# noamzilo/sed-crnn

Measured on AMD Instinct MI355X. Metric: mel-frames/sec training throughput (seq=256, mel=40), higher is better.
Workload: dtype f32; 1 GPU; BASELINE config 2: mono (B=128,256,40,1) per GPU, 3xConv3x3(128)+BN+ReLU+pool(1,2)+dropout0.5, BiGRU 2x128, Linear(256,1), BCEWithLogits, Adam lr 1e-3; full fit step (fwd+loss+bwd+allreduce+Adam); global_batch=128, seq_len=256, n_mels=40, parallelism=single

## Files before the change

### include/sedcrnn.h

```cpp
#ifndef SEDCRNN_H
#define SEDCRNN_H

#include <stddef.h>
#include <stdint.h>

#ifdef __cplusplus
extern "C" {
#endif

#define SED_MAX_CONV 4
#define SED_MAX_GRU 4
#define SED_MAX_DENSE 4

int sed_version(void);
const char* sed_last_error_string(void);

int sed_conv3x3_pack_weights(const float* w_oihw, float* wp_fwd, float* wp_dgrad,
                             int Cout, int Cin, void* stream);

int sed_conv3x3_stat_rows(int B, int Cin, int F, int T, int Cout, int x_is_nchw);

int sed_conv3x3_fwd(const float* x, int x_is_nchw, const float* wp, const float* bias,
                    float* y, float* stat_partials,
                    int B, int Cin, int F, int T, int Cout, void* stream);
// ... 72 lines not shown
                              float drop_p, uint64_t seed, const uint64_t* seed_dev, void* stream);

int sed_bn_relu_pool_route(const float* y, const float* scale, const float* shift, unsigned char* route,
                           int B, int T, int F, int C, int pool_f, int pool_t, void* stream);
int sed_bn_bwd_rows(int B, int T, int pool_t);
int sed_bn_relu_pool_drop_bwd_reduce(const float* y, const float* dout, const float* scale,
                                     const float* shift, const float* mean, const float* rstd,
                                     float* partials, int B, int T, int F, int C, int pool_f,
                                     int pool_t, int out_tcf, float drop_p, uint64_t seed, const uint64_t* seed_dev, void* stream);
int sed_bn_bwd_finalize(const float* partials, int rows, int C, float* sum_g, float* sum_gx,
                        float* dgamma, float* dbeta, void* stream);
int sed_bn_bwd_finalize_small_gamma(const float* partials, int rows, int C, float* sum_g, float* sum_gx,
                                    float* dgamma, float* dbeta, const float* dpooled, const float* pooled,
                                    const float* y, const float* gamma, const float* beta, const float* mean,
                                    const float* rstd, const float* scale, const float* shift,
                                    int B, int T, int F, int pool_f, int pool_t, float drop_p, void* stream);
int sed_bn_bwd_reduce_pooled_supported(int F, int C, int pool_f, int pool_t, int out_tcf);
int sed_bn_bwd_reduce_pooled(const float* pooled, const float* dout, const float* gamma, const float* beta,
                             const float* y, const float* mean, const float* rstd, const float* scale, const float* shift,
                             float* partials, int B, int T, int F, int C, int pool_f, int pool_t, int out_tcf, float drop_p, void* stream);
int sed_bn_relu_pool_drop_bwd_apply(const float* y, const float* dout, const float* scale,
                                    const float* shift, const float* mean, const float* rstd,
                                    const float* sum_g, const float* sum_gx, float* dy,
                                    float* dbias_partials, int B, int T, int F, int C, int pool_f,
                                    int pool_t, int out_tcf, float drop_p, uint64_t seed, const uint64_t* seed_dev, void* stream);
int sed_reduce_rows(const float* partials, int rows, int C, int row_stride, float* out, void* stream);

int sed_conv1_fused_supported(int Cin, int F, int T, int C, int pool_f, int pool_t);
int sed_conv1_fused_rows(int B, int T);
size_t sed_conv1_stats_workspace_bytes(int B, int Cin, int T);
size_t sed_conv1_moments_doubles(int Cin);
int sed_conv1_stats(const float* x, const float* wp, const float* bias, float* stat_partials, void* workspace,
                    int B, int Cin, int F, int T, int C, double* moments, void* stream);
int sed_conv1_bn_relu_pool_drop_fwd(const float* x, const float* wp, const float* bias, const float* scale,
                                    const float* shift, float* out, int B, int Cin, int F, int T, int C,
                                    int pool_f, int pool_t, float drop_p, uint64_t seed, const uint64_t* seed_dev,
                                    unsigned char* argmax_bits, void* stream);
int sed_conv1_route(const float* x, const float* wp, const float* bias, const float* scale, const float* shift,
                    unsigned char* route, int B, int Cin, int F, int T, int C, int pool_f, int pool_t, void* stream);
int sed_conv1_bwd_reduce(const float* x, const float* wp, const float* bias, const float* dout,
                         const float* scale, const float* shift, const float* mean, const float* rstd,
                         float* partials, int B, int Cin, int F, int T, int C, int pool_f, int pool_t,
                         float drop_p, uint64_t seed, const uint64_t* seed_dev, void* stream);
size_t sed_conv1_bwd_apply_workspace_bytes(int B, int Cin, int T, int C);
int sed_conv1_bwd_apply_wgrad(const float* x, const float* wp, const float* bias, const float* dout,
                              const float* scale, const float* shift, const float* mean, const float* rstd,
                              const float* sum_g, const float* sum_gx, float* dw_oihw, float* dbias,
                              void* workspace, int B, int Cin, int F, int T, int C, int pool_f, int pool_t,
                              float drop_p, uint64_t seed, const uint64_t* seed_dev,
                              const float* gamma, const float* beta, float* dgamma, void* stream);

int sed_conv1_rgrad_supported(int Cin, int F, int T, int C, int pool_f, int pool_t);
size_t sed_conv1_bwd_wgrad_workspace_bytes(int B, int Cin, int T, int C);
int sed_conv1_bwd_wgrad(const float* x, const float* dout, const float* pooled, const unsigned char* argmax_bits,
                        const double* moments, const float* wp, const float* bias, const float* mean, const float* rstd,
                        const float* scale, const float* sum_g, const float* sum_gx, float* dw_oihw, float* dbias,
                        void* workspace, int B, int Cin, int F, int T, int C, float drop_p,
                        const float* gamma, const float* beta, float* dgamma, void* stream);
int sed_conv1_bwd_wgrad_assemble(const float* partials, int rows, const double* moments, const float* wp, const float* bias,
                                 const float* mean, const float* rstd, const float* scale, const float* sum_g,
                                 const float* sum_gx, float* dw_oihw, float* dbias, int B, int Cin, int F, int T, int C,
                                 const float* gamma, const float* beta, float* dgamma, void* stream);

int sed_gemm_f32(const float* A, long a_si, long a_sk, const float* B, long b_sk, long b_sj,
                 float* C, long ldc, const float* bias, float beta, int M, int N, int K, void* stream);
size_t sed_gemm_f32_workspace_bytes(int M, int N, int K);
int sed_gemm_f32_ws(const float* A, long a_si, long a_sk, const float* B, long b_sk, long b_sj,
                    float* C, long ldc, const float* bias, int M, int N, int K, void* workspace, void* stream);

int sed_gemm_bf16_nt(const void* A, const void* B, const float* bias, float* C, long ldc, int M, int N, int K, void* stream);

int sed_gemm_f32_wgrad(const float* A, long a_si, long a_sk, const float* B, long b_sk, long b_sj,
                       float* C, long ldc, int M, int N, int K, void* workspace, void* stream);

int sed_linear_fwd(const float* x, const float* W, const float* b, float* y,
                   int M, int K, int N, int relu, void* stream);
size_t sed_linear_bwd_workspace_bytes(int M, int K, int N);
int sed_linear_bwd(const float* x, const float* W, const float* y, float* dy, float* dx,
                   float* dW, float* db, void* workspace, int M, int K, int N, int relu, void* stream);

size_t sed_gru_seq_workspace_bytes(int H);
int sed_gru_seq_fwd(const float* gi, const float* const* whh, const float* const* bhh,
                    float* out, float* saved, void* workspace, int B, int T, int H, void* stream);
size_t sed_gru_seq_bwd_workspace_bytes(int B, int H);
int sed_gru_seq_bwd(const float* dout, const float* saved, const float* const* whh,
                    float* dgi, float* dgh, float* const* dbih, float* const* dbhh, void* workspace,
                    int B, int T, int H, void* stream);
int sed_gru_seq_variant(int B, int H, int* bt, int* hreg, int* hlds);

int sed_loss_fwd_bwd(const float* logits, const float* targets, int n, int kind, float alpha,
                     float gamma, int reduction_mean, float* loss, float* dlogits, float* probs,
                     void* stream);
int sed_sigmoid(const float* x, float* y, int n, void* stream);
int sed_scale(float* x, long n, float alpha, void* stream);

size_t sed_sqnorm_workspace_bytes(long n);
int sed_grad_norm_clip_coef(const float* g, long n, float max_norm, float* norm_out,
                            void* workspace, void* stream);
int sed_adam_step(float* p, const float* g, float* m, float* v, long n, float lr, float beta1,
                  float beta2, float eps, float weight_decay, int step, const float* grad_scale,
                  const uint64_t* step_state, void* stream);
int sed_step_advance(uint64_t* step_state, void* stream);

size_t sed_logmel_tables_bytes(const float* melfb_host, int n_fft, int n_mels);
int sed_logmel_build_tables(const float* window_host, const float* melfb_host, int n_fft, int n_mels,
                            void* tables_host, size_t tables_bytes);
int sed_logmel(const float* pcm, long n_samples, const void* tables, size_t tables_bytes,
               const float* mu, const float* inv_sigma, float* out,
               int n_fft, int hop, int n_mels, int pad_mode, void* stream);
size_t sed_logmel_batch_workspace_bytes(int R);
int sed_logmel_batch(const float* pcm, long pcm_len, const long* clips_host, int R, const void* tables, size_t tables_bytes,
                     const float* mu, const float* inv_sigma, float* out, long out_rows, int n_fft, int hop, int n_mels,
                     int pad_mode, void* workspace, size_t workspace_bytes, void* stream);
size_t sed_logmel_multi_workspace_bytes(int R, int channels);
int sed_logmel_multi(const float* pcm, long pcm_len, const long* clips_host, int R, int channels, const void* tables,
                     size_t tables_bytes, const float* mu, const float* inv_sigma, float* out, long out_rows, int n_fft, int hop,
                     int n_mels, int pad_mode, void* workspace, size_t workspace_bytes, void* stream);
size_t sed_logmel_gcc_workspace_bytes(int R, int channels);
int sed_logmel_gcc(const float* pcm, long pcm_len, const long* clips_host, int R, int channels, const void* tables,
                   size_t tables_bytes, const float* mu, const float* inv_sigma, float* out, long out_rows, int n_fft, int hop,
// ... 58 lines not shown
                      const long* table_host, int S, void* workspace, size_t workspace_bytes, void* stream);

typedef sed_tune_setting sed_decoder_setting;
int sed_detect_events_classwise(const float* probs, long n_out, int K, const sed_decoder_setting* classes_host, int max_events,
                                void* workspace, size_t workspace_bytes, int* cls, int* onset, int* offset, float* peak,
                                int* peak_frame, int* count, void* stream);
int sed_detect_events_batch_classwise(const float* probs, const long* n_out_host, int R, int K,
                                      const sed_decoder_setting* classes_host, int max_events, void* workspace, size_t workspace_bytes,
                                      int* rec, int* cls, int* onset, int* offset, float* peak, int* peak_frame, int* event_off,
                                      void* stream);
int sed_stream_step_classwise(void* state, size_t state_bytes, int S, int K, int win_out, int hop_out, int median, int max_new_windows,
                              int combine, int trim, const sed_decoder_setting* classes_host, const float* logits, long logits_len,
                              const long* table_host, int max_new_decided, float* probs, long probs_rows, int max_events,
                              int* ev_stream, int* cls, int* onset, int* offset, float* peak, int* peak_frame, int* event_off,
                              void* workspace, size_t workspace_bytes, void* stream);

typedef struct sed_net_cfg {
    int B, Cin, F, T;
    int n_conv;
    int C[SED_MAX_CONV];
    int pool_f[SED_MAX_CONV], pool_t[SED_MAX_CONV];
    float drop_p[SED_MAX_CONV];
    int n_gru;
    int H[SED_MAX_GRU];
    int n_dense;
    int D[SED_MAX_DENSE];
    float bn_eps, bn_momentum;
    int conv_mode;
    int flags;
} sed_net_cfg;
#define SED_NET_AUX_FIRST 0x1
#define SED_NET_NO_GATE 0x2
#define SED_NET_DIRECT_CONV 0x4

typedef struct sed_net_params {
    float* conv_w[SED_MAX_CONV];
    float* conv_b[SED_MAX_CONV];
    float* bn_g[SED_MAX_CONV];
    float* bn_b[SED_MAX_CONV];
    float* bn_rm[SED_MAX_CONV];
    float* bn_rv[SED_MAX_CONV];
    float* gru_wih[SED_MAX_GRU][2];
    float* gru_whh[SED_MAX_GRU][2];
    float* gru_bih[SED_MAX_GRU][2];
    float* gru_bhh[SED_MAX_GRU][2];
    float* dense_w[SED_MAX_DENSE];
    float* dense_b[SED_MAX_DENSE];
} sed_net_params;

int sed_net_out_shape(const sed_net_cfg* cfg, int* Tp, int* Fp);
size_t sed_net_workspace_bytes(const sed_net_cfg* cfg, int training);
int sed_net_forward(const sed_net_cfg* cfg, const sed_net_params* p, const float* x, float* logits,
                    void* workspace, int training, uint64_t seed, const uint64_t* seed_dev, void* stream);
int sed_net_backward(const sed_net_cfg* cfg, const sed_net_params* p, const sed_net_params* g,
                     const float* x, const float* dlogits, void* workspace, uint64_t seed, const uint64_t* seed_dev,
                     int stage_begin, int stage_end, void* stream, void* aux_stream);
int sed_net_backward_ready_stage(const sed_net_cfg* cfg, int block);

int sed_net_sync_region(const sed_net_cfg* cfg, int backward, int block, size_t* offset_bytes, size_t* n_floats);
int sed_net_forward_phases(const sed_net_cfg* cfg, const sed_net_params* p, const float* x, float* logits,
                           void* workspace, int training, uint64_t seed, int phase_begin, int phase_end,
                           float count_scale, void* stream);
int sed_net_backward_phases(const sed_net_cfg* cfg, const sed_net_params* p, const sed_net_params* g,
                            const float* x, const float* dlogits, void* workspace, uint64_t seed,
                            int phase_begin, int phase_end, float count_scale, void* stream);

int sed_net_workspace_region(const sed_net_cfg* cfg, int training, const char* name, int index,
                             size_t* offset_bytes, size_t* n_floats);

int sed_net_inference_plan(const sed_net_cfg* cfg, int* conv_bf16, int* proj_bf16);

int sed_net_routing(const sed_net_cfg* cfg, const sed_net_params* p, const float* x, const void* workspace, int block,
                    unsigned char* route, void* stream);

enum sed_kernel_tag {
    SED_K_CONV_MFMA_FWD = 0,
    SED_K_CONV_SMALL_FWD,
    SED_K_CONV_MFMA_WGRAD,
    SED_K_CONV_SMALL_WGRAD,
    SED_K_BN_FWD,
    SED_K_BN_BWD_REDUCE,
    SED_K_BN_BWD_APPLY,
    SED_K_GEMM,
    SED_K_GRU_FWD,
    SED_K_GRU_BWD,
    SED_K_ADAM,
    SED_K_LOGMEL,
    SED_K_CONV_MFMA_DGRAD,
    SED_K_COUNT
// ... 11 lines not shown
```

### sed_crnn_amd/_lib.py

```python
import ctypes as C
import os

HERE = os.path.dirname(os.path.abspath(__file__))
LIB_PATH = os.environ.get("SED_CRNN_LIB") or os.path.join(HERE, "libsedcrnn.so")

SED_MAX_CONV = 4
SED_MAX_GRU = 4
SED_MAX_DENSE = 4

_fp = C.c_void_p
_stream = C.c_void_p


class NetCfg(C.Structure):
    _fields_ = [
        ("B", C.c_int), ("Cin", C.c_int), ("F", C.c_int), ("T", C.c_int),
        ("n_conv", C.c_int),
        ("C", C.c_int * SED_MAX_CONV),
        ("pool_f", C.c_int * SED_MAX_CONV), ("pool_t", C.c_int * SED_MAX_CONV),
        ("drop_p", C.c_float * SED_MAX_CONV),
        ("n_gru", C.c_int), ("H", C.c_int * SED_MAX_GRU),
        ("n_dense", C.c_int), ("D", C.c_int * SED_MAX_DENSE),
        ("bn_eps", C.c_float), ("bn_momentum", C.c_float),
        ("conv_mode", C.c_int),
# ... 26 lines not shown
    "sed_conv3x3_stat_rows": (_i, [_i, _i, _i, _i, _i, _i]),
    "sed_conv3x3_fwd": (_i, [_fp, _i, _fp, _fp, _fp, _fp, _i, _i, _i, _i, _i, _stream]),
    "sed_conv3x3_pack_weights_ex": (_i, [_fp, _fp, _fp, _i, _i, _i, _stream]),
    "sed_conv3x3_fwd_ex": (_i, [_fp, _i, _fp, _fp, _fp, _fp, _i, _i, _i, _i, _i, _i, _stream]),
    "sed_conv3x3_wgrad_workspace_bytes": (_sz, [_i, _i, _i, _i, _i]),
    "sed_conv3x3_wgrad_zero_row_bytes": (_sz, [_i, _i, _i, _i, _i]),
    "sed_conv3x3_wgrad": (_i, [_fp, _i, _fp, _fp, _fp, _i, _i, _i, _i, _i, _stream]),
    "sed_conv3x3_wgrad_ex": (_i, [_fp, _i, _fp, _fp, _fp, _i, _i, _i, _i, _i, _i, _stream]),
    "sed_conv3x3_bn_relu_pool_eval_supported": (_i, [_i, _i, _i, _i, _i]),
    "sed_conv3x3_pack_weights_bn_folded": (_i, [_fp, _fp, _fp, _fp, _fp, _fp, _f, _fp, _fp, _i, _i, _stream]),
    "sed_conv3x3_bn_relu_pool_eval": (_i, [_fp, _fp, _fp, _fp, _i, _i, _i, _i, _i, _stream]),
    "sed_conv3x3_bf16_eval_supported": (_i, [_i, _i, _i, _i, _i]),
    "sed_conv3x3_bf16_pack_weights_bn_folded": (_i, [_fp, _fp, _fp, _fp, _fp, _fp, _f, _fp, _fp, _i, _i, _stream]),
    "sed_conv3x3_bf16_bn_relu_pool_eval": (_i, [_fp, _i, _fp, _fp, _fp, _i, _i, _i, _i, _i, _stream]),
    "sed_conv3x3_dgrad_bnred_rows": (_i, [_i, _i, _i, _i, _i]),
    "sed_conv3x3_dgrad_bnred": (_i, [_fp, _fp, _fp, _fp, _fp, _fp, _fp, _fp, _fp, _fp, _f, _i, _i, _i, _i, _i, _i, _i, _i, _i, _stream]),
    "sed_conv3x3_wino_rows": (_i, [_i, _i, _i, _i, _i]),
    "sed_conv3x3_wino_phase_ticks": (_i, [_fp]),
    "sed_conv3x3_wino_packed_floats": (_sz, [_i, _i]),
    "sed_conv3x3_wino_pack_weights": (_i, [_fp, _fp, _fp, _i, _i, _stream]),
    "sed_conv3x3_wino_fwd": (_i, [_fp, _fp, _fp, _fp, _fp, _i, _i, _i, _i, _i, _stream]),
    "sed_conv3x3_wino_dgrad_bnred": (_i, [_fp, _fp, _fp, _fp, _fp, _fp, _fp, _fp, _fp, _fp, _f, _i, _i, _i, _i, _i, _i, _i, _i, _i, _stream]),
    "sed_conv3x3_wino_pack_weights_bn_folded": (_i, [_fp, _fp, _fp, _fp, _fp, _fp, _f, _fp, _fp, _i, _i, _stream]),
    "sed_conv3x3_wino_bn_relu_pool_eval": (_i, [_fp, _fp, _fp, _fp, _i, _i, _i, _i, _i, _stream]),
    "sed_conv3x3_wino_rg_rows": (_i, [_i, _i, _i, _i, _i, _i]),
    "sed_conv3x3_wino_dgrad_bnred_rg": (_i, [_fp, _fp, _fp, _fp, _fp, _fp, _fp, _fp, _fp, _f, _fp, _i, _fp, _fp, _i, _i, _i, _i, _i, _stream]),
    "sed_conv3x3_dgrad_bnred_rg_rows": (_i, [_i, _i, _i, _i, _i, _i]),
    "sed_conv3x3_dgrad_bnred_rg": (_i, [_fp, _fp, _fp, _fp, _fp, _fp, _fp, _fp, _fp, _f, _fp, _i, _fp, _fp, _i, _i, _i, _i, _i, _stream]),
    "sed_conv1_fused_supported": (_i, [_i, _i, _i, _i, _i, _i]),
    "sed_conv1_fused_rows": (_i, [_i, _i]),
    "sed_conv1_stats_workspace_bytes": (_sz, [_i, _i, _i]),
    "sed_conv1_moments_doubles": (_sz, [_i]),
    "sed_conv1_stats": (_i, [_fp, _fp, _fp, _fp, _fp, _i, _i, _i, _i, _i, _fp, _stream]),
    "sed_conv1_bn_relu_pool_drop_fwd": (_i, [_fp, _fp, _fp, _fp, _fp, _fp, _i, _i, _i, _i, _i, _i, _i, _f, _u64, _fp, _fp, _stream]),
    "sed_conv1_rgrad_supported": (_i, [_i, _i, _i, _i, _i, _i]),
    "sed_conv1_bwd_wgrad_workspace_bytes": (_sz, [_i, _i, _i, _i]),
    "sed_conv1_bwd_wgrad": (_i, [_fp, _fp, _fp, _fp, _fp, _fp, _fp, _fp, _fp, _fp, _fp, _fp, _fp, _fp, _fp, _i, _i, _i, _i, _i, _f, _fp, _fp, _fp, _stream]),
    "sed_conv1_bwd_wgrad_assemble": (_i, [_fp, _i, _fp, _fp, _fp, _fp, _fp, _fp, _fp, _fp, _fp, _fp, _i, _i, _i, _i, _i, _fp, _fp, _fp, _stream]),
    "sed_conv1_route": (_i, [_fp, _fp, _fp, _fp, _fp, _fp, _i, _i, _i, _i, _i, _i, _i, _stream]),
    "sed_conv1_bwd_reduce": (_i, [_fp, _fp, _fp, _fp, _fp, _fp, _fp, _fp, _fp, _i, _i, _i, _i, _i, _i, _i, _f, _u64, _fp, _stream]),
    "sed_conv1_bwd_apply_workspace_bytes": (_sz, [_i, _i, _i, _i]),
    "sed_conv1_bwd_apply_wgrad": (_i, [_fp, _fp, _fp, _fp, _fp, _fp, _fp, _fp, _fp, _fp, _fp, _fp, _fp, _i, _i, _i, _i, _i, _i, _i, _f, _u64, _fp, _fp, _fp, _fp, _stream]),
    "sed_bn_finalize_train": (_i, [_fp, _i, _i, _d, _fp, _fp, _fp, _fp, _f, _f, _fp, _fp, _fp, _fp, _stream]),
    "sed_bn_stat_sums": (_i, [_fp, _i, _i, _fp, _stream]),
    "sed_bn_finalize_from_sums": (_i, [_fp, _i, _d, _fp, _fp, _fp, _fp, _f, _f, _fp, _fp, _fp, _fp, _stream]),
    "sed_bn_finalize_eval": (_i, [_fp, _fp, _fp, _fp, _f, _i, _fp, _fp, _stream]),
    "sed_bn_relu_pool_drop_fwd": (_i, [_fp, _fp, _fp, _fp, _i, _i, _i, _i, _i, _i, _i, _f, _u64, _fp, _stream]),
    "sed_bn_relu_pool_route": (_i, [_fp, _fp, _fp, _fp, _i, _i, _i, _i, _i, _i, _stream]),
    "sed_bn_bwd_rows": (_i, [_i, _i, _i]),
    "sed_bn_relu_pool_drop_bwd_reduce": (_i, [_fp, _fp, _fp, _fp, _fp, _fp, _fp, _i, _i, _i, _i, _i, _i, _i, _f, _u64, _fp, _stream]),
    "sed_bn_bwd_finalize": (_i, [_fp, _i, _i, _fp, _fp, _fp, _fp, _stream]),
    "sed_bn_bwd_finalize_small_gamma": (_i, [_fp, _i, _i, _fp, _fp, _fp, _fp, _fp, _fp, _fp, _fp, _fp, _fp, _fp, _fp, _fp, _i, _i, _i, _i, _i, _f, _stream]),
    "sed_bn_bwd_reduce_pooled_supported": (_i, [_i, _i, _i, _i, _i]),
    "sed_bn_bwd_reduce_pooled": (_i, [_fp, _fp, _fp, _fp, _fp, _fp, _fp, _fp, _fp, _fp, _i, _i, _i, _i, _i, _i, _i, _f, _stream]),
    "sed_bn_relu_pool_drop_bwd_apply": (_i, [_fp, _fp, _fp, _fp, _fp, _fp, _fp, _fp, _fp, _fp, _i, _i, _i, _i, _i, _i, _i, _f, _u64, _fp, _stream]),
    "sed_reduce_rows": (_i, [_fp, _i, _i, _i, _fp, _stream]),
    "sed_gemm_f32": (_i, [_fp, _l, _l, _fp, _l, _l, _fp, _l, _fp, _f, _i, _i, _i, _stream]),
    "sed_gemm_f32_workspace_bytes": (_sz, [_i, _i, _i]),
    "sed_gemm_f32_ws": (_i, [_fp, _l, _l, _fp, _l, _l, _fp, _l, _fp, _i, _i, _i, _fp, _stream]),
    "sed_gemm_bf16_nt": (_i, [_fp, _fp, _fp, _fp, _l, _i, _i, _i, _stream]),
    "sed_gemm_f32_wgrad": (_i, [_fp, _l, _l, _fp, _l, _l, _fp, _l, _i, _i, _i, _fp, _stream]),
    "sed_linear_fwd": (_i, [_fp, _fp, _fp, _fp, _i, _i, _i, _i, _stream]),
    "sed_linear_bwd_workspace_bytes": (_sz, [_i, _i, _i]),
    "sed_linear_bwd": (_i, [_fp, _fp, _fp, _fp, _fp, _fp, _fp, _fp, _i, _i, _i, _i, _stream]),
    "sed_gru_seq_workspace_bytes": (_sz, [_i]),
    "sed_gru_seq_fwd": (_i, [_fp, _pp, _pp, _fp, _fp, _fp, _i, _i, _i, _stream]),
    "sed_gru_seq_bwd_workspace_bytes": (_sz, [_i, _i]),
    "sed_gru_seq_bwd": (_i, [_fp, _fp, _pp, _fp, _fp, _pp, _pp, _fp, _i, _i, _i, _stream]),
    "sed_gru_seq_variant": (_i, [_i, _i, C.POINTER(_i), C.POINTER(_i), C.POINTER(_i)]),
    "sed_loss_fwd_bwd": (_i, [_fp, _fp, _i, _i, _f, _f, _i, _fp, _fp, _fp, _stream]),
    "sed_sigmoid": (_i, [_fp, _fp, _i, _stream]),
    "sed_scale": (_i, [_fp, _l, _f, _stream]),
    "sed_sqnorm_workspace_bytes": (_sz, [_l]),
    "sed_grad_norm_clip_coef": (_i, [_fp, _l, _f, _fp, _fp, _stream]),
    "sed_adam_step": (_i, [_fp, _fp, _fp, _fp, _l, _f, _f, _f, _f, _f, _i, _fp, _fp, _stream]),
    "sed_step_advance": (_i, [_fp, _stream]),
    "sed_logmel_tables_bytes": (_sz, [_fp, _i, _i]),
    "sed_logmel_build_tables": (_i, [_fp, _fp, _i, _i, _fp, _sz]),
    "sed_logmel": (_i, [_fp, _l, _fp, _sz, _fp, _fp, _fp, _i, _i, _i, _i, _stream]),
    "sed_logmel_batch_workspace_bytes": (_sz, [_i]),
    "sed_logmel_batch": (_i, [_fp, _l, _fp, _i, _fp, _sz, _fp, _fp, _fp, _l, _i, _i, _i, _i, _fp, _sz, _stream]),
    "sed_logmel_multi_workspace_bytes": (_sz, [_i, _i]),
    "sed_logmel_multi": (_i, [_fp, _l, _fp, _i, _i, _fp, _sz, _fp, _fp, _fp, _l, _i, _i, _i, _i, _fp, _sz, _stream]),
    "sed_logmel_gcc_workspace_bytes": (_sz, [_i, _i]),
    "sed_logmel_gcc": (_i, [_fp, _l, _fp, _i, _i, _fp, _sz, _fp, _fp, _fp, _l, _i, _i, _i, _i, _i, _fp, _sz, _stream]),
    "sed_resample_workspace_bytes": (_sz, [_i]),
    "sed_resample_check_table": (_i, [_fp, _i, _l, _l, _l, _i, _i, _i]),
    "sed_resample": (_i, [_fp, _l, _i, _i, _fp, _l, _fp, _l, _i, _i, _i, _fp, _i, _fp, _l, _fp, _sz, _stream]),
    "sed_resample_select_workspace_bytes": (_sz, [_i]),
    "sed_resample_select_check_table": (_i, [_fp, _i, _i, _l, _l, _l, _i, _i, _i]),
    "sed_resample_select": (_i, [_fp, _l, _i, _i, _fp, _l, _fp, _l, _i, _i, _i, _fp, _i, _fp, _l, _fp, _sz, _stream]),
    "sed_window_batch": (_i, [_fp, _fp, _l, _i, _i, _i, _fp, _fp, _fp, _i, _i, _i, _fp, _fp, _i, _i, _i, _stream]),
    "sed_pack_sequences": (_i, [_fp, _l, _i, _i, _i, _i, _fp, _stream]),
    "sed_col_mean_std_workspace_bytes": (_sz, [_i]),
    "sed_col_mean_std": (_i, [_fp, _l, _i, _fp, _fp, _fp, _stream]),
    "sed_col_standardize": (_i, [_fp, _l, _i, _fp, _fp, _fp, _stream]),
    "sed_segment_counts": (_i, [_fp, _fp, _l, _i, _i, _f, _fp, _stream]),
    "sed_detect_stitch": (_i, [_fp, _l, _i, _i, _i, _l, _l, _i, _i, _fp, _stream]),
    "sed_detect_workspace_bytes": (_sz, [_l, _i, _i]),
    "sed_detect_events": (_i, [_fp, _l, _i, _i, _f, _f, _i, _i, _i, _fp, _sz, _fp, _fp, _fp, _fp, _fp, _fp, _stream]),
    "sed_detect_batch_workspace_bytes": (_sz, [_l, _i, _i, _i]),
    "sed_detect_stitch_batch": (_i, [_fp, _l, _fp, _i, _i, _i, _i, _fp, _l, _fp, _sz, _stream]),
    "sed_detect_events_batch": (_i, [_fp, _fp, _i, _i, _i, _f, _f, _i, _i, _i, _fp, _sz, _fp, _fp, _fp, _fp, _fp, _fp, _fp, _stream]),
    "sed_tune_workspace_bytes": (_sz, [_l, _i, _i, _i, _i]),
    "sed_tune_sweep": (_i, [_fp, _fp, _i, _i, _fp, _i, _fp, _fp, _fp, _fp, _i, _i, _fp, _sz, _fp, _stream]),
    "sed_stream_state_bytes": (_sz, [_i, _i, _i, _i, _i, _i]),
    "sed_stream_init": (_i, [_fp, _sz, _i, _i, _i, _i, _i, _i, _stream]),
    "sed_stream_reset": (_i, [_fp, _sz, _i, _i, _i, _i, _i, _i, _fp, _i, _stream]),
    "sed_stream_step_workspace_bytes": (_sz, [_i, _i, _i]),
    "sed_stream_step": (_i, [_fp, _sz, _i, _i, _i, _i, _i, _i, _i, _i, _f, _f, _i, _i, _fp, _l, _fp, _i, _fp, _l, _i, _fp, _fp, _fp,
                             _fp, _fp, _fp, _fp, _fp, _sz, _stream]),
    "sed_stream_append_workspace_bytes": (_sz, [_i]),
    "sed_stream_append": (_i, [_fp, _l, _l, _fp, _l, _fp, _l, _fp, _i, _fp, _sz, _stream]),
    "sed_detect_events_classwise": (_i, [_fp, _l, _i, _fp, _i, _fp, _sz, _fp, _fp, _fp, _fp, _fp, _fp, _stream]),
    "sed_detect_events_batch_classwise": (_i, [_fp, _fp, _i, _i, _fp, _i, _fp, _sz, _fp, _fp, _fp, _fp, _fp, _fp, _fp, _stream]),
    "sed_stream_step_classwise": (_i, [_fp, _sz, _i, _i, _i, _i, _i, _i, _i, _i, _fp, _fp, _l, _fp, _i, _fp, _l, _i, _fp, _fp, _fp,
                                       _fp, _fp, _fp, _fp, _fp, _sz, _stream]),
    "sed_prof_enable": (_i, [C.c_uint]),
    "sed_prof_read": (_i, [_i, C.POINTER(_d), C.POINTER(_l), C.POINTER(_d)]),
    "sed_prof_tag_name": (C.c_char_p, [_i]),
    "sed_prof_tag_count": (_i, []),
    "sed_net_out_shape": (_i, [C.POINTER(NetCfg), C.POINTER(_i), C.POINTER(_i)]),
    "sed_net_workspace_bytes": (_sz, [C.POINTER(NetCfg), _i]),
    "sed_net_forward": (_i, [C.POINTER(NetCfg), C.POINTER(NetParams), _fp, _fp, _fp, _i, _u64, _fp, _stream]),
    "sed_net_sync_region": (_i, [C.POINTER(NetCfg), _i, _i, C.POINTER(_sz), C.POINTER(_sz)]),
    "sed_net_workspace_region": (_i, [C.POINTER(NetCfg), _i, C.c_char_p, _i, C.POINTER(_sz), C.POINTER(_sz)]),
    "sed_net_routing": (_i, [C.POINTER(NetCfg), C.POINTER(NetParams), _fp, _fp, _i, _fp, _stream]),
    "sed_net_inference_plan": (_i, [C.POINTER(NetCfg), C.POINTER(C.c_int), C.POINTER(C.c_int)]),
    "sed_net_forward_phases": (_i, [C.POINTER(NetCfg), C.POINTER(NetParams), _fp, _fp, _fp, _i, _u64, _i, _i, _f, _stream]),
    "sed_net_backward_phases": (_i, [C.POINTER(NetCfg), C.POINTER(NetParams), C.POINTER(NetParams), _fp, _fp, _fp, _u64, _i, _i, _f, _stream]),
    "sed_net_backward": (_i, [C.POINTER(NetCfg), C.POINTER(NetParams), C.POINTER(NetParams), _fp, _fp, _fp, _u64, _fp, _i, _i, _stream, _stream]),
    "sed_net_backward_ready_stage": (_i, [C.POINTER(NetCfg), _i]),
}

_lib = None


class SedHipError(RuntimeError):
    pass


def lib():
    global _lib
    if _lib is None:
        if not os.path.exists(LIB_PATH):
            raise SedHipError(
                f"{LIB_PATH} is missing: build it with `python -m sed_crnn_amd.build` "
                "(hipcc --offload-arch=gfx950). sed_crnn_amd has no fallback path.")
        L = C.CDLL(LIB_PATH)
        for name, (res, args) in SIGNATURES.items():
            fn = getattr(L, name)
            fn.restype = res
            fn.argtypes = args
        _lib = L
    return _lib


def check(rc, what=""):
    if rc != 0:
        msg = lib().sed_last_error_string().decode("utf-8", "replace")
        raise SedHipError(f"{what or 'libsedcrnn'} failed (code {rc}): {msg}")
# ... 12 lines not shown
```

### sed_crnn_amd/csrc/bnpool.hip

```cpp
#include "common.h"

#define BN_MAX_BLOCKS 1024

__device__ __forceinline__ void bn_two_channel_sums(const float* __restrict__ part, int rows, int C, int c, bool live,
                                                    double (*sred)[2][2], double* A_out, double* Q_out) {
    const int sl = threadIdx.x >> 1, lane = threadIdx.x & 63, wv = threadIdx.x >> 6;
    double a = 0.0, q = 0.0;
    if (live) {
#pragma unroll 8
        for (int r = sl; r < rows; r += 512) {
            const float* p0 = part + (size_t)r * 2 * C + c;
            a += (double)p0[0];
            q += (double)p0[C];
        }
    }
#pragma unroll
    for (int o = 2; o < 64; o <<= 1) { a += __shfl_xor(a, o, 64); q += __shfl_xor(q, o, 64); }
    if (lane < 2) { sred[wv][lane][0] = a; sred[wv][lane][1] = q; }
    __syncthreads();
    double A = 0.0, Q = 0.0;
    if (threadIdx.x < 2) {
        for (int w = 0; w < 16; ++w) { A += sred[w][threadIdx.x][0]; Q += sred[w][threadIdx.x][1]; }
    }
    *A_out = A; *Q_out = Q;
}

__global__ __launch_bounds__(1024) void bn_finalize_train_k(
    const float* __restrict__ part, int rows, int C, double count, const float* __restrict__ gamma,
    const float* __restrict__ beta, float* __restrict__ rmean, float* __restrict__ rvar, float momentum,
    float eps, float* __restrict__ mean_o, float* __restrict__ rstd_o, float* __restrict__ scale_o,
    float* __restrict__ shift_o) {
    __shared__ double sred[16][2][2];
    const int c = blockIdx.x * 2 + (threadIdx.x & 1);
    double A, Q;
    bn_two_channel_sums(part, rows, C, c, c < C, sred, &A, &Q);
    if (threadIdx.x < 2 && c < C) {
        double m = A / count;
        double var = Q / count - m * m;
        if (var < 0.0) var = 0.0;
        float rstd = (float)(1.0 / sqrt(var + (double)eps));
        float g = gamma[c], bt = beta[c];
        mean_o[c] = (float)m;
        rstd_o[c] = rstd;
        float sc = g * rstd;
        scale_o[c] = sc;
        shift_o[c] = bt - (float)m * sc;
        if (rmean) {
            double unb = count > 1.0 ? var * count / (count - 1.0) : var;
            rmean[c] = (1.f - momentum) * rmean[c] + momentum * (float)m;
            rvar[c] = (1.f - momentum) * rvar[c] + momentum * (float)unb;
        }
    }
}

extern "C" int sed_bn_finalize_train(const float* part, int rows, int C, double count, const float* gamma,
                                     const float* beta, float* rmean, float* rvar, float momentum, float eps,
                                     float* mean, float* rstd, float* scale, float* shift, void* stream) {
    SED_REQUIRE(part && gamma && beta && mean && rstd && scale && shift, "bn_finalize_train: null pointer");
    SED_REQUIRE(rows > 0 && C > 0 && count > 0, "bn_finalize_train: bad sizes rows=%d C=%d", rows, C);
    bn_finalize_train_k<<<cdiv(C, 2), 1024, 0, as_stream(stream)>>>(part, rows, C, count, gamma, beta, rmean, rvar,
                                                                      momentum, eps, mean, rstd, scale, shift);
    SED_LAUNCH_CHECK("bn_finalize_train");
    return 0;
}

__global__ __launch_bounds__(1024) void bn_stat_sums_k(const float* __restrict__ part, int rows, int C, float* __restrict__ sums) {
    __shared__ double s1[32][33], s2[32][33];
    const int cl = threadIdx.x & 31, sl = threadIdx.x >> 5;
    const int c = blockIdx.x * 32 + cl;
    double a = 0.0, q = 0.0;
    if (c < C)
#pragma unroll 8
        for (int r = sl; r < rows; r += 32) {
            a += (double)part[(size_t)r * 2 * C + c];
            q += (double)part[(size_t)r * 2 * C + C + c];
        }
    s1[sl][cl] = a;
    s2[sl][cl] = q;
    __syncthreads();
    if (sl == 0 && c < C) {
        double A = 0.0, Q = 0.0;
        for (int s = 0; s < 32; ++s) { A += s1[s][cl]; Q += s2[s][cl]; }
        sums[c] = (float)A;
        sums[C + c] = (float)Q;
// ... 656 lines not shown
```

### sed_crnn_amd/csrc/common.h

```cpp
#pragma once
#include <hip/hip_runtime.h>
#include <stdint.h>
#include <stdio.h>
#include "../../include/sedcrnn.h"

#define SED_EINVAL (-1)
#define SED_EUNSUPPORTED (-2)

void sed_set_error(const char* fmt, ...);

#define SED_REQUIRE(cond, ...)                     \
    do {                                           \
        if (!(cond)) {                             \
            sed_set_error(__VA_ARGS__);            \
            return SED_EINVAL;                     \
        }                                          \
    } while (0)

#define SED_LAUNCH_CHECK(name)                                                      \
    do {                                                                            \
        hipError_t e__ = hipGetLastError();                                         \
        if (e__ != hipSuccess) {                                                    \
            sed_set_error("%s: launch failed: %s", name, hipGetErrorString(e__));   \
            return (int)e__;                                                        \
        }                                                                           \
    } while (0)

#define SED_TRY(expr)            \
    do {                         \
        int r__ = (expr);        \
        if (r__ != 0) return r__; \
    } while (0)

extern unsigned g_sed_prof_mask;
void sed_prof_begin(int tag, hipStream_t s, double units);
void sed_prof_end(int tag, hipStream_t s);
struct SedProfScope {
    int tag; hipStream_t s; bool on;
    SedProfScope(int tag_, hipStream_t s_, double units) : tag(tag_), s(s_), on((g_sed_prof_mask >> tag_) & 1u) {
        if (on) sed_prof_begin(tag, s, units);
    }
    ~SedProfScope() { if (on) sed_prof_end(tag, s); }
};

int sed_internal_conv_pack_multi(int n, const float* const* w, float* const* wf, float* const* wd, const int* Cout, const int* Cin,
                                 const int* wino_f, const int* wino_d, void* stream);

int sed_internal_conv_pack_eval(int n, const float* const* w, const float* const* bias, const float* const* gamma,
                                const float* const* beta, const float* const* rm, const float* const* rv, float eps,
                                float* const* wf, float* const* scale, float* const* shift, float* const* bias_folded, const int* fold,
                                const int* wino, const int* Cout, const int* Cin, const float* perm_src0, const float* perm_src1, float* perm_dst,
                                int perm_rows, int perm_C, int perm_Fp, void* const* wbf16, int perm_bf16, void* stream);

int sed_internal_conv3x3_wgrad(const float* x, int x_is_nchw, const float* dy, float* dw, void* workspace,
                               int B, int Cin, int F, int T, int Cout, int mode, unsigned* arrive, void* stream);
int sed_internal_conv3x3_wgrad_workgroups(int B, int Cin, int F, int T, int Cout, int x_is_nchw, int mode);

int sed_internal_stream_gate(const unsigned* counter, unsigned target, int timeout_us, void* stream);

int sed_internal_logmel_multi(const float* pcm, long pcm_len, const long* clips_host, int R, int channels, const void* tables,
                              size_t tables_bytes, const float* mu, const float* inv_sigma, float* out, long out_rows, int n_fft, int hop,
                              int n_mels, int pad_mode, int row_stride, void* workspace, size_t workspace_bytes, void* stream);

static inline hipStream_t as_stream(void* s) { return (hipStream_t)s; }
static inline int cdiv(long a, long b) { return (int)((a + b - 1) / b); }

typedef float f32x2 __attribute__((ext_vector_type(2)));
typedef float f32x4 __attribute__((ext_vector_type(4)));
typedef float f32x16 __attribute__((ext_vector_type(16)));

#ifdef __HIPCC__
__device__ __forceinline__ uint32_t sed_fmix32(uint32_t h) {
    h ^= h >> 16; h *= 0x85ebca6bu; h ^= h >> 13; h *= 0xc2b2ae35u; h ^= h >> 16;
    return h;
}
__device__ __forceinline__ float sed_uniform(uint64_t seed, uint64_t idx) {
    uint32_t lo = (uint32_t)idx, hi = (uint32_t)(idx >> 32);
    uint32_t h = sed_fmix32(lo ^ (uint32_t)seed);
    h = sed_fmix32(h + (uint32_t)(seed >> 32) + hi * 0x9E3779B1u);
    return (float)(h >> 8) * (1.0f / 16777216.0f);
}
__device__ __forceinline__ float sed_drop_mult(uint64_t seed, uint64_t idx, float p, float inv_keep) {
    return (sed_uniform(seed, idx) >= p) ? inv_keep : 0.0f;
}

__device__ __forceinline__ int sed_fdiv(int n, float inv) { return (int)(((float)n + 0.5f) * inv); }

__device__ __forceinline__ float wave_sum(float v) {
#pragma unroll
    for (int o = 32; o > 0; o >>= 1) v += __shfl_xor(v, o, 64);
    return v;
}
__device__ __forceinline__ double wave_sum_d(double v) {
#pragma unroll
    for (int o = 32; o > 0; o >>= 1) v += __shfl_xor(v, o, 64);
    return v;
}
__device__ __forceinline__ float sigmoidf_(float x) { return 1.0f / (1.0f + __expf(-x)); }
#endif
```

### sed_crnn_amd/csrc/conv.hip

```cpp
#include "common.h"
#include "conv_shared.h"
#include <type_traits>

#define CV_CIC 32
#define CV_LD 36
#define CV_MTW 5
#define WG_FT 40
#define WG_NX 6
#define WG_ND 10

#define CV_TPAD 56
#define CV_NH 8

struct ConvPlan {
    int kind;
    int TT;
    int FT, nft;
    int nct;
    int tblocks;
    int rows;
    int nco, nci;
    size_t lds;
    double score;
};
// ... 62 lines not shown
    int cc = ci >> 5, g = (ci & 31) >> 3, h = (ci & 7) >> 2, j = ci & 3;
    int cot = co >> 5, r = co & 31;
    return ((((((size_t)tap * (Cin >> 5) + cc) * 4 + g) * (Cout >> 5) + cot) * 64) + r + 32 * h) * 4 + j;
}

__global__ void conv_pack_w_k(const float* __restrict__ w, float* __restrict__ wf,
                              float* __restrict__ wd, int Cout, int Cin) {
    int i = blockIdx.x * blockDim.x + threadIdx.x;
    int n = Cout * Cin * 9;
    if (i >= n) return;
    int tap = i % 9, ci = (i / 9) % Cin, co = i / (9 * Cin);
    float v = w[i];
    const bool frag = (Cin % 32 == 0) && (Cout % 32 == 0);
    if (wf) wf[frag ? conv_frag_index(tap, co, ci, Cout, Cin) : ((size_t)tap * Cout + co) * Cin + ci] = v;
    if (wd) wd[frag ? conv_frag_index(8 - tap, ci, co, Cin, Cout) : ((size_t)(8 - tap) * Cin + ci) * Cout + co] = v;
}

extern "C" int sed_conv3x3_pack_weights(const float* w, float* wf, float* wd, int Cout, int Cin, void* stream) {
    SED_REQUIRE(w && Cout > 0 && Cin > 0, "conv3x3_pack_weights: bad arguments");
    int n = Cout * Cin * 9;
    conv_pack_w_k<<<cdiv(n, 256), 256, 0, as_stream(stream)>>>(w, wf, wd, Cout, Cin);
    SED_LAUNCH_CHECK("conv_pack_w");
    return 0;
}

struct ConvPackMulti {
    const float* w[SED_MAX_CONV]; float* wf[SED_MAX_CONV]; float* wd[SED_MAX_CONV]; int Cout[SED_MAX_CONV], Cin[SED_MAX_CONV];
    const float* gamma[SED_MAX_CONV]; const float* beta[SED_MAX_CONV]; const float* rm[SED_MAX_CONV]; const float* rv[SED_MAX_CONV];
    const float* bias[SED_MAX_CONV]; float* scale_out[SED_MAX_CONV]; float* shift_out[SED_MAX_CONV]; float* bias_out[SED_MAX_CONV];
    int fold[SED_MAX_CONV]; float eps;
    int wino_f[SED_MAX_CONV], wino_d[SED_MAX_CONV];
    const float* perm_src[2]; float* perm_dst; int perm_rows, perm_C, perm_Fp;
    __bf16* wb[SED_MAX_CONV]; int perm_bf16;
};
__global__ void conv_pack_w_multi_k(ConvPackMulti a, int n) {
    const int l = blockIdx.y;
    const int i = blockIdx.x * blockDim.x + threadIdx.x;
    if (l == n) {
        extern __shared__ __attribute__((aligned(16))) float prow[];
        const int K = a.perm_C * a.perm_Fp;
        for (int row = blockIdx.x; row < 2 * a.perm_rows; row += gridDim.x) {
            const float* src = a.perm_src[row >= a.perm_rows] + (size_t)(row >= a.perm_rows ? row - a.perm_rows : row) * K;
            __syncthreads();
            for (int k = threadIdx.x; k < K; k += blockDim.x) prow[k] = src[k];
            __syncthreads();
            float* dst = a.perm_dst + (size_t)row * K;
            for (int k = threadIdx.x; k < K; k += blockDim.x) {
                const int f = k / a.perm_C, c = k - f * a.perm_C;
                if (a.perm_bf16) ((__bf16*)a.perm_dst + (size_t)row * K)[k] = (__bf16)prow[c * a.perm_Fp + f];
                else dst[k] = prow[c * a.perm_Fp + f];
            }
        }
        return;
    }
    const int Cout = a.Cout[l], Cin = a.Cin[l];
    if (a.wino_f[l] | a.wino_d[l])
        wino_pack_one(a.w[l], a.wino_f[l] ? a.wf[l] : nullptr, a.wino_d[l] ? a.wd[l] : nullptr, Cout, Cin, i,
                      a.fold[l] ? a.gamma[l] : nullptr, a.rv[l], a.eps);
    if (a.gamma[l] && i < Cout) {
        const float sc = a.gamma[l][i] / sqrtf(a.rv[l][i] + a.eps), sh = a.beta[l][i] - a.rm[l][i] * sc;
        if (a.scale_out[l]) { a.scale_out[l][i] = sc; a.shift_out[l][i] = sh; }
        if (a.fold[l]) a.bias_out[l][i] = (a.bias[l] ? a.bias[l][i] : 0.f) * sc + sh;
    }
    if (i >= Cout * Cin * 9) return;
    const int tap = i % 9, ci = (i / 9) % Cin, co = i / (9 * Cin);
    float v = a.w[l][i];
    if (a.fold[l]) v *= a.gamma[l][co] / sqrtf(a.rv[l][co] + a.eps);
    const bool frag = (Cin % 32 == 0) && (Cout % 32 == 0);
    if (a.wb[l]) a.wb[l][bf16_eval_frag_index(tap, co, ci, Cout, Cin)] = (__bf16)v;
    if (a.wf[l] && !a.wino_f[l]) a.wf[l][frag ? conv_frag_index(tap, co, ci, Cout, Cin) : ((size_t)tap * Cout + co) * Cin + ci] = v;
    if (a.wd[l] && !a.wino_d[l]) a.wd[l][frag ? conv_frag_index(8 - tap, ci, co, Cin, Cout) : ((size_t)(8 - tap) * Cin + ci) * Cout + co] = v;
}
static int set_lds_early(size_t bytes) {
    hipError_t e = hipFuncSetAttribute((const void*)conv_pack_w_multi_k, hipFuncAttributeMaxDynamicSharedMemorySize, (int)bytes);
    if (e != hipSuccess) { sed_set_error("hipFuncSetAttribute(%zu B LDS): %s", bytes, hipGetErrorString(e)); return (int)e; }
    return 0;
}
static int pack_multi_launch(const ConvPackMulti& a, int n, void* stream) {
    int nmax = 0;
    for (int l = 0; l < n; ++l) {
        const int nl = a.Cout[l] * a.Cin[l] * 9;
        if (nl > nmax) nmax = nl;
    }
    const int gx = cdiv(nmax > 0 ? nmax : 1, 256);
    const size_t lds = a.perm_src[0] ? (size_t)a.perm_C * a.perm_Fp * sizeof(float) : 0;
    SED_REQUIRE(lds <= 64 * 1024, "conv_pack: a GRU input row of %zu bytes does not fit the re-ordering buffer", lds);
    if (lds > 48 * 1024) SED_TRY(set_lds_early(lds));
    conv_pack_w_multi_k<<<dim3(gx, n + (a.perm_src[0] ? 1 : 0)), 256, lds, as_stream(stream)>>>(a, n);
    SED_LAUNCH_CHECK("conv_pack_w_multi");
    return 0;
}
int sed_internal_conv_pack_multi(int n, const float* const* w, float* const* wf, float* const* wd, const int* Cout, const int* Cin,
                                 const int* wino_f, const int* wino_d, void* stream) {
    SED_REQUIRE(n > 0 && n <= SED_MAX_CONV && w && wf && wd && Cout && Cin, "conv_pack_multi: bad arguments");
    ConvPackMulti a{};
    for (int l = 0; l < n; ++l) {
        SED_REQUIRE(w[l] && Cout[l] > 0 && Cin[l] > 0, "conv_pack_multi: bad layer %d", l);
        a.w[l] = w[l]; a.wf[l] = wf[l]; a.wd[l] = wd[l]; a.Cout[l] = Cout[l]; a.Cin[l] = Cin[l];
        a.wino_f[l] = (wino_f && wino_f[l] && wf[l]) ? 1 : 0;
        a.wino_d[l] = (wino_d && wino_d[l] && wd[l]) ? 1 : 0;
        SED_REQUIRE(!(a.wino_f[l] | a.wino_d[l]) || (Cout[l] % 64 == 0 && Cin[l] % 64 == 0), "conv_pack_multi: layer %d cannot take the Winograd packing", l);
    }
    return pack_multi_launch(a, n, stream);
}
int sed_internal_conv_pack_eval(int n, const float* const* w, const float* const* bias, const float* const* gamma,
                                const float* const* beta, const float* const* rm, const float* const* rv, float eps,
                                float* const* wf, float* const* scale, float* const* shift, float* const* bias_folded, const int* fold,
                                const int* wino, const int* Cout, const int* Cin, const float* perm_src0, const float* perm_src1, float* perm_dst,
                                int perm_rows, int perm_C, int perm_Fp, void* const* wbf16, int perm_bf16, void* stream) {
    SED_REQUIRE(n > 0 && n <= SED_MAX_CONV && w && gamma && beta && rm && rv && wf && scale && shift && fold && Cout && Cin, "conv_pack_eval: bad arguments");
    ConvPackMulti a{};
    for (int l = 0; l < n; ++l) {
        const bool wb = wbf16 && wbf16[l];
        SED_REQUIRE(w[l] && gamma[l] && beta[l] && rm[l] && rv[l] && (wf[l] || wb) && Cout[l] > 0 && Cin[l] > 0, "conv_pack_eval: bad layer %d", l);
        SED_REQUIRE(!wb || (fold[l] && Cout[l] % 32 == 0 && Cin[l] % 16 == 0 && !(wino && wino[l])), "conv_pack_eval: layer %d cannot take the bf16 packing", l);
        a.wb[l] = wb ? (__bf16*)wbf16[l] : nullptr;
        SED_REQUIRE(fold[l] ? (bias_folded && bias_folded[l]) : (scale[l] && shift[l]), "conv_pack_eval: layer %d lacks its outputs", l);
        a.w[l] = w[l]; a.wf[l] = wf[l]; a.Cout[l] = Cout[l]; a.Cin[l] = Cin[l];
        a.gamma[l] = gamma[l]; a.beta[l] = beta[l]; a.rm[l] = rm[l]; a.rv[l] = rv[l]; a.bias[l] = bias ? bias[l] : nullptr;
        a.scale_out[l] = scale[l]; a.shift_out[l] = shift[l]; a.bias_out[l] = bias_folded ? bias_folded[l] : nullptr; a.fold[l] = fold[l];
        a.wino_f[l] = (wino && wino[l]) ? 1 : 0;
        SED_REQUIRE(!a.wino_f[l] || (Cout[l] % 64 == 0 && Cin[l] % 64 == 0), "conv_pack_eval: layer %d cannot take the Winograd packing", l);
    }
    a.eps = eps;
    if (perm_src0) {
        SED_REQUIRE(perm_src1 && perm_dst && perm_rows > 0 && perm_C > 0 && perm_Fp > 0, "conv_pack_eval: bad permutation");
        a.perm_src[0] = perm_src0; a.perm_src[1] = perm_src1; a.perm_dst = perm_dst; a.perm_rows = perm_rows; a.perm_C = perm_C; a.perm_Fp = perm_Fp;
        a.perm_bf16 = perm_bf16 ? 1 : 0;
// ... 1871 lines not shown
```

### sed_crnn_amd/csrc/conv1.hip

```cpp
#include "common.h"

#define C1_TT 4
#define C1_MAXBLOCKS 2048

template <int CIN>
struct C1W { f32x4 w[9 * CIN]; f32x4 b; };

template <int CIN>
__device__ __forceinline__ void c1_load_w(C1W<CIN>& W, const float* __restrict__ wp, const float* __restrict__ bias,
                                          int Cout, int cg) {
#pragma unroll
    for (int tap = 0; tap < 9; ++tap)
#pragma unroll
        for (int ci = 0; ci < CIN; ++ci)
#pragma unroll
            for (int k = 0; k < 4; ++k) W.w[tap * CIN + ci][k] = wp[((size_t)tap * Cout + cg * 4 + k) * CIN + ci];
    W.b = bias ? *(const f32x4*)(bias + cg * 4) : (f32x4){0, 0, 0, 0};
}

template <int CIN>
__device__ __forceinline__ f32x4 c1_conv(const C1W<CIN>& W, const float* __restrict__ halo, int tl, int f, int F2) {
    f32x4 acc = W.b;
#pragma unroll
    for (int kh = 0; kh < 3; ++kh)
// ... 285 lines not shown
            const int tl = q / F, f = q - tl * F;
            const int b = tile / tblocks, t0 = (tile - b * tblocks) * C1_GT;
            if (t0 + tl >= T) continue;
            const float* hb = halo + u * hn;
            float v[NK];
#pragma unroll
            for (int kh = 0; kh < 3; ++kh)
#pragma unroll
                for (int kw = 0; kw < 3; ++kw)
#pragma unroll
                    for (int ci = 0; ci < CIN; ++ci) v[(kh * 3 + kw) * CIN + ci] = hb[((tl + kw) * F2 + f + kh) * CIN + ci];
            int g = NK;
#pragma unroll
            for (int k = 0; k < NK; ++k) {
                acc[k] += v[k];
#pragma unroll
                for (int k2 = k; k2 < NK; ++k2) acc[g++] += v[k] * v[k2];
            }
        }
    }
    __syncthreads();
    float* red = smem;
    const int lane = tid & 63, wave = tid >> 6;
#pragma unroll
    for (int i = 0; i < NG; ++i) {
        const float sum = wave_sum(acc[i]);
        if (lane == 0) red[i * 4 + wave] = sum;
    }
    __syncthreads();
    for (int i = tid; i < NG; i += 256)
        partials[(size_t)blockIdx.x * NG + i] = (red[i * 4] + red[i * 4 + 1]) + (red[i * 4 + 2] + red[i * 4 + 3]);
}

template <int CIN>
__global__ __launch_bounds__(256) void conv1_gram_finalize_k(const float* __restrict__ partials, int nblk, const float* __restrict__ wp,
                                                             const float* __restrict__ bias, double count, int C, float* __restrict__ stat,
                                                             double* __restrict__ gram_out) {
    constexpr int NK = 9 * CIN, NG = NK + NK * (NK + 1) / 2;
    __shared__ double G[NG];
    __shared__ double Gq[4][64];
    {
        const int il = threadIdx.x & 63, q = threadIdx.x >> 6;
        for (int i0 = 0; i0 < NG; i0 += 64) {
            const int i = i0 + il;
            double a = 0.0;
            if (i < NG) {
#pragma unroll 8
                for (int r = q; r < nblk; r += 4) a += (double)partials[(size_t)r * NG + i];
            }
            Gq[q][il] = a;
            __syncthreads();
            if (q == 0 && i < NG) G[i] = (Gq[0][il] + Gq[1][il]) + (Gq[2][il] + Gq[3][il]);
            __syncthreads();
        }
    }
    __syncthreads();
    if (gram_out)
        for (int i = threadIdx.x; i < NG; i += 256) gram_out[i] = G[i];
    for (int c = threadIdx.x; c < C; c += 256) {
        double w[NK];
#pragma unroll
        for (int k = 0; k < NK; ++k) w[k] = (double)wp[((size_t)(k / CIN) * C + c) * CIN + (k % CIN)];
        const double b = bias ? (double)bias[c] : 0.0;
        double ws1 = 0.0, q = 0.0;
        int g = NK;
#pragma unroll
        for (int k = 0; k < NK; ++k) {
            ws1 += w[k] * G[k];
#pragma unroll
            for (int k2 = k; k2 < NK; ++k2) { q += (k2 == k ? 1.0 : 2.0) * w[k] * w[k2] * G[g]; ++g; }
        }
        stat[c] = (float)(count * b + ws1);
        stat[C + c] = (float)(q + 2.0 * b * ws1 + count * b * b);
    }
}

#define C1_MM_BLOCKS 1024
typedef float f32x4_t __attribute__((ext_vector_type(4)));
template <int CIN>
__global__ __launch_bounds__(256) void conv1_moments_mfma_k(const float* __restrict__ x, float* __restrict__ partials, int B, int F, int T) {
    constexpr int NK = 9 * CIN, NT = (NK + 1 + 15) / 16, NP = NT * (NT + 1) / 2;
    extern __shared__ __attribute__((aligned(16))) float smem[];
    const int F2 = F + 2;
    const int hn = (C1_GT + 2) * F2 * CIN;
    float* halo = smem;
    const int tid = threadIdx.x, lane = tid & 63, wave = tid >> 6, m = lane & 15, kq = lane >> 4;
    const int tblocks = (T + C1_GT - 1) / C1_GT, ntiles = B * tblocks;
    int off[NT];
    bool real[NT];
#pragma unroll
    for (int t = 0; t < NT; ++t) {
        const int fi = 16 * t + m;
        real[t] = fi < NK;
        const int k = real[t] ? fi : 0, tap = k / CIN, ci = k - tap * CIN, kh = tap / 3, kw = tap - kh * 3;
        off[t] = real[t] ? (kw * F2 + kh) * CIN + ci + kq * CIN : hn + (fi == NK ? 0 : 1);
    }
    f32x4_t acc[NP];
#pragma unroll
    for (int q = 0; q < NP; ++q) acc[q] = (f32x4_t){0.f, 0.f, 0.f, 0.f};
    if (tid == 0) { halo[hn] = 1.f; halo[hn + 1] = 0.f; }
    for (int tile = blockIdx.x; tile < ntiles; tile += gridDim.x) {
        const int b = tile / tblocks, t0 = (tile - b * tblocks) * C1_GT;
        __syncthreads();
        for (int j = tid; j < hn; j += 256) {
            int tt = j % (C1_GT + 2), ff = (j / (C1_GT + 2)) % F2, ci = j / ((C1_GT + 2) * F2);
            const int t = t0 + tt - 1, f = ff - 1;
            float v = 0.f;
// ... 388 lines not shown
#define C1_LAUNCH(CIN_, P12_)                                                                                          \
    do {                                                                                                               \
        if (lds > 48 * 1024)                                                                                           \
            (void)hipFuncSetAttribute((const void*)conv1_fused_k<CIN_, MODE, P12_>, hipFuncAttributeMaxDynamicSharedMemorySize, (int)lds); \
        conv1_fused_k<CIN_, MODE, P12_><<<grid, 256, lds, s>>>(x, wp, bias, scale, shift, mean, rstd, sum_g, sum_gx, dout, out, \
                                                              partials, B, F, T, C, pf, pt, drop_p, seed, seed_dev);  \
    } while (0)
    if (Cin == 1) { if (p12) C1_LAUNCH(1, true); else C1_LAUNCH(1, false); }
    else if (Cin == 2) { if (p12) C1_LAUNCH(2, true); else C1_LAUNCH(2, false); }
    else if ((MODE == 1 || MODE == 4) && p12) {
        if (Cin == 3) C1_LAUNCH(3, true);
        else C1_LAUNCH(4, true);
    } else {
        sed_set_error("conv1: %d input channels are supported by the forward pass with the (1,2) pool only", Cin);
        return SED_EUNSUPPORTED;
    }
#undef C1_LAUNCH
    return 0;
}

#define C1_CHECK(who)                                                                                             \
    SED_REQUIRE(sed_conv1_fused_supported(Cin, F, T, C, pf, pt), who ": shape Cin=%d F=%d T=%d C=%d pool=(%d,%d) is not " \
                "supported by the fused first block", Cin, F, T, C, pf, pt)

extern "C" size_t sed_conv1_stats_workspace_bytes(int B, int Cin, int T) {
    const int nk = 9 * Cin;
    if (Cin > 2) {
        const int nt = (nk + 1 + 15) / 16, np = nt * (nt + 1) / 2;
        return (size_t)C1_MM_BLOCKS * np * 256 * sizeof(float) + (size_t)(nk + nk * (nk + 1) / 2) * sizeof(double);
    }
    return (size_t)256 * (nk + nk * (nk + 1) / 2) * sizeof(float);
}

extern "C" int sed_conv1_stats(const float* x, const float* wp, const float* bias, float* stat_partials, void* workspace,
                               int B, int Cin, int F, int T, int C, double* gram_out, void* stream) {
    SED_REQUIRE(x && wp && stat_partials && workspace, "conv1_stats: null pointer");
    SED_REQUIRE(c1_shape_ok(Cin, F, T, C, 1, 1, 4), "conv1_stats: shape Cin=%d F=%d T=%d C=%d is not supported", Cin, F, T, C);
    hipStream_t s = as_stream(stream);
    SedProfScope prof(SED_K_CONV_SMALL_FWD, s, 4.0 * B * Cin * (double)F * T);
    if (Cin > 2) {
        const int nk = 9 * Cin, nt = (nk + 1 + 15) / 16, np = nt * (nt + 1) / 2;
        int nb = B * ((T + C1_GT - 1) / C1_GT);
        if (nb > C1_MM_BLOCKS) nb = C1_MM_BLOCKS;
        size_t lds = ((size_t)(C1_GT + 2) * (F + 2) * Cin + 4) * sizeof(float), red = (size_t)4 * np * 256 * sizeof(float);
        if (red > lds) lds = red;
        SED_REQUIRE(lds <= 150 * 1024, "conv1_stats: F=%d Cin=%d needs %zu B of LDS", F, Cin, lds);
        const double cnt = (double)B * T * F;
        double* G = gram_out ? gram_out : (double*)((float*)workspace + (size_t)C1_MM_BLOCKS * np * 256);
#define C1_MOM(CIN_)                                                                                                              \
    do {                                                                                                                          \
        if (lds > 48 * 1024) (void)hipFuncSetAttribute((const void*)conv1_moments_mfma_k<CIN_>, hipFuncAttributeMaxDynamicSharedMemorySize, (int)lds); \
        conv1_moments_mfma_k<CIN_><<<nb, 256, lds, s>>>(x, (float*)workspace, B, F, T);                                             \
        conv1_moments_mfma_sum_k<CIN_><<<dim3(nk + 1, nk + 1), 64, 0, s>>>((const float*)workspace, nb, G);                       \
        conv1_moments_stat_k<CIN_><<<cdiv(C, 4), 256, 0, s>>>(G, wp, bias, cnt, C, stat_partials);                                 \
    } while (0)
        if (Cin == 3) C1_MOM(3); else C1_MOM(4);
#undef C1_MOM
        SED_LAUNCH_CHECK("conv1_moments");
        return 0;
    }
    const int pf = 1, pt = 1;
    C1_CHECK("conv1_stats");
    int grid = (B * ((T + C1_GT - 1) / C1_GT) + C1_GR - 1) / C1_GR;
    if (grid > 256) grid = 256;
    const int nk = 9 * Cin, ng = nk + nk * (nk + 1) / 2;
    size_t lds = (size_t)C1_GR * (C1_GT + 2) * (F + 2) * Cin * sizeof(float), red = (size_t)ng * 4 * sizeof(float);
    SED_REQUIRE(lds <= 150 * 1024, "conv1_stats: F=%d Cin=%d needs %zu B of LDS", F, Cin, lds);
    if (red > lds) lds = red;
    const double count = (double)B * T * F;
    if (lds > 48 * 1024) {
        (void)hipFuncSetAttribute((const void*)conv1_gram_k<1>, hipFuncAttributeMaxDynamicSharedMemorySize, (int)lds);
        (void)hipFuncSetAttribute((const void*)conv1_gram_k<2>, hipFuncAttributeMaxDynamicSharedMemorySize, (int)lds);
    }
    if (Cin == 1) {
        conv1_gram_k<1><<<grid, 256, lds, s>>>(x, (float*)workspace, B, F, T);
        SED_LAUNCH_CHECK("conv1_gram");
        conv1_gram_finalize_k<1><<<1, 256, 0, s>>>((const float*)workspace, grid, wp, bias, count, C, stat_partials, gram_out);
    } else {
        conv1_gram_k<2><<<grid, 256, lds, s>>>(x, (float*)workspace, B, F, T);
        SED_LAUNCH_CHECK("conv1_gram");
        conv1_gram_finalize_k<2><<<1, 256, 0, s>>>((const float*)workspace, grid, wp, bias, count, C, stat_partials, gram_out);
    }
    SED_LAUNCH_CHECK("conv1_gram_finalize");
    return 0;
}

extern "C" int sed_conv1_bn_relu_pool_drop_fwd(const float* x, const float* wp, const float* bias, const float* scale,
                                               const float* shift, float* out, int B, int Cin, int F, int T, int C,
                                               int pf, int pt, float drop_p, uint64_t seed, const uint64_t* seed_dev,
                                               unsigned char* argmax_bits, void* stream) {
    SED_REQUIRE(x && wp && scale && shift && out, "conv1_fwd: null pointer");
    SED_REQUIRE(drop_p >= 0.f && drop_p < 1.f, "conv1_fwd: drop_p=%f out of [0,1)", drop_p);
    SED_REQUIRE(c1_shape_ok(Cin, F, T, C, pf, pt, (pf == 1 && pt == 2) ? 4 : 2), "conv1_fwd: shape Cin=%d F=%d T=%d C=%d pool=(%d,%d) is not "
                "supported by the fused first block", Cin, F, T, C, pf, pt);
    hipStream_t s = as_stream(stream);
    SedProfScope prof(SED_K_BN_FWD, s, 4.0 * B * C * (double)(T / pt) * (F / pf));
    SED_REQUIRE(!argmax_bits || (pf == 1 && pt == 2), "conv1_fwd: arg-max bits exist for the (1,2) pool only");
    SED_TRY(c1_launch<1>(x, wp, bias, scale, shift, nullptr, nullptr, nullptr, nullptr, nullptr, out, reinterpret_cast<float*>(argmax_bits), B, Cin, F, T, C, pf, pt, drop_p, seed, seed_dev, s));
    SED_LAUNCH_CHECK("conv1_fwd");
    return 0;
}

extern "C" int sed_conv1_route(const float* x, const float* wp, const float* bias, const float* scale, const float* shift,
                               unsigned char* route, int B, int Cin, int F, int T, int C, int pf, int pt, void* stream) {
    SED_REQUIRE(x && wp && scale && shift && route, "conv1_route: null pointer");
    SED_REQUIRE(c1_shape_ok(Cin, F, T, C, pf, pt, (pf == 1 && pt == 2) ? 4 : 2), "conv1_route: shape Cin=%d F=%d T=%d C=%d pool=(%d,%d) is not "
                "supported by the fused first block", Cin, F, T, C, pf, pt);
    SED_REQUIRE(pf * pt <= 254, "conv1_route: a %dx%d window does not fit the one-byte code", pf, pt);
    SED_TRY(c1_launch<4>(x, wp, bias, scale, shift, nullptr, nullptr, nullptr, nullptr, nullptr, reinterpret_cast<float*>(route), nullptr,
                         B, Cin, F, T, C, pf, pt, 0.f, 0, nullptr, as_stream(stream)));
    SED_LAUNCH_CHECK("conv1_route");
    return 0;
}

extern "C" int sed_conv1_bwd_reduce(const float* x, const float* wp, const float* bias, const float* dout,
                                    const float* scale, const float* shift, const float* mean, const float* rstd,
                                    float* partials, int B, int Cin, int F, int T, int C, int pf, int pt, float drop_p,
// ... 103 lines not shown
```

### sed_crnn_amd/csrc/gemm.hip

```cpp
#include <type_traits>
#include "common.h"

#define GM_BK 32
#define GM_LDK 36

template <bool KC, int NR, int TILE>
__device__ __forceinline__ void gm_load(f32x4* reg, const float* __restrict__ P, long s_mn, long s_k, int mn0, int MN,
                                        int K, int vec, int k0, int tid) {
#pragma unroll
    for (int u = 0; u < NR; ++u) {
        int i = tid + u * 256;
        f32x4 v = {0, 0, 0, 0};
        if (KC) {
            int row = i >> 3, kq = i & 7;
            int m = mn0 + row, k = k0 + kq * 4;
            const float* p = P + (long)m * s_mn + k;
            if (m < MN) {
                if (vec && k + 3 < K) v = *(const f32x4*)p;
                else
#pragma unroll
                    for (int e = 0; e < 4; ++e) if (k + e < K) v[e] = p[e];
            }
        } else {
            int kk = i / (TILE / 4), mq = i - kk * (TILE / 4);
// ... 393 lines not shown
    double a = 0.0;
#pragma unroll 8
    for (int c = 0; c < chunks; ++c) a += (double)part[(size_t)c * tot + i];
    if (i < NK) dW[i] = (float)a;
    else if (db) db[i - NK] = (float)a;
}

extern "C" size_t sed_linear_bwd_workspace_bytes(int M, int K, int N) {
    return (size_t)cdiv(M, LIN_CHUNK) * ((size_t)N * K + N) * sizeof(float);
}

extern "C" int sed_linear_bwd(const float* x, const float* W, const float* y, float* dy, float* dx, float* dW,
                              float* db, void* workspace, int M, int K, int N, int relu, void* stream) {
    SED_REQUIRE(x && W && dy && dW && workspace && M > 0 && K > 0 && N > 0, "linear_bwd: bad arguments");
    SED_REQUIRE(!relu || y, "linear_bwd: relu=1 needs the forward output y");
    hipStream_t s = as_stream(stream);
    if (relu) {
        long n = (long)M * N;
        linear_relu_mask_k<<<cdiv(n, 256), 256, 0, s>>>(y, dy, n);
        SED_LAUNCH_CHECK("linear_relu_mask");
    }
    if (dx) {
        long n = (long)M * K;
        linear_dx_k<<<cdiv(n, 256), 256, 0, s>>>(dy, W, dx, M, K, N);
        SED_LAUNCH_CHECK("linear_dx");
    }
    int tot = N * K + N, chunks = cdiv(M, LIN_CHUNK);
    linear_dw_partial_k<<<dim3(cdiv(tot, 256), chunks), 256, 0, s>>>(dy, x, (float*)workspace, M, K, N);
    SED_LAUNCH_CHECK("linear_dw_partial");
    linear_dw_reduce_k<<<cdiv(tot, 256), 256, 0, s>>>((const float*)workspace, chunks, tot, N * K, dW, db);
    SED_LAUNCH_CHECK("linear_dw_reduce");
    return 0;
}
```

### sed_crnn_amd/csrc/gru.hip

```cpp
#include "common.h"

static inline int gru_bt(int H, int B) {
    int bt = B >= 512 ? 4 : (B >= 256 ? 2 : 1);
    if (H >= 128 && bt > 2) bt = 2;
    return bt;
}

__global__ void gru_pack_whh_t_k(const float* __restrict__ w0, const float* __restrict__ w1,
                                 float* __restrict__ wt, int H) {
    int i = blockIdx.x * blockDim.x + threadIdx.x;
    int n = 3 * H * H;
    if (i >= 2 * n) return;
    int dir = i / n, e = i - dir * n;
    int g = e / H, k = e - g * H;
    const float* w = dir ? w1 : w0;
    wt[(size_t)dir * n + (size_t)k * 3 * H + g] = w[e];
}

constexpr int gru_nt(int hreg) { return hreg > 0 ? ((3 * hreg + 63) / 64) * 64 : 1024; }

__device__ __forceinline__ float gru_dot4(float w0, float w1, float w2, float w3, const f32x4& h) {
    return fmaf(w3, h[3], fmaf(w2, h[2], fmaf(w0, h[0], w1 * h[1])));
}

// ... 273 lines not shown
    const int bt = gru_bt(H, B);
    if (H == 8 || H == 16 || H == 32 || H == 64 || H == 128) return {bt, H, 0};
    if (H == 256 && bt == 1) return {bt, hyb_hreg, GRU_HL};
    return {bt, 0, 0};
}

extern "C" int sed_gru_seq_variant(int B, int H, int* bt, int* hreg, int* hlds) {
    SED_REQUIRE(bt && hreg && hlds, "gru_seq_variant: null pointer");
    SED_REQUIRE(B > 0 && H > 0 && H % 4 == 0 && 3 * H <= 1024, "gru_seq_variant: H=%d must be a multiple of 4 and <= 341", H);
    const GruVariant v = gru_variant(H, B, GRU_HR_FWD);
    *bt = v.bt; *hreg = v.hreg; *hlds = v.hlds;
    return 0;
}

#define GRU_BT3(HR, KERNEL, ...)                                                              \
    if (v.bt == 1) KERNEL<HR, 1><<<grid, nt, lds, s>>>(__VA_ARGS__);                          \
    else if (v.bt == 2) KERNEL<HR, 2><<<grid, nt, lds, s>>>(__VA_ARGS__);                     \
    else KERNEL<HR, 4><<<grid, nt, lds, s>>>(__VA_ARGS__)
#define GRU_DISPATCH(KERNEL, ...)                                                             \
    if (v.hlds > 0) {                                                                         \
        KERNEL<GRU_HRX, 1, 256, GRU_HL><<<grid, nt, lds + (size_t)GRU_HL * 768 * sizeof(float), s>>>(__VA_ARGS__); \
    } else switch (v.hreg) {                                                                  \
        case 8: GRU_BT3(8, KERNEL, __VA_ARGS__); break;                                       \
        case 16: GRU_BT3(16, KERNEL, __VA_ARGS__); break;                                     \
        case 32: GRU_BT3(32, KERNEL, __VA_ARGS__); break;                                     \
        case 64: GRU_BT3(64, KERNEL, __VA_ARGS__); break;                                     \
        case 128:                                                                             \
            if (v.bt == 1) KERNEL<128, 1><<<grid, nt, lds, s>>>(__VA_ARGS__);                 \
            else KERNEL<128, 2><<<grid, nt, lds, s>>>(__VA_ARGS__);                           \
            break;                                                                            \
        default: GRU_BT3(0, KERNEL, __VA_ARGS__); break;                                      \
    }

extern "C" int sed_gru_seq_fwd(const float* gi, const float* const* whh, const float* const* bhh, float* out,
                               float* saved, void* workspace, int B, int T, int H, void* stream) {
    SED_REQUIRE(gi && whh && bhh && out && workspace && whh[0] && whh[1] && bhh[0] && bhh[1], "gru_seq_fwd: null pointer");
    SED_REQUIRE(B > 0 && T > 0 && H > 0 && H % 4 == 0 && 3 * H <= 1024, "gru_seq_fwd: H=%d must be a multiple of 4 and <= 341", H);
    hipStream_t s = as_stream(stream);
    float* wt = (float*)workspace;
    int n = 2 * 3 * H * H;
    gru_pack_whh_t_k<<<cdiv(n, 256), 256, 0, s>>>(whh[0], whh[1], wt, H);
    SED_LAUNCH_CHECK("gru_pack_whh_t");
    const GruVariant v = gru_variant(H, B, GRU_HR_FWD);
    dim3 grid(cdiv(B, v.bt), 2);
    int nt = gru_threads(H);
    size_t lds = (size_t)v.bt * 4 * H * sizeof(float);
    SedProfScope prof(SED_K_GRU_FWD, s, 2.0 * 2 * B * (double)T * 3 * H * H);
    if (v.hlds > 0)
        (void)hipFuncSetAttribute((const void*)gru_seq_fwd_k<GRU_HR_FWD, 1, 256, GRU_HL>, hipFuncAttributeMaxDynamicSharedMemorySize, 160 * 1024);
#define GRU_HRX GRU_HR_FWD
    GRU_DISPATCH(gru_seq_fwd_k, gi, wt, bhh[0], bhh[1], out, saved, B, T, H);
#undef GRU_HRX
    SED_LAUNCH_CHECK("gru_seq_fwd");
    return 0;
}

extern "C" size_t sed_gru_seq_bwd_workspace_bytes(int B, int H) { return (size_t)cdiv(B, gru_bt(H, B)) * 2 * 4 * H * sizeof(float); }

extern "C" int sed_gru_seq_bwd(const float* dout, const float* saved, const float* const* whh, float* dgi,
                               float* dgh, float* const* dbih, float* const* dbhh, void* workspace, int B, int T,
                               int H, void* stream) {
    SED_REQUIRE(dout && saved && whh && whh[0] && whh[1] && dgi && dgh, "gru_seq_bwd: null pointer");
    const bool want_bias = dbih && dbhh;
    SED_REQUIRE(!want_bias || (workspace && dbih[0] && dbih[1] && dbhh[0] && dbhh[1]), "gru_seq_bwd: bias gradients need all four outputs and a workspace");
    float* bpart = want_bias ? (float*)workspace : nullptr;
    SED_REQUIRE(B > 0 && T > 0 && H > 0 && H % 4 == 0 && 3 * H <= 1024, "gru_seq_bwd: H=%d must be a multiple of 4 and <= 341", H);
    hipStream_t s = as_stream(stream);
    const GruVariant v = gru_variant(H, B, GRU_HR);
    dim3 grid(cdiv(B, v.bt), 2);
    int nt = gru_threads(H);
    size_t lds = (size_t)v.bt * 6 * H * sizeof(float);
    SedProfScope prof(SED_K_GRU_BWD, s, 2.0 * 2 * B * (double)T * 3 * H * H);
    if (v.hlds > 0)
        (void)hipFuncSetAttribute((const void*)gru_seq_bwd_k<GRU_HR, 1, 256, GRU_HL>, hipFuncAttributeMaxDynamicSharedMemorySize, 160 * 1024);
#define GRU_HRX GRU_HR
    GRU_DISPATCH(gru_seq_bwd_k, dout, saved, whh[0], whh[1], dgi, dgh, bpart, B, T, H);
#undef GRU_HRX
    SED_LAUNCH_CHECK("gru_seq_bwd");
    if (want_bias) {
        gru_bias_grad_k<<<cdiv(8 * H, 256), 256, 0, s>>>(bpart, cdiv(B, v.bt), H, dbih[0], dbih[1], dbhh[0], dbhh[1]);
        SED_LAUNCH_CHECK("gru_bias_grad");
    }
    return 0;
}
```

### sed_crnn_amd/csrc/misc.hip

```cpp
#include "common.h"

__global__ __launch_bounds__(1024) void loss_fwd_bwd_k(const float* __restrict__ x, const float* __restrict__ t,
                                                       int n, int kind, float alpha, float gamma, float scale,
                                                       float* __restrict__ loss, float* __restrict__ dx,
                                                       float* __restrict__ probs) {
    __shared__ double red[16];
    double acc = 0.0;
    for (int i = threadIdx.x; i < n; i += 1024) {
        float xi = x[i], ti = t[i];
        float p = 1.f / (1.f + expf(-xi));
        float l, d;
        if (kind == 0) {
            l = fmaxf(xi, 0.f) - xi * ti + log1pf(expf(-fabsf(xi)));
            d = p - ti;
        } else {
            bool pos = (ti == 1.f);
            float pt = pos ? p : 1.f - p;
            float om = 1.f - pt;
            float lg = logf(pt + 1e-12f);
            float pw = powf(om, gamma);
            l = -alpha * pw * lg;
            float dpw = (gamma == 0.f) ? 0.f : gamma * powf(om, gamma - 1.f);
            float dl_dpt = -alpha * (-dpw * lg + pw / (pt + 1e-12f));
            float dpt_dx = pos ? p * (1.f - p) : -p * (1.f - p);
            d = dl_dpt * dpt_dx;
        }
        acc += (double)l;
        if (dx) dx[i] = d * scale;
        if (probs) probs[i] = p;
    }
    acc = wave_sum_d(acc);
    if ((threadIdx.x & 63) == 0) red[threadIdx.x >> 6] = acc;
    __syncthreads();
    if (threadIdx.x == 0) {
        double a = 0.0;
        for (int w = 0; w < 16; ++w) a += red[w];
        loss[0] = (float)(a * (double)scale);
    }
}

extern "C" int sed_loss_fwd_bwd(const float* logits, const float* targets, int n, int kind, float alpha, float gamma,
                                int reduction_mean, float* loss, float* dlogits, float* probs, void* stream) {
    SED_REQUIRE(logits && targets && loss && n > 0, "loss_fwd_bwd: bad arguments");
    SED_REQUIRE(kind == 0 || kind == 1, "loss_fwd_bwd: kind must be 0 (bce) or 1 (focal)");
    float scale = reduction_mean ? 1.f / (float)n : 1.f;
    loss_fwd_bwd_k<<<1, 1024, 0, as_stream(stream)>>>(logits, targets, n, kind, alpha, gamma, scale, loss, dlogits, probs);
    SED_LAUNCH_CHECK("loss_fwd_bwd");
    return 0;
}

__global__ void sigmoid_k(const float* __restrict__ x, float* __restrict__ y, int n) {
    int i = blockIdx.x * blockDim.x + threadIdx.x;
    if (i < n) y[i] = 1.f / (1.f + expf(-x[i]));
}

extern "C" int sed_sigmoid(const float* x, float* y, int n, void* stream) {
    SED_REQUIRE(x && y && n > 0, "sigmoid: bad arguments");
    sigmoid_k<<<cdiv(n, 256), 256, 0, as_stream(stream)>>>(x, y, n);
    SED_LAUNCH_CHECK("sigmoid");
// ... 126 lines not shown
```

### sed_crnn_amd/csrc/net.hip

```cpp
#include <string.h>
#include "common.h"

namespace {

struct ConvL { int Cin, C, T, F, Tp, Fp, pf, pt, rows, bn_rows, nchw, fused; float drop;
               int red_rows;
               int rg_rows;
               int rgrad;
               int wino, wino_d;
               int ev;
               int bf; };

struct GruL { int in, H; };

struct Layout {
    int n_conv, n_gru, n_dense, M, Tp, Fp, feat;
    int proj_bf;
    ConvL cv[SED_MAX_CONV];
    GruL gr[SED_MAX_GRU];
    int dK[SED_MAX_DENSE], dN[SED_MAX_DENSE];
    size_t wp_f[SED_MAX_CONV], wp_d[SED_MAX_CONV], conv_out[SED_MAX_CONV], stat[SED_MAX_CONV];
    size_t mean[SED_MAX_CONV], rstd[SED_MAX_CONV], scale[SED_MAX_CONV], shift[SED_MAX_CONV];
    size_t pooled[SED_MAX_CONV], bn_sums[SED_MAX_CONV], c1_stat_ws, c1_bits, c1_mom;
    size_t bias_f[SED_MAX_CONV];
    size_t wih_perm;
    size_t gi[SED_MAX_GRU], gout[SED_MAX_GRU], saved[SED_MAX_GRU], gru_ws;
    size_t act[SED_MAX_DENSE];
    size_t wgrad_zrow;
    size_t wg_arrive;
    size_t bn_part, sum_g, sum_gx, dbias_part, dconv[SED_MAX_CONV], gradA, wgrad_ws, wgrad_ws_aux, c1_ws, dgi[SED_MAX_GRU], dgh[SED_MAX_GRU], gru_bws, dgout[SED_MAX_GRU];
    size_t dact[SED_MAX_DENSE], lin_ws, gemm_ws, gemm_ws_aux;
    size_t total;
};

struct Carver {
    size_t off = 0;
    size_t take(size_t n) { size_t o = off; off += (n + 63) & ~(size_t)63; return o; }
};

int build_layout(const sed_net_cfg* c, int training, Layout* L) {
    SED_REQUIRE(c, "net: null config");
    SED_REQUIRE(c->B > 0 && c->Cin > 0 && c->F > 0 && c->T > 0, "net: bad input shape B=%d Cin=%d F=%d T=%d", c->B, c->Cin, c->F, c->T);
    SED_REQUIRE(c->n_conv >= 1 && c->n_conv <= SED_MAX_CONV, "net: n_conv=%d out of range", c->n_conv);
    SED_REQUIRE(c->n_gru >= 1 && c->n_gru <= SED_MAX_GRU, "net: n_gru=%d out of range", c->n_gru);
    SED_REQUIRE(c->n_dense >= 1 && c->n_dense <= SED_MAX_DENSE, "net: n_dense=%d out of range", c->n_dense);
    SED_REQUIRE(c->conv_mode >= 0 && c->conv_mode <= 2, "net: conv_mode=%d (0 = exact fp32, 1 = bf16x3 experiment, 2 = bf16 inference)", c->conv_mode);
    SED_REQUIRE(c->conv_mode != 2 || !training, "net: conv_mode 2 (bf16 inference) is an eval-only plan; training runs with conv_mode 0 or 1");
    SED_REQUIRE((c->flags & ~(SED_NET_AUX_FIRST | SED_NET_NO_GATE | SED_NET_DIRECT_CONV)) == 0, "net: unknown flags 0x%x", c->flags);
    memset(L, 0, sizeof(*L));
    L->n_conv = c->n_conv; L->n_gru = c->n_gru; L->n_dense = c->n_dense;
    const int fm = c->conv_mode == 2 ? 0 : c->conv_mode;
    int bfl[SED_MAX_CONV] = {0};
    if (c->conv_mode == 2) {
        int Ci = c->Cin, Ti = c->T, Fi = c->F;
        int ok[SED_MAX_CONV] = {0};
        for (int l = 0; l < c->n_conv; ++l) {
            const int pf = c->pool_f[l], pt = c->pool_t[l];
            ok[l] = l > 0 && pf == 1 && pt == 2 && c->C[l] > 0 && Ti >= 2 && sed_conv3x3_bf16_eval_supported(c->B, Ci, Fi, Ti, c->C[l]);
            if (l == c->n_conv - 1 && (size_t)c->C[l] * Fi * sizeof(float) > 64 * 1024) ok[l] = 0;
            Ci = c->C[l]; Ti = pt > 0 ? Ti / pt : Ti; Fi = pf > 0 ? Fi / pf : Fi;
        }
        for (int l = c->n_conv - 1; l >= 0 && ok[l]; --l) bfl[l] = 1;
    }
    Carver cv;
    int Cin = c->Cin, T = c->T, F = c->F;
    size_t max_pool = 0, max_wgrad = 0, c1_ws = 64, c1_stat_ws = 64;
    int max_bn_rows = 0, maxC = 0;
    for (int l = 0; l < c->n_conv; ++l) {
        ConvL& q = L->cv[l];
        q.Cin = Cin; q.C = c->C[l]; q.T = T; q.F = F; q.pf = c->pool_f[l]; q.pt = c->pool_t[l];
        q.drop = c->drop_p[l]; q.nchw = (l == 0);
        SED_REQUIRE(q.C > 0 && q.C % 4 == 0, "net: conv channels C[%d]=%d must be a positive multiple of 4", l, q.C);
        SED_REQUIRE(q.pf >= 1 && q.pt >= 1 && T / q.pt >= 1 && F / q.pf >= 1,
                    "net: block %d: T=%d/F=%d smaller than the pool (%d,%d)", l, T, F, q.pt, q.pf);
        SED_REQUIRE(q.drop >= 0.f && q.drop < 1.f, "net: drop_p[%d]=%f out of [0,1)", l, q.drop);
        q.Tp = T / q.pt; q.Fp = F / q.pf;
        q.fused = (l == 0 && c->n_conv > 1 && sed_conv1_fused_supported(q.Cin, q.F, q.T, q.C, q.pf, q.pt)) ? 1 : 0;
        q.bf = bfl[l];
        if (l == 0 && !q.fused && c->n_conv > 1 && q.Cin <= 4 && fm == 0 &&
            sed_conv1_rgrad_supported(q.Cin, q.F, q.T, q.C, q.pf, q.pt) &&
            sed_conv3x3_dgrad_bnred_rows(c->B, c->C[1], q.F / q.pf, q.T / q.pt, q.C) > 0)
// ... 51 lines not shown
        if (l == 1 && rr > 0 && L->cv[0].fused && L->cv[0].rgrad && L->cv[0].Cin <= 2) {
            const int gr = q.wino_d ? sed_conv3x3_wino_rg_rows(c->B, q.C, q.F, q.T, q.Cin, L->cv[0].Cin)
                                    : sed_conv3x3_dgrad_bnred_rg_rows(c->B, q.C, q.F, q.T, q.Cin, L->cv[0].Cin);
            L->cv[0].rg_rows = gr;
            const size_t need = (size_t)gr * q.Cin * (1 + 9 * L->cv[0].Cin);
            if (need > c1_ws) c1_ws = need;
        }
    }
    L->c1_stat_ws = cv.take(c1_stat_ws);
    L->c1_bits = L->cv[0].rgrad ? cv.take(((size_t)c->B * L->cv[0].Tp * L->cv[0].Fp * (L->cv[0].C / 4) + 3) / 4) : 0;
    L->c1_mom = L->cv[0].rgrad ? cv.take(2 * sed_conv1_moments_doubles(L->cv[0].Cin)) : 0;
    L->Tp = T; L->Fp = F; L->feat = Cin * F; L->M = c->B * T;
    const size_t M = (size_t)L->M;
    if (L->cv[c->n_conv - 1].ev && (size_t)L->feat * sizeof(float) > 64 * 1024) {
        ConvL& q = L->cv[c->n_conv - 1];
        q.ev = 0;
        L->conv_out[c->n_conv - 1] = cv.take((size_t)c->B * q.T * q.F * q.C);
    }
    L->proj_bf = L->cv[c->n_conv - 1].bf;
    L->wih_perm = ((L->cv[c->n_conv - 1].ev || L->proj_bf) && c->H[0] > 0) ? cv.take((size_t)6 * c->H[0] * L->feat / (L->proj_bf ? 2 : 1)) : 0;
    int in = L->feat, maxH = 0, max2H = 0;
    for (int i = 0; i < c->n_gru; ++i) {
        int H = c->H[i];
        SED_REQUIRE(H > 0 && H % 4 == 0 && 3 * H <= 1024, "net: GRU hidden H[%d]=%d must be a multiple of 4 and <= 341", i, H);
        L->gr[i].in = in; L->gr[i].H = H;
        L->gi[i] = cv.take(M * 6 * H);
        L->gout[i] = cv.take(M * 2 * H);
        L->saved[i] = training ? cv.take(M * 10 * H) : 0;
        if (H > maxH) maxH = H;
        in = 2 * H;
        if (in > max2H) max2H = in;
    }
    L->gru_ws = cv.take((size_t)6 * maxH * maxH);
    size_t max_lin_ws = 0;
    for (int j = 0; j < c->n_dense; ++j) {
        SED_REQUIRE(c->D[j] > 0, "net: dense size D[%d]=%d", j, c->D[j]);
        L->dK[j] = in; L->dN[j] = c->D[j];
        L->act[j] = (j < c->n_dense - 1) ? cv.take(M * c->D[j]) : 0;
        size_t w = sed_linear_bwd_workspace_bytes(L->M, in, c->D[j]) / sizeof(float);
        if (w > max_lin_ws) max_lin_ws = w;
        in = c->D[j];
    }
    if (training) {
        L->bn_part = cv.take((size_t)max_bn_rows * 2 * maxC);
        L->sum_g = cv.take((size_t)2 * maxC); L->sum_gx = 0;
        L->dbias_part = cv.take((size_t)max_bn_rows * maxC);
        for (int l = 0; l < c->n_conv; ++l)
            L->dconv[l] = L->cv[l].fused ? 0 : cv.take((size_t)c->B * L->cv[l].T * L->cv[l].F * L->cv[l].C);
        size_t ga = max_pool > M * (size_t)L->feat ? max_pool : M * (size_t)L->feat;
        L->gradA = cv.take(ga);
        L->wg_arrive = cv.take(64);
        L->wgrad_ws = cv.take(max_wgrad + 64);
        L->wgrad_ws_aux = cv.take(max_wgrad + 64);
        L->c1_ws = cv.take(c1_ws);
        for (int i = 0; i < c->n_gru; ++i) {
            L->dgi[i] = cv.take(M * 6 * c->H[i]);
            L->dgh[i] = cv.take(M * 6 * c->H[i]);
        }
        L->gru_bws = cv.take(sed_gru_seq_bwd_workspace_bytes(c->B, maxH) / sizeof(float));
        for (int i = 0; i < c->n_gru; ++i) L->dgout[i] = cv.take(M * 2 * c->H[i]);
        for (int j = 0; j < c->n_dense - 1; ++j) L->dact[j] = cv.take(M * c->D[j]);
        L->lin_ws = cv.take(max_lin_ws);
    }
    {
        size_t gw = 0;
        for (int i = 0; i < c->n_gru; ++i) {
            size_t f = sed_gemm_f32_workspace_bytes(L->M, 6 * c->H[i], L->gr[i].in) / sizeof(float);
            if (f > gw) gw = f;
            if (training) {
                size_t a = sed_gemm_f32_workspace_bytes(3 * c->H[i], c->H[i], L->M) / sizeof(float);
                size_t b = sed_gemm_f32_workspace_bytes(6 * c->H[i], L->gr[i].in, L->M) / sizeof(float);
                if (a > gw) gw = a;
                if (b > gw) gw = b;
            }
        }
        L->gemm_ws = cv.take(gw + 64);
        L->gemm_ws_aux = training ? cv.take(gw + 64) : 0;
    }
    L->total = cv.off;
    return 0;
}

inline uint64_t layer_seed(uint64_t seed, int l) { return seed + 0x9E3779B97F4A7C15ull * (uint64_t)(l + 1); }

}

extern "C" int sed_net_out_shape(const sed_net_cfg* cfg, int* Tp, int* Fp) {
    Layout L;
    SED_TRY(build_layout(cfg, 0, &L));
    if (Tp) *Tp = L.Tp;
    if (Fp) *Fp = L.Fp;
    return 0;
}

extern "C" size_t sed_net_workspace_bytes(const sed_net_cfg* cfg, int training) {
    Layout L;
    if (build_layout(cfg, training, &L) != 0) return 0;
    return L.total * sizeof(float);
}

static int forward_impl(const sed_net_cfg* c, const sed_net_params* p, const float* x, float* logits, void* workspace,
                        int training, uint64_t seed, const uint64_t* seed_dev, int pb, int pe, float count_scale, void* stream) {
    SED_REQUIRE(p && x && logits && workspace, "net_forward: null pointer");
    Layout L;
    SED_TRY(build_layout(c, training, &L));
    SED_REQUIRE(pb >= 0 && pe <= 2 * L.n_conv + 1 && pb < pe, "net_forward: bad phase range [%d,%d)", pb, pe);
    float* ws = (float*)workspace;
    const int B = c->B;
    SED_REQUIRE(c->conv_mode != 2 || (pb == 0 && pe == 2 * L.n_conv + 1), "net_forward: the bf16 inference plan (conv_mode 2) runs whole, not in phases");
    const bool eval_plan = !training && (c->conv_mode == 0 || c->conv_mode == 2) && pb == 0 && pe == 2 * L.n_conv + 1;
    const ConvL& qtop = L.cv[L.n_conv - 1];
    const bool wih_permuted = eval_plan && (qtop.ev || L.proj_bf) && L.wih_perm != 0;
    if (eval_plan) {
        const float* w[SED_MAX_CONV]; const float* bs[SED_MAX_CONV]; const float* gm[SED_MAX_CONV]; const float* bt[SED_MAX_CONV];
        const float* rm[SED_MAX_CONV]; const float* rv[SED_MAX_CONV];
        float* wf[SED_MAX_CONV]; float* sc[SED_MAX_CONV]; float* sh[SED_MAX_CONV]; float* bf[SED_MAX_CONV];
        int fold[SED_MAX_CONV], co[SED_MAX_CONV], ci[SED_MAX_CONV], wn[SED_MAX_CONV];
        void* wb[SED_MAX_CONV];
        for (int l = 0; l < L.n_conv; ++l) {
            SED_REQUIRE(p->conv_w[l] && p->conv_b[l] && p->bn_g[l] && p->bn_b[l] && p->bn_rm[l] && p->bn_rv[l],
                        "net_forward: missing parameters of conv block %d", l);
            w[l] = p->conv_w[l]; bs[l] = p->conv_b[l]; gm[l] = p->bn_g[l]; bt[l] = p->bn_b[l]; rm[l] = p->bn_rm[l]; rv[l] = p->bn_rv[l];
            wf[l] = ws + L.wp_f[l]; sc[l] = ws + L.scale[l]; sh[l] = ws + L.shift[l]; bf[l] = ws + L.bias_f[l];
            fold[l] = L.cv[l].ev || L.cv[l].bf; co[l] = L.cv[l].C; ci[l] = L.cv[l].Cin; wn[l] = L.cv[l].ev && L.cv[l].wino;
            wb[l] = L.cv[l].bf ? (void*)wf[l] : nullptr;
            if (L.cv[l].bf) wf[l] = nullptr;
        }
        if (wih_permuted) SED_REQUIRE(p->gru_wih[0][0] && p->gru_wih[0][1], "net_forward: missing parameters of GRU layer 0");
        SED_TRY(sed_internal_conv_pack_eval(L.n_conv, w, bs, gm, bt, rm, rv, c->bn_eps, wf, sc, sh, bf, fold, wn, co, ci,
                                            wih_permuted ? p->gru_wih[0][0] : nullptr, wih_permuted ? p->gru_wih[0][1] : nullptr,
                                            ws + L.wih_perm, 3 * L.gr[0].H, qtop.C, qtop.Fp, wb, L.proj_bf, stream));
        for (int l = 0; l < L.n_conv; ++l) {
            const ConvL& q = L.cv[l];
            const float* in = (l == 0) ? x : ws + L.pooled[l - 1];
            const int last = (l == L.n_conv - 1);
            if (q.bf) {
                SED_TRY(sed_conv3x3_bf16_bn_relu_pool_eval(in, l > 0 && L.cv[l - 1].bf, ws + L.wp_f[l], ws + L.bias_f[l], ws + L.pooled[l],
                                                           B, q.Cin, q.F, q.T, q.C, stream));
            } else if (q.fused) {
                SED_TRY(sed_conv1_bn_relu_pool_drop_fwd(in, ws + L.wp_f[l], p->conv_b[l], ws + L.scale[l], ws + L.shift[l], ws + L.pooled[l],
                                                        B, q.Cin, q.F, q.T, q.C, q.pf, q.pt, 0.f, 0, nullptr, nullptr, stream));
            } else if (q.ev && q.wino) {
                SED_TRY(sed_conv3x3_wino_bn_relu_pool_eval(in, ws + L.wp_f[l], ws + L.bias_f[l], ws + L.pooled[l], B, q.Cin, q.F, q.T, q.C, stream));
            } else if (q.ev) {
                SED_TRY(sed_conv3x3_bn_relu_pool_eval(in, ws + L.wp_f[l], ws + L.bias_f[l], ws + L.pooled[l], B, q.Cin, q.F, q.T, q.C, stream));
            } else {
                SED_TRY(sed_conv3x3_fwd_ex(in, q.nchw, ws + L.wp_f[l], p->conv_b[l], ws + L.conv_out[l], nullptr, B, q.Cin, q.F, q.T, q.C, 0, stream));
                SED_TRY(sed_bn_relu_pool_drop_fwd(ws + L.conv_out[l], ws + L.scale[l], ws + L.shift[l], ws + L.pooled[l], B,
                                                  q.T, q.F, q.C, q.pf, q.pt, last, 0.f, 0, nullptr, stream));
            }
        }
    }
    const bool packed_up_front = !eval_plan && pb == 0 && c->conv_mode == 0 && L.n_conv > 1;
    if (packed_up_front) {
        const float* w[SED_MAX_CONV]; float* wf[SED_MAX_CONV]; float* wd[SED_MAX_CONV]; int co[SED_MAX_CONV], ci[SED_MAX_CONV];
        int wnf[SED_MAX_CONV], wnd[SED_MAX_CONV];
        for (int l = 0; l < L.n_conv; ++l) {
            SED_REQUIRE(p->conv_w[l], "net_forward: missing parameters of conv block %d", l);
            w[l] = p->conv_w[l]; wf[l] = ws + L.wp_f[l]; wd[l] = (training && l > 0) ? ws + L.wp_d[l] : nullptr;
            co[l] = L.cv[l].C; ci[l] = L.cv[l].Cin; wnf[l] = L.cv[l].wino; wnd[l] = L.cv[l].wino_d;
        }
        SED_TRY(sed_internal_conv_pack_multi(L.n_conv, w, wf, wd, co, ci, wnf, wnd, stream));
    }
    for (int l = 0; l < L.n_conv && !eval_plan; ++l) {
        const ConvL& q = L.cv[l];
        const float* in = (l == 0) ? x : ws + L.pooled[l - 1];
        const bool do_a = pb <= 2 * l && 2 * l < pe, do_b = pb <= 2 * l + 1 && 2 * l + 1 < pe;
        if (!do_a && !do_b) continue;
        const bool one_shot = do_a && do_b && count_scale == 1.f;
        SED_REQUIRE(p->conv_w[l] && p->conv_b[l] && p->bn_g[l] && p->bn_b[l] && p->bn_rm[l] && p->bn_rv[l],
                    "net_forward: missing parameters of conv block %d", l);
        if (do_a) {
            if (!packed_up_front) {
                float* const wdp = (training && l > 0) ? ws + L.wp_d[l] : nullptr;
                if (q.wino || (q.wino_d && wdp))
                    SED_TRY(sed_conv3x3_wino_pack_weights(p->conv_w[l], q.wino ? ws + L.wp_f[l] : nullptr, q.wino_d ? wdp : nullptr, q.C, q.Cin, stream));
                if (!q.wino || (wdp && !q.wino_d))
                    SED_TRY(sed_conv3x3_pack_weights_ex(p->conv_w[l], q.wino ? nullptr : ws + L.wp_f[l], q.wino_d ? nullptr : wdp,
                                                        q.C, q.Cin, (l > 0) ? c->conv_mode : 0, stream));
            }
            if (q.fused) {
                if (training) SED_TRY(sed_conv1_stats(in, ws + L.wp_f[l], p->conv_b[l], ws + L.stat[l], ws + L.c1_stat_ws, B, q.Cin, q.F, q.T, q.C,
                                                      q.rgrad ? (double*)(ws + L.c1_mom) : nullptr, stream));
            } else if (q.wino) {
                SED_TRY(sed_conv3x3_wino_fwd(in, ws + L.wp_f[l], p->conv_b[l], ws + L.conv_out[l], training ? ws + L.stat[l] : nullptr,
                                             B, q.Cin, q.F, q.T, q.C, stream));
            } else {
                SED_TRY(sed_conv3x3_fwd_ex(in, q.nchw, ws + L.wp_f[l], p->conv_b[l], ws + L.conv_out[l],
                                           training ? ws + L.stat[l] : nullptr, B, q.Cin, q.F, q.T, q.C, (l > 0) ? c->conv_mode : 0, stream));
            }
            if (training && !one_shot) SED_TRY(sed_bn_stat_sums(ws + L.stat[l], q.rows, q.C, ws + L.bn_sums[l], stream));
        }
        if (!do_b) continue;
        const double count = (double)B * q.T * q.F;
        if (training && one_shot)
            SED_TRY(sed_bn_finalize_train(ws + L.stat[l], q.rows, q.C, count, p->bn_g[l], p->bn_b[l],
                                          p->bn_rm[l], p->bn_rv[l], c->bn_momentum, c->bn_eps, ws + L.mean[l],
                                          ws + L.rstd[l], ws + L.scale[l], ws + L.shift[l], stream));
        else if (training)
            SED_TRY(sed_bn_finalize_from_sums(ws + L.bn_sums[l], q.C, count * (double)count_scale, p->bn_g[l], p->bn_b[l],
                                              p->bn_rm[l], p->bn_rv[l], c->bn_momentum, c->bn_eps, ws + L.mean[l],
                                              ws + L.rstd[l], ws + L.scale[l], ws + L.shift[l], stream));
        else
            SED_TRY(sed_bn_finalize_eval(p->bn_g[l], p->bn_b[l], p->bn_rm[l], p->bn_rv[l], c->bn_eps, q.C,
                                         ws + L.scale[l], ws + L.shift[l], stream));
        const int last = (l == L.n_conv - 1);
        if (q.fused)
            SED_TRY(sed_conv1_bn_relu_pool_drop_fwd(in, ws + L.wp_f[l], p->conv_b[l], ws + L.scale[l], ws + L.shift[l],
                                                    ws + L.pooled[l], B, q.Cin, q.F, q.T, q.C, q.pf, q.pt,
                                                    training ? q.drop : 0.f, layer_seed(seed, l), seed_dev,
                                                    (training && q.rgrad) ? (unsigned char*)(ws + L.c1_bits) : nullptr, stream));
        else
            SED_TRY(sed_bn_relu_pool_drop_fwd(ws + L.conv_out[l], ws + L.scale[l], ws + L.shift[l], ws + L.pooled[l], B,
                                              q.T, q.F, q.C, q.pf, q.pt, last, training ? q.drop : 0.f,
                                              layer_seed(seed, l), seed_dev, stream));
    }
    if (pe <= 2 * L.n_conv) return 0;
    const int M = L.M;
    const float* gin = ws + L.pooled[L.n_conv - 1];
    for (int i = 0; i < L.n_gru; ++i) {
        const int H = L.gr[i].H, K = L.gr[i].in;
        for (int d = 0; d < 2; ++d)
            SED_REQUIRE(p->gru_wih[i][d] && p->gru_whh[i][d] && p->gru_bih[i][d] && p->gru_bhh[i][d],
                        "net_forward: missing parameters of GRU layer %d dir %d", i, d);
        const float* wih[2] = {p->gru_wih[i][0], p->gru_wih[i][1]};
        if (i == 0 && wih_permuted) { wih[0] = ws + L.wih_perm; wih[1] = wih[0] + (size_t)3 * H * K; }
        const bool fused = wih[1] == wih[0] + (size_t)3 * H * K && p->gru_bih[i][1] == p->gru_bih[i][0] + 3 * H;
        if (i == 0 && eval_plan && L.proj_bf) {
            const void* wb16 = (const void*)(ws + L.wih_perm);
            if (p->gru_bih[i][1] == p->gru_bih[i][0] + 3 * H) {
                SED_TRY(sed_gemm_bf16_nt(gin, wb16, p->gru_bih[i][0], ws + L.gi[i], 6 * H, M, 6 * H, K, stream));
            } else {
                for (int d = 0; d < 2; ++d)
                    SED_TRY(sed_gemm_bf16_nt(gin, (const void*)((const uint16_t*)wb16 + (size_t)d * 3 * H * K), p->gru_bih[i][d],
                                             ws + L.gi[i] + d * 3 * H, 6 * H, M, 3 * H, K, stream));
            }
        } else if (fused) {
            SED_TRY(sed_gemm_f32_ws(gin, K, 1, wih[0], 1, K, ws + L.gi[i], 6 * H, p->gru_bih[i][0], M, 6 * H, K, ws + L.gemm_ws, stream));
        } else {
            for (int d = 0; d < 2; ++d)
                SED_TRY(sed_gemm_f32(gin, K, 1, wih[d], 1, K, ws + L.gi[i] + d * 3 * H, 6 * H,
                                     p->gru_bih[i][d], 0.f, M, 3 * H, K, stream));
        }
        const float* whh[2] = {p->gru_whh[i][0], p->gru_whh[i][1]};
        const float* bhh[2] = {p->gru_bhh[i][0], p->gru_bhh[i][1]};
        SED_TRY(sed_gru_seq_fwd(ws + L.gi[i], whh, bhh, ws + L.gout[i], training ? ws + L.saved[i] : nullptr,
                                ws + L.gru_ws, B, L.Tp, H, stream));
        gin = ws + L.gout[i];
    }
    const float* din = gin;
    for (int j = 0; j < L.n_dense; ++j) {
        SED_REQUIRE(p->dense_w[j] && p->dense_b[j], "net_forward: missing parameters of dense layer %d", j);
        const int last = (j == L.n_dense - 1);
        float* y = last ? logits : ws + L.act[j];
        SED_TRY(sed_linear_fwd(din, p->dense_w[j], p->dense_b[j], y, M, L.dK[j], L.dN[j], !last, stream));
        din = y;
    }
    return 0;
}

extern "C" int sed_net_forward(const sed_net_cfg* c, const sed_net_params* p, const float* x, float* logits,
                               void* workspace, int training, uint64_t seed, const uint64_t* seed_dev, void* stream) {
    return forward_impl(c, p, x, logits, workspace, training, seed, seed_dev, 0, 2 * (c ? c->n_conv : 0) + 1, 1.f, stream);
}

extern "C" int sed_net_forward_phases(const sed_net_cfg* c, const sed_net_params* p, const float* x, float* logits,
                                      void* workspace, int training, uint64_t seed, int phase_begin, int phase_end,
                                      float count_scale, void* stream) {
    SED_REQUIRE(count_scale >= 1.f, "net_forward_phases: count_scale must be >= 1");
    SED_REQUIRE(!c || c->conv_mode != 2, "net_forward_phases: conv_mode 2 (bf16 inference) has no phases; run it with sed_net_forward, training = 0");
    return forward_impl(c, p, x, logits, workspace, training, seed, nullptr, phase_begin, phase_end, count_scale, stream);
}

extern "C" int sed_net_sync_region(const sed_net_cfg* c, int backward, int block, size_t* offset_bytes, size_t* n_floats) {
    Layout L;
    SED_TRY(build_layout(c, 1, &L));
    SED_REQUIRE(block >= 0 && block < L.n_conv && offset_bytes && n_floats, "net_sync_region: bad arguments");
    *offset_bytes = (backward ? L.sum_g : L.bn_sums[block]) * sizeof(float);
    *n_floats = (size_t)2 * L.cv[block].C;
    return 0;
}

extern "C" int sed_net_workspace_region(const sed_net_cfg* c, int training, const char* name, int index,
                                        size_t* offset_bytes, size_t* n_floats) {
    Layout L;
    SED_TRY(build_layout(c, training, &L));
    SED_REQUIRE(name && offset_bytes && n_floats, "net_workspace_region: null pointer");
    const bool conv_idx = index >= 0 && index < L.n_conv, gru_idx = index >= 0 && index < L.n_gru;
    size_t off = 0, n = 0;
    bool ok = false;
    auto is = [&](const char* q) { return strcmp(name, q) == 0; };
    if (conv_idx) {
        const ConvL& q = L.cv[index];
        const size_t nout = (size_t)c->B * q.T * q.F * q.C, npool = (size_t)c->B * q.Tp * q.Fp * q.C;
        if (is("conv_out") && !q.fused && !q.ev && !q.bf) { off = L.conv_out[index]; n = nout; ok = true; }
        else if (is("pooled")) { off = L.pooled[index]; n = npool; ok = true; }
// ... 107 lines not shown
            SED_TRY(sed_bn_relu_pool_drop_bwd_apply(ws + L.conv_out[l], ws + L.gradA, ws + L.scale[l], ws + L.shift[l],
                                                    ws + L.mean[l], ws + L.rstd[l], sum_g, sum_gx, ws + L.dconv[l],
                                                    ws + L.dbias_part, B, q.T, q.F, q.C, q.pf, q.pt, last, q.drop, sd, seed_dev, st));
            SED_TRY(sed_reduce_rows(ws + L.dbias_part, q.bn_rows, q.C, q.C, g->conv_b[l], st));
        }
    }
    return 0;
}

static int dgrad(const Layout& L, const sed_net_cfg* c, const sed_net_params* p, const float* x, float* ws, int l, void* st) {
    const ConvL& q = L.cv[l];
    const ConvL& u = L.cv[l - 1];
    if (u.rg_rows > 0 && q.wino_d)
        return sed_conv3x3_wino_dgrad_bnred_rg(ws + L.dconv[l], ws + L.wp_d[l], (u.fused && u.rgrad && u.rg_rows > 0) ? nullptr : ws + L.gradA, ws + L.bn_part, ws + L.pooled[l - 1],
                                               p->bn_g[l - 1], p->bn_b[l - 1], ws + L.mean[l - 1], ws + L.rstd[l - 1], u.drop,
                                               x, u.Cin, (const unsigned char*)(ws + L.c1_bits), ws + L.c1_ws, c->B, q.C, q.F, q.T, q.Cin, st);
    if (u.rg_rows > 0)
        return sed_conv3x3_dgrad_bnred_rg(ws + L.dconv[l], ws + L.wp_d[l], ws + L.gradA, ws + L.bn_part, ws + L.pooled[l - 1],
                                          p->bn_g[l - 1], p->bn_b[l - 1], ws + L.mean[l - 1], ws + L.rstd[l - 1], u.drop,
                                          x, u.Cin, (const unsigned char*)(ws + L.c1_bits), ws + L.c1_ws, c->B, q.C, q.F, q.T, q.Cin, st);
    if (q.wino_d)
        return sed_conv3x3_wino_dgrad_bnred(ws + L.dconv[l], ws + L.wp_d[l], ws + L.gradA, ws + L.bn_part, ws + L.pooled[l - 1],
                                            p->bn_g[l - 1], p->bn_b[l - 1], u.fused ? nullptr : ws + L.conv_out[l - 1],
                                            ws + L.mean[l - 1], ws + L.rstd[l - 1], u.drop, u.pf, u.pt, u.F, u.T, c->B, q.C, q.F, q.T, q.Cin, st);
    if (u.red_rows > 0)
        return sed_conv3x3_dgrad_bnred(ws + L.dconv[l], ws + L.wp_d[l], ws + L.gradA, ws + L.bn_part, ws + L.pooled[l - 1],
                                       p->bn_g[l - 1], p->bn_b[l - 1],
                                       u.fused ? nullptr : ws + L.conv_out[l - 1],
                                       ws + L.mean[l - 1], ws + L.rstd[l - 1],
                                       u.drop, u.pf, u.pt, u.F, u.T, c->B, q.C, q.F, q.T, q.Cin, st);
    return sed_conv3x3_fwd_ex(ws + L.dconv[l], 0, ws + L.wp_d[l], nullptr, ws + L.gradA, nullptr, c->B, q.C, q.F, q.T, q.Cin, c->conv_mode, st);
}

extern "C" int sed_net_backward(const sed_net_cfg* c, const sed_net_params* p, const sed_net_params* g,
                                const float* x, const float* dlogits, void* workspace, uint64_t seed,
                                const uint64_t* seed_dev, int stage_begin, int stage_end, void* stream, void* aux_stream) {
    SED_REQUIRE(p && g && x && dlogits && workspace, "net_backward: null pointer");
    constexpr int kMaxDev = 16;
    static thread_local hipEvent_t ev_all[kMaxDev][2][SED_MAX_CONV] = {};
    static thread_local hipEvent_t ev_gru_all[kMaxDev][SED_MAX_GRU + 5] = {};
    hipStream_t s_main = as_stream(stream), s_aux = as_stream(aux_stream);
    hipEvent_t* ev_dg = nullptr;
    hipEvent_t* ev_bn = nullptr;
    hipEvent_t* ev_gru = nullptr;
    if (s_aux && s_aux != s_main) {
        int dev = 0;
        if (hipGetDevice(&dev) != hipSuccess || dev < 0 || dev >= kMaxDev) {
            sed_set_error("net_backward: device index %d outside [0,%d)", dev, kMaxDev);
            return SED_EINVAL;
        }
        ev_dg = ev_all[dev][0];
        ev_bn = ev_all[dev][1];
        ev_gru = ev_gru_all[dev];
        for (int i = 0; i < SED_MAX_GRU + 5; ++i)
            if (!ev_gru[i] && hipEventCreateWithFlags(&ev_gru[i], hipEventDisableTiming) != hipSuccess) {
                sed_set_error("net_backward: hipEventCreate failed");
                return SED_EINVAL;
            }
        for (int l = 0; l < SED_MAX_CONV; ++l)
            if (!ev_dg[l]) {
                if (hipEventCreateWithFlags(&ev_dg[l], hipEventDisableTiming) != hipSuccess ||
                    hipEventCreateWithFlags(&ev_bn[l], hipEventDisableTiming) != hipSuccess) {
                    sed_set_error("net_backward: hipEventCreate failed");
                    return SED_EINVAL;
                }
            }
    } else {
        s_aux = nullptr;
    }
    Layout L;
    SED_TRY(build_layout(c, 1, &L));
    SED_REQUIRE(stage_begin >= 0 && stage_end <= L.n_conv + 1 && stage_begin < stage_end,
                "net_backward: bad stage range [%d,%d)", stage_begin, stage_end);
    float* ws = (float*)workspace;
    const int B = c->B, M = L.M;

    const int wg_clean = ((L.wgrad_zrow > 0 && s_aux) ? SED_WGRAD_ZERO_ROW_CLEAN : 0) | ((c->flags & SED_NET_DIRECT_CONV) ? SED_WGRAD_DIRECT : 0);
    if (s_aux && stage_begin == 0 && L.n_conv > 1) {
        hipError_t e = hipEventRecord(ev_gru[SED_MAX_GRU + 4], s_main);
        if (e == hipSuccess) e = hipStreamWaitEvent(s_aux, ev_gru[SED_MAX_GRU + 4], 0);
        if (e == hipSuccess) e = hipMemsetAsync(ws + L.wg_arrive, 0, (64 + L.wgrad_zrow) * sizeof(float), s_aux);
        if (e == hipSuccess && L.wgrad_zrow > 0) e = hipMemsetAsync(ws + L.wgrad_ws_aux, 0, L.wgrad_zrow * sizeof(float), s_aux);
        if (e == hipSuccess) e = hipEventRecord(ev_gru[SED_MAX_GRU + 3], s_aux);
        if (e != hipSuccess) {
            sed_set_error("net_backward: clearing the weight-gradient zero rows failed: %s", hipGetErrorString(e));
            return (int)e;
        }
    }

    if (stage_begin == 0) {
        const float* gru_last = ws + L.gout[L.n_gru - 1];
        for (int j = L.n_dense - 1; j >= 0; --j) {
            const int last = (j == L.n_dense - 1);
            const float* xin = (j == 0) ? gru_last : ws + L.act[j - 1];
            float* dy = last ? const_cast<float*>(dlogits) : ws + L.dact[j];
            float* dx = (j == 0) ? ws + L.dgout[L.n_gru - 1] : ws + L.dact[j - 1];
            SED_REQUIRE(g->dense_w[j] && g->dense_b[j], "net_backward: missing gradient buffers of dense layer %d", j);
            SED_TRY(sed_linear_bwd(xin, p->dense_w[j], last ? nullptr : ws + L.act[j], dy, dx, g->dense_w[j],
                                   g->dense_b[j], ws + L.lin_ws, M, L.dK[j], L.dN[j], !last, stream));
        }
        for (int i = L.n_gru - 1; i >= 0; --i) {
            const int H = L.gr[i].H, K = L.gr[i].in;
            const float* xin = (i == 0) ? ws + L.pooled[L.n_conv - 1] : ws + L.gout[i - 1];
            float* dxin = (i == 0) ? ws + L.gradA : ws + L.dgout[i - 1];
            const float* whh[2] = {p->gru_whh[i][0], p->gru_whh[i][1]};
            float* dgi = ws + L.dgi[i];
            float* dgh = ws + L.dgh[i];
            for (int d = 0; d < 2; ++d)
                SED_REQUIRE(g->gru_wih[i][d] && g->gru_whh[i][d] && g->gru_bih[i][d] && g->gru_bhh[i][d],
                            "net_backward: missing gradient buffers of GRU layer %d dir %d", i, d);
            float* dbih[2] = {g->gru_bih[i][0], g->gru_bih[i][1]};
            float* dbhh[2] = {g->gru_bhh[i][0], g->gru_bhh[i][1]};
            SED_TRY(sed_gru_seq_bwd(ws + L.dgout[i], ws + L.saved[i], whh, dgi, dgh, dbih, dbhh, ws + L.gru_bws, B, L.Tp, H, stream));
            const bool on_aux = s_aux && i > 0;
            void* wst = on_aux ? aux_stream : stream;
            float* wws = ws + (on_aux ? L.gemm_ws_aux : L.gemm_ws);
            if (on_aux) {
                (void)hipEventRecord(ev_gru[i], s_main);
                (void)hipStreamWaitEvent(s_aux, ev_gru[i], 0);
            }
            auto dw_hh = [&]() -> int {
                for (int d = 0; d < 2; ++d)
                    SED_TRY(sed_gemm_f32_wgrad(dgh + d * 3 * H, 1, 6 * H, ws + L.saved[i] + ((size_t)d * 5 + 4) * H, 10 * H, 1,
                                               g->gru_whh[i][d], H, 3 * H, H, M, wws, wst));
                return 0;
            };
            if (on_aux || !s_aux) SED_TRY(dw_hh());
            const bool fused = p->gru_wih[i][1] == p->gru_wih[i][0] + (size_t)3 * H * K &&
                               g->gru_wih[i][1] == g->gru_wih[i][0] + (size_t)3 * H * K;
            auto dw_ih = [&](void* st, float* gws) -> int {
                if (fused)
                    return sed_gemm_f32_wgrad(dgi, 1, 6 * H, xin, K, 1, g->gru_wih[i][0], K, 6 * H, K, M, gws, st);
                for (int d = 0; d < 2; ++d)
                    SED_TRY(sed_gemm_f32(dgi + d * 3 * H, 1, 6 * H, xin, K, 1, g->gru_wih[i][d], K, nullptr, 0.f, 3 * H, K, M, st));
                return 0;
            };
            if (on_aux) SED_TRY(dw_ih(aux_stream, wws));
            if (i == 0 && s_aux) (void)hipEventRecord(ev_gru[SED_MAX_GRU], s_aux);
            if (fused) {
                SED_TRY(sed_gemm_f32(dgi, 6 * H, 1, p->gru_wih[i][0], K, 1, dxin, K, nullptr, 0.f, M, K, 6 * H, stream));
            } else {
                for (int d = 0; d < 2; ++d)
                    SED_TRY(sed_gemm_f32(dgi + d * 3 * H, 6 * H, 1, p->gru_wih[i][d], K, 1, dxin, K, nullptr, d ? 1.f : 0.f,
                                         M, K, 3 * H, stream));
            }
            if (i == 0 && s_aux) {
                const int top = L.n_conv - 1;
                (void)hipEventRecord(ev_dg[top], s_main);
                (void)hipStreamWaitEvent(s_aux, ev_dg[top], 0);
                SED_TRY(bn_backward(L, c, p, g, x, ws, seed, seed_dev, top, 3, 1.f, aux_stream));
                (void)hipEventRecord(ev_bn[top], s_aux);
            }
            if (!on_aux) SED_TRY(dw_ih(stream, ws + L.gemm_ws));
            if (s_aux && i == 0) SED_TRY(dw_hh());
        }
        if (s_aux) (void)hipStreamWaitEvent(s_main, ev_gru[SED_MAX_GRU], 0);
    }
    auto bn_passes = [&](int l, void* st) -> int { return bn_backward(L, c, p, g, x, ws, seed, seed_dev, l, 3, 1.f, st); };
    auto wgrad_on = [&](int l, void* st) -> int {
        const ConvL& q = L.cv[l];
        const float* xin = (l == 0) ? x : ws + L.pooled[l - 1];
        float* scratch = ws + ((l == 0 && L.n_conv > 1) ? L.c1_ws : L.wgrad_ws);
        return sed_conv3x3_wgrad_ex(xin, q.nchw, ws + L.dconv[l], g->conv_w[l], scratch, B, q.Cin, q.F, q.T, q.C, (l > 0) ? (c->conv_mode | wg_clean) : 0, st);
    };
    auto wgrad = [&](int l) -> int { return wgrad_on(l, stream); };
    const bool wg0_with_bn = L.n_conv > 1 && !L.cv[0].fused;
    const int top = L.n_conv - 1;
    const bool top_wgrad_on_aux = s_aux && top > 1 && (c->flags & SED_NET_DIRECT_CONV);
    const bool top_wgrad_in_stage = s_aux && top > 1 && !top_wgrad_on_aux;
    for (int s = (stage_begin > 1 ? stage_begin : 1); s < stage_end; ++s) {
        const int l = L.n_conv - s;
        const ConvL& q = L.cv[l];
        if (l == top) {
            if (s_aux) (void)hipStreamWaitEvent(s_main, ev_bn[top], 0);
            else SED_TRY(bn_passes(top, stream));
        } else if (l == 0 && s_aux) {
            (void)hipStreamWaitEvent(s_main, ev_bn[0], 0);
        }
        if (l == 0) {
            if (!q.fused && !wg0_with_bn) SED_TRY(wgrad(0));
            continue;
        }
        if (s_aux) (void)hipStreamWaitEvent(s_main, ev_gru[SED_MAX_GRU + 3], 0);
        SED_TRY(dgrad(L, c, p, x, ws, l, stream));
        if (l > 1) {
            if (top_wgrad_on_aux && l == top) {
                (void)hipEventRecord(ev_gru[SED_MAX_GRU + 1], s_main);
// ... 37 lines not shown
            SED_TRY(bn_passes(0, stream));
            if (wg0_with_bn) SED_TRY(wgrad_on(0, stream));
            SED_TRY(main_wgrads());
            (void)hipEventRecord(ev_bn[0], s_main);
        } else if (s_aux) {
            const bool fin_on_main = L.cv[0].red_rows > 0;
            if (fin_on_main) SED_TRY(bn_backward(L, c, p, g, x, ws, seed, seed_dev, 0, 1, 1.f, stream));
            (void)hipEventRecord(ev_dg[0], s_main);
            auto aux_chain = [&]() -> int {
                (void)hipStreamWaitEvent(s_aux, ev_dg[0], 0);
                SED_TRY(sed_internal_stream_gate(arrive, gate_target, 2000, aux_stream));
                SED_TRY(bn_backward(L, c, p, g, x, ws, seed, seed_dev, 0, fin_on_main ? 2 : 3, 1.f, aux_stream));
                if (wg0_with_bn) SED_TRY(wgrad_on(0, aux_stream));
                (void)hipEventRecord(ev_bn[0], s_aux);
                return 0;
            };
            if (c->flags & SED_NET_AUX_FIRST) {
                SED_TRY(aux_chain());
                SED_TRY(main_wgrads());
            } else {
                SED_TRY(main_wgrads());
                SED_TRY(aux_chain());
            }
        } else {
            SED_TRY(bn_passes(0, stream));
            if (wg0_with_bn) SED_TRY(wgrad_on(0, stream));
            SED_TRY(main_wgrads());
        }
        if (top_wgrad_on_aux) (void)hipStreamWaitEvent(s_main, ev_gru[SED_MAX_GRU + 2], 0);
    }
    return 0;
}

extern "C" int sed_net_backward_ready_stage(const sed_net_cfg* c, int block) {
    if (!c || block < 0 || block >= c->n_conv) { sed_set_error("net_backward_ready_stage: bad arguments"); return SED_EINVAL; }
    return block == 0 ? c->n_conv : c->n_conv - 1;
}

extern "C" int sed_net_backward_phases(const sed_net_cfg* c, const sed_net_params* p, const sed_net_params* g,
                                       const float* x, const float* dlogits, void* workspace, uint64_t seed,
                                       int phase_begin, int phase_end, float count_scale, void* stream) {
    SED_REQUIRE(p && g && x && dlogits && workspace, "net_backward_phases: null pointer");
    SED_REQUIRE(count_scale >= 1.f, "net_backward_phases: count_scale must be >= 1");
    Layout L;
    SED_TRY(build_layout(c, 1, &L));
    SED_REQUIRE(phase_begin >= 0 && phase_end <= 2 * L.n_conv + 1 && phase_begin < phase_end,
                "net_backward_phases: bad phase range [%d,%d)", phase_begin, phase_end);
    float* ws = (float*)workspace;
    const int B = c->B;
    if (phase_begin == 0) SED_TRY(sed_net_backward(c, p, g, x, dlogits, workspace, seed, nullptr, 0, 1, stream, nullptr));
    for (int ph = (phase_begin > 1 ? phase_begin : 1); ph < phase_end; ++ph) {
        const int k = (ph - 1) >> 1, l = L.n_conv - 1 - k;
        const ConvL& q = L.cv[l];
        if (ph & 1) {
            SED_TRY(bn_backward(L, c, p, g, x, ws, seed, nullptr, l, 1, 1.f, stream));
            continue;
        }
        SED_TRY(bn_backward(L, c, p, g, x, ws, seed, nullptr, l, 2, count_scale, stream));
        if (q.fused) continue;
        const float* xin = (l == 0) ? x : ws + L.pooled[l - 1];
        SED_TRY(sed_conv3x3_wgrad_ex(xin, q.nchw, ws + L.dconv[l], g->conv_w[l], ws + ((l == 0 && L.n_conv > 1) ? L.c1_ws : L.wgrad_ws),
                                     B, q.Cin, q.F, q.T, q.C, (l > 0) ? c->conv_mode : 0, stream));
        if (l > 0) SED_TRY(dgrad(L, c, p, x, ws, l, stream));
    }
    return 0;
}
// ... 1 lines not shown
```

### sed_crnn_amd/model.py

```python
import ctypes as C
import math
import weakref

import torch
import torch.nn as nn

from . import _lib
from ._lib import NetCfg, NetParams, check, lib

_MASK64 = (1 << 64) - 1
_ARENA_OWNERS = weakref.WeakValueDictionary()


def arena_owner(param):
    try:
        m = _ARENA_OWNERS.get(param.untyped_storage().data_ptr())
    except Exception:
        return None
    if m is not None and any(q is param for q in m._arena_params):
        return m
    return None


class ConvParams(nn.Module):
# ... 104 lines not shown
class HipCRNN(nn.Module):

    def _init_spec(self, *, in_channels, n_mels, conv_channels, pools, drops, gru_hidden, dense, bn_eps=1e-5,
                   bn_momentum=0.1):
        if not (1 <= len(conv_channels) == len(pools) == len(drops) <= _lib.SED_MAX_CONV):
            raise ValueError(f"1..{_lib.SED_MAX_CONV} conv blocks with one pool and one dropout rate each, got "
                             f"{len(conv_channels)}/{len(pools)}/{len(drops)}")
        if not (1 <= len(gru_hidden) <= _lib.SED_MAX_GRU and 1 <= len(dense) <= _lib.SED_MAX_DENSE):
            raise ValueError(f"1..{_lib.SED_MAX_GRU} GRU layers and 1..{_lib.SED_MAX_DENSE} dense layers, got "
                             f"{len(gru_hidden)} and {len(dense)}")
        bad = [c for c in conv_channels if c <= 0 or c % 4 or c > 1024]
        if bad:
            raise ValueError(f"conv channel counts must be multiples of 4 up to 1024 (float4 channel vectors), got {bad}")
        bad = [h for h in gru_hidden if h <= 0 or h % 4 or 3 * h > 1024]
        if bad:
            raise ValueError(f"GRU hidden sizes must be multiples of 4 up to 340 (the recurrence keeps 3H gate columns per "
                             f"workgroup), got {bad}")
        if any(not (0.0 <= d < 1.0) for d in drops):
            raise ValueError(f"dropout rates must lie in [0, 1), got {list(drops)}")
        if in_channels < 1 or n_mels < 1 or any(pf < 1 or pt < 1 for pf, pt in pools):
            raise ValueError("in_channels, n_mels and the pool sizes must be positive")
        self.in_channels, self.n_mels = in_channels, n_mels
        self.conv_channels = list(conv_channels)
        self.pools = [tuple(p) for p in pools]
        self.drops = list(drops)
        self.gru_hidden, self.dense = list(gru_hidden), list(dense)
        self.bn_eps, self.bn_momentum = bn_eps, bn_momentum
        f = n_mels
        for pf, _ in self.pools:
            f //= pf
        self.flat_features = conv_channels[-1] * f
        self.time_factor = math.prod(pt for _, pt in self.pools)
        self._last = None
        self.overlap_wgrad = True
        self._sync_bn, self._sync_group = False, None
        self._aux_stream = None
        self._ticket = 0
        self._bound_grads = False
        self._arena_dirty = False
        self._ws_pinned = set()
        self._seed_counter = 0
        self._nbt_pending = 0
        self._ws = {}
        self._structs = None
        self._arena = None

    def _roles(self):
        raise NotImplementedError

    def _flatten(self):
        r = self._roles()
        order = []
        for j in range(len(self.dense)):
            order += [r["dense_w"][j], r["dense_b"][j]]
        for i in range(len(self.gru_hidden)):
            for role in ("gru_wih", "gru_whh", "gru_bih", "gru_bhh"):
                order += [r[role][i][0], r[role][i][1]]
        stage_ends = []
        off = 0
        offs = []
        nconv = len(self.conv_channels)

        def place(ps):
            nonlocal off
            for p in ps:
                offs.append(off)
# ... 7 lines not shown
            stage_ends.append(off)
        dev = order[0].device
        flat = torch.zeros(off, device=dev, dtype=torch.float32)
        flat_g = torch.zeros(off, device=dev, dtype=torch.float32)
        views = []
        with torch.no_grad():
            for p, o in zip(order, offs):
                n = p.numel()
                flat[o:o + n].copy_(p.detach().reshape(-1))
                p.data = flat[o:o + n].view(p.shape)
                views.append(flat_g[o:o + n].view(p.shape))
                p.grad = None
        assert len(order) == len(list(self.parameters())), "every parameter must have a role"
        self._arena, self._arena_grad = flat, flat_g
        _ARENA_OWNERS[flat.untyped_storage().data_ptr()] = self
        self._arena_params, self._grad_views, self._arena_offsets = order, views, offs
        self._stage_ends = stage_ends
        self._structs = None
        self._ws = {}
        self._ws_pinned = set()
        self._arena_dirty = False
        self._last = None
        if self._bound_grads:
            self.bind_flat_grads()

    def _apply(self, fn, *a, **k):
        super()._apply(fn, *a, **k)
        if hasattr(self, "_arena_params"):
            self._flatten()
        return self

    def __getstate__(self):
        st = self.__dict__.copy()
        for k in ("_structs", "_ws", "_aux_stream", "_last", "_arena", "_arena_grad", "_arena_params", "_grad_views",
                  "_arena_offsets", "_stage_ends"):
            st.pop(k, None)
        return st

    def __setstate__(self, st):
        self.__dict__.update(st)
        self._structs, self._ws, self._aux_stream, self._arena = None, {}, None, None
        with torch.no_grad():
            for p_ in self.parameters():
                p_.data = p_.data.clone()
        self._flatten()

    def flat_parameters(self):
        return self._arena

    def flat_grads(self):
        return self._arena_grad

    def bucket_slices(self):
        b = [0] + self._stage_ends
        n = len(self.conv_channels)
        cfg = self._cfg(1, self.time_factor)
        ready = [lib().sed_net_backward_ready_stage(C.byref(cfg), n - s) for s in range(1, n + 1)]
        out = [(b[0], b[1])]
        for st in range(1, n + 1):
            mine = [s for s in range(1, n + 1) if ready[s - 1] == st]
            out.append((b[mine[0]], b[mine[-1] + 1]) if mine else (b[st], b[st]))
        return out

    def bind_flat_grads(self):
        self._bound_grads = True
        for p, g in zip(self._arena_params, self._grad_views):
            p.grad = g if p.requires_grad else None
# ... 153 lines not shown
        return ws[off.value // 4: off.value // 4 + n.value]

    def eval_workspace_view(self, name, index=0):
        if getattr(self, "_last_eval", None) is None:
            raise RuntimeError("sed_crnn_amd: no eval forward to look into")
        cfg, ws = self._last_eval
        off, n = C.c_size_t(), C.c_size_t()
        check(lib().sed_net_workspace_region(C.byref(cfg), 0, name.encode(), int(index), C.byref(off), C.byref(n)),
              "sed_net_workspace_region")
        bf16 = False
        if name == "pooled" and cfg.conv_mode == 2:
            cb, pj = (C.c_int * _lib.SED_MAX_CONV)(), C.c_int(0)
            check(lib().sed_net_inference_plan(C.byref(cfg), cb, C.byref(pj)), "sed_net_inference_plan")
            bf16 = bool(cb[int(index)])
        o = off.value // 4
        if bf16:
            return ws[o: o + (n.value + 1) // 2].view(torch.bfloat16)[:n.value]
        return ws[o: o + n.value]

    def routing(self, block):
        if self._last is None:
            raise RuntimeError("sed_crnn_amd: no training forward to look into")
        cfg, ws, x = self._last
        P, _ = self._param_structs()
        T, F = cfg.T, cfg.F
        for l in range(block):
            T, F = T // self.pools[l][1], F // self.pools[l][0]
        pf, pt = self.pools[block]
        route = torch.empty(cfg.B, T // pt, F // pf, self.conv_channels[block], device=x.device, dtype=torch.uint8)
        check(lib().sed_net_routing(C.byref(cfg), C.byref(P), _lib.ptr(x), _lib.ptr(ws), int(block), _lib.ptr(route),
                                    _lib.stream_ptr()), "sed_net_routing")
        return route

    def _run_forward(self, x, training, step_state=None):
        self._check_input(x)
        x = x.detach().contiguous().float()
        B, _, _, T = x.shape
        cfg = self._cfg(B, T, training)
        P, _ = self._param_structs()
        ws = self._workspace(cfg, training)
        if not training:
            self._last_eval = (cfg, ws)
        logits = torch.empty(B, T // self.time_factor, self.dense[-1], device=x.device, dtype=torch.float32)
        if training:
            self._ticket += 1
            self._seed = self._next_seed() if step_state is None else self._graph_seed()
            self._nbt_pending += 1
            self._last = (cfg, ws, x)
            self._last_state = step_state
        seed = self._seed if training else 0
        world = self._sync_world() if training else 1
        if world > 1:
            args = (C.byref(cfg), C.byref(P), _lib.ptr(x), _lib.ptr(logits), _lib.ptr(ws), 1, seed)
            n = len(self.conv_channels)
            for l in range(n):
                check(lib().sed_net_forward_phases(*args, 2 * l, 2 * l + 1, float(world), _lib.stream_ptr()), "sed_net_forward_phases")
                self._allreduce_region(cfg, ws, 0, l)
                check(lib().sed_net_forward_phases(*args, 2 * l + 1, 2 * l + 2, float(world), _lib.stream_ptr()), "sed_net_forward_phases")
            check(lib().sed_net_forward_phases(*args, 2 * n, 2 * n + 1, float(world), _lib.stream_ptr()), "sed_net_forward_phases")
            return logits
        check(lib().sed_net_forward(C.byref(cfg), C.byref(P), _lib.ptr(x), _lib.ptr(logits), _lib.ptr(ws),
                                    int(training), seed, _lib.ptr(step_state) if training else None, _lib.stream_ptr()),
              "sed_net_forward")
        return logits

    def _run_backward(self, x, dlogits, stage_begin=0, stage_end=None):
        if self._last is None:
            raise RuntimeError("sed_crnn_amd: backward without a training forward (or its workspace was evicted)")
        cfg, ws, x = self._last
        P, G = self._param_structs()
        if stage_end is None:
            stage_end = len(self.conv_channels) + 1
        world = self._sync_world()
        if world > 1:
            args = (C.byref(cfg), C.byref(P), C.byref(G), _lib.ptr(x), _lib.ptr(dlogits), _lib.ptr(ws), self._seed)
            n = len(self.conv_channels)
            for s in range(stage_begin, stage_end):
                if s == 0:
                    check(lib().sed_net_backward_phases(*args, 0, 1, float(world), _lib.stream_ptr()), "sed_net_backward_phases")
                    continue
                k = s - 1
                check(lib().sed_net_backward_phases(*args, 2 * k + 1, 2 * k + 2, float(world), _lib.stream_ptr()), "sed_net_backward_phases")
                self._allreduce_region(cfg, ws, 1, n - 1 - k)
                check(lib().sed_net_backward_phases(*args, 2 * k + 2, 2 * k + 3, float(world), _lib.stream_ptr()), "sed_net_backward_phases")
            return
        if getattr(self, "_aux_stream", None) is None or self._aux_stream.device != x.device:
            self._aux_stream = torch.cuda.Stream(device=x.device)
        aux = C.c_void_p(self._aux_stream.cuda_stream) if self.overlap_wgrad else None
        check(lib().sed_net_backward(C.byref(cfg), C.byref(P), C.byref(G), _lib.ptr(x), _lib.ptr(dlogits),
                                     _lib.ptr(ws), self._seed, _lib.ptr(getattr(self, "_last_state", None)), stage_begin,
                                     stage_end, _lib.stream_ptr(), aux), "sed_net_backward")

    def forward(self, x):
        if self.training and torch.is_grad_enabled():
            return _NetFn.apply(self, x, *self._arena_params)
        return self._run_forward(x, training=self.training)

    def _flush_nbt(self):
        if self._nbt_pending:
            for m in self.modules():
                if isinstance(m, BNParams):
                    m.num_batches_tracked += self._nbt_pending
            self._nbt_pending = 0

    def state_dict(self, *a, **k):
        self._flush_nbt()
        return super().state_dict(*a, **k)

    def load_state_dict(self, sd, *a, **k):
        self._nbt_pending = 0
        out = super().load_state_dict(sd, *a, **k)
        return out


class TimePooledCRNN(HipCRNN):

    def __init__(self, conv_channels=128, dropout=0.5, *, in_channels=1, n_mels=40, time_pool=(2, 2, 2),
                 gru_hidden=32, gru_layers=2, n_classes=1):
        super().__init__()
        n = len(time_pool)
        self._init_spec(in_channels=in_channels, n_mels=n_mels, conv_channels=[conv_channels] * n,
# ... 123 lines not shown
```

### sed_crnn_amd/ops.py

```python
import ctypes as C

import torch

from ._lib import check, lib, ptr, stream_ptr


def _f32c(t):
    assert t.is_cuda and t.dtype == torch.float32 and t.is_contiguous(), "expect contiguous fp32 CUDA tensor"
    return t


def conv3x3_pack(w, mode=0):
    Cout, Cin = w.shape[:2]
    wf = torch.empty(9, Cout, Cin, device=w.device)
    wd = torch.empty(9, Cin, Cout, device=w.device)
    check(lib().sed_conv3x3_pack_weights_ex(ptr(_f32c(w)), ptr(wf), ptr(wd), Cout, Cin, mode, stream_ptr()), "conv3x3_pack")
    return wf, wd


def conv3x3_fwd(x, wp, bias, x_is_nchw, want_stats=True, mode=0):
    if x_is_nchw:
        B, Cin, F, T = x.shape
    else:
        B, T, F, Cin = x.shape
# ... 261 lines not shown
    dgh = torch.empty(B, T, 2, 3 * H, device=dout.device)
    if not want_bias:
        check(lib().sed_gru_seq_bwd(ptr(_f32c(dout)), ptr(saved), _pp(whh), ptr(dgi), ptr(dgh), None, None, None,
                                    B, T, H, stream_ptr()), "gru_seq_bwd")
        return dgi, dgh
    dbih = [torch.empty(3 * H, device=dout.device) for _ in range(2)]
    dbhh = [torch.empty(3 * H, device=dout.device) for _ in range(2)]
    ws = torch.empty(lib().sed_gru_seq_bwd_workspace_bytes(B, H) // 4 + 1, device=dout.device)
    check(lib().sed_gru_seq_bwd(ptr(_f32c(dout)), ptr(saved), _pp(whh), ptr(dgi), ptr(dgh), _pp(dbih), _pp(dbhh),
                                ptr(ws), B, T, H, stream_ptr()), "gru_seq_bwd")
    return dgi, dgh, dbih, dbhh


def gru_seq_variant(B, H):
    bt, hreg, hlds = C.c_int(), C.c_int(), C.c_int()
    check(lib().sed_gru_seq_variant(B, H, C.byref(bt), C.byref(hreg), C.byref(hlds)), "gru_seq_variant")
    return bt.value, hreg.value, hlds.value


def loss_fwd_bwd(logits, targets, kind="bce", alpha=0.25, gamma=2.0, reduction="mean"):
    if kind not in ("bce", "focal"):
        raise ValueError(f"loss kind must be 'bce' or 'focal', got {kind!r}")
    if reduction not in ("mean", "sum"):
        raise ValueError(f"reduction must be 'mean' or 'sum' (the fused loss returns a scalar), got {reduction!r}")
    if logits.shape != targets.shape:
        raise ValueError(f"logits {tuple(logits.shape)} and targets {tuple(targets.shape)} differ in shape")
    n = logits.numel()
    loss = torch.empty(1, device=logits.device)
    d = torch.empty_like(logits)
    p = torch.empty_like(logits)
    check(lib().sed_loss_fwd_bwd(ptr(_f32c(logits)), ptr(_f32c(targets)), n, 0 if kind == "bce" else 1, alpha, gamma,
                                 int(reduction == "mean"), ptr(loss), ptr(d), ptr(p), stream_ptr()), "loss_fwd_bwd")
    return loss, d, p


def sigmoid(x):
    y = torch.empty_like(x)
    check(lib().sed_sigmoid(ptr(_f32c(x)), ptr(y), x.numel(), stream_ptr()), "sigmoid")
    return y


def grad_norm_clip_coef(g, max_norm):
    out = torch.empty(2, device=g.device)
    ws = torch.empty(lib().sed_sqnorm_workspace_bytes(g.numel()) // 4, device=g.device)
    check(lib().sed_grad_norm_clip_coef(ptr(g), g.numel(), float(max_norm), ptr(out), ptr(ws), stream_ptr()), "grad_norm")
    return out


def adam_step(p, g, m, v, lr, beta1, beta2, eps, weight_decay, step, grad_scale=None, step_state=None):
    check(lib().sed_adam_step(ptr(p), ptr(g), ptr(m), ptr(v), p.numel(), lr, beta1, beta2, eps, weight_decay, step,
                              ptr(grad_scale), ptr(step_state), stream_ptr()), "adam_step")


def conv1_fused_block(x, w, bias, gamma, beta, pool_f, pool_t, dout=None, drop_p=0.0, seed=0, eps=1e-5, moments_path=False):
    B, Cin, F, T = x.shape
    Cc = w.shape[0]
    L = lib()
    assert L.sed_conv1_fused_supported(Cin, F, T, Cc, pool_f, pool_t) or (moments_path and L.sed_conv1_rgrad_supported(Cin, F, T, Cc, pool_f, pool_t))
    wf, _ = conv3x3_pack(w)
    rows = L.sed_conv1_fused_rows(B, T)
    stat = torch.empty(1, 2, Cc, device=x.device)
    sws = torch.empty(L.sed_conv1_stats_workspace_bytes(B, Cin, T) // 4 + 1, device=x.device)
    mom = torch.empty(L.sed_conv1_moments_doubles(Cin), device=x.device, dtype=torch.float64) if moments_path else None
    check(L.sed_conv1_stats(ptr(_f32c(x)), ptr(wf), ptr(bias), ptr(stat), ptr(sws), B, Cin, F, T, Cc, ptr(mom), stream_ptr()), "conv1_stats")
    rm, rv = torch.zeros(Cc, device=x.device), torch.ones(Cc, device=x.device)
    mean, rstd, scale, shift = bn_finalize_train(stat, B * T * F, gamma, beta, rm, rv, eps=eps)
# ... 30 lines not shown
```

### sed_crnn_amd/trainer.py

```python
import torch

from . import ops
from .dist import BucketedAllReduce


class FusedTrainStep:
    def __init__(self, model, lr=1e-3, betas=(0.9, 0.999), eps=1e-8, weight_decay=0.0, loss="bce",
                 focal_alpha=0.25, focal_gamma=2.0, clip_norm=None, process_group=None, distributed=None, graph=False):
        self.model = model
        self.lr, self.betas, self.eps, self.wd = lr, betas, eps, weight_decay
        self.loss_kind, self.alpha, self.gamma = loss, focal_alpha, focal_gamma
        self.clip_norm = clip_norm
        self.t = 0
        p = self._p = model.flat_parameters()
        self.m, self.v = torch.zeros_like(p), torch.zeros_like(p)
        if distributed is None:
            distributed = torch.distributed.is_available() and torch.distributed.is_initialized() \
                and torch.distributed.get_world_size(process_group) > 1
        self.reducer = BucketedAllReduce(model.flat_grads(), model.bucket_slices(), process_group) if distributed else None
        self.graph = bool(graph) and self.reducer is None
        self._graphs = {}
        self._state = torch.zeros(2, dtype=torch.int64, device=p.device) if self.graph else None
        self.time_allreduce = False
        self.allreduce_events = []
# ... 4 lines not shown
                               "created; its Adam moments, captured graphs and all-reduce buckets point at the old ones")
        if self.graph:
            return self._step_graph(x, y)
        return self._step_eager(x, y)

    def _step_graph(self, x, y):
        key = (tuple(x.shape), tuple(y.shape))
        ent = self._graphs.get(key)
        if ent is None:
            self._graphs[key] = "warm"
            return self._step_eager(x, y.float(), state=self._state)
        if ent == "warm":
            sx, sy = x.clone(), y.clone().float()
            torch.cuda.synchronize()
            g = torch.cuda.CUDAGraph()
            with torch.cuda.graph(g):
                out = self._step_eager(sx, sy, state=self._state)
            self.t -= 1
            self.model.pin_workspace(sx.shape[0], sx.shape[3], True)
            ent = self._graphs[key] = (g, sx, sy, out, self.model._last[1])
        g, sx, sy, out, _ws = ent
        sx.copy_(x)
        sy.copy_(y)
        g.replay()
        self.t += 1
        return out

    def _step_eager(self, x, y, state=None):
        m = self.model
        m.train()
        if state is not None:
            from ._lib import check, lib, ptr, stream_ptr
            check(lib().sed_step_advance(ptr(state), stream_ptr()), "sed_step_advance")
        logits = m._run_forward(x, training=True, step_state=state)
        loss, dlogits, probs = ops.loss_fwd_bwd(logits, y, self.loss_kind, self.alpha, self.gamma, "mean")
        nstage = len(m.conv_channels) + 1
        if self.reducer is None:
            m._run_backward(x, dlogits, 0, nstage)
        else:
            for s in range(nstage):
                m._run_backward(x, dlogits, s, s + 1)
                self.reducer.launch(s)
            if self.time_allreduce and x.is_cuda:
                e0, e1 = torch.cuda.Event(enable_timing=True), torch.cuda.Event(enable_timing=True)
                e0.record()
                self.reducer.wait_all()
                e1.record()
                self.allreduce_events.append((e0, e1))
            else:
                self.reducer.wait_all()
        g = m.flat_grads()
        coef = ops.grad_norm_clip_coef(g, self.clip_norm)[1:2] if self.clip_norm else None
        self.t += 1
        ops.adam_step(m.flat_parameters(), g, self.m, self.v, self.lr, self.betas[0], self.betas[1], self.eps,
                      self.wd, self.t, coef, step_state=state)
        return loss, probs
```

Measured before the change: 5.923 million mel-frames/s.

## Fuse head linear with loss, conv1 stats with BN finalize, and pack GRU weights

```diff
diff --git a/include/sedcrnn.h b/include/sedcrnn.h
--- a/include/sedcrnn.h
+++ b/include/sedcrnn.h
@@ -128,6 +128,10 @@
 size_t sed_conv1_moments_doubles(int Cin);
 int sed_conv1_stats(const float* x, const float* wp, const float* bias, float* stat_partials, void* workspace,
                     int B, int Cin, int F, int T, int C, double* moments, void* stream);
+int sed_conv1_stats_bn_finalize(const float* x, const float* wp, const float* bias, float* stat_partials, void* workspace,
+                                int B, int Cin, int F, int T, int C, double* moments, const float* gamma, const float* beta,
+                                float* running_mean, float* running_var, float momentum, float eps, float* mean, float* rstd,
+                                float* scale, float* shift, void* stream);
 int sed_conv1_bn_relu_pool_drop_fwd(const float* x, const float* wp, const float* bias, const float* scale,
                                     const float* shift, float* out, int B, int Cin, int F, int T, int C,
                                     int pool_f, int pool_t, float drop_p, uint64_t seed, const uint64_t* seed_dev,
@@ -174,14 +178,27 @@
 size_t sed_linear_bwd_workspace_bytes(int M, int K, int N);
 int sed_linear_bwd(const float* x, const float* W, const float* y, float* dy, float* dx,
                    float* dW, float* db, void* workspace, int M, int K, int N, int relu, void* stream);
+size_t sed_head_loss_workspace_bytes(int M, int K);
+int sed_head_loss_rows(const float* x, const float* W, const float* b, const float* targets, int M, int K, int kind,
+                       float alpha, float gamma, float* logits, float* dlogits, float* probs, float* dx,
+                       void* workspace, void* stream);
+int sed_head_loss_finish(const void* workspace, int M, int K, float* loss, float* dW, float* db, void* stream);
+int sed_head_loss_fwd_bwd(const float* x, const float* W, const float* b, const float* targets, int M, int K, int kind,
+                          float alpha, float gamma, float* logits, float* loss, float* dlogits, float* probs, float* dx,
+                          float* dW, float* db, void* workspace, void* stream);
 
 size_t sed_gru_seq_workspace_bytes(int H);
 int sed_gru_seq_fwd(const float* gi, const float* const* whh, const float* const* bhh,
                     float* out, float* saved, void* workspace, int B, int T, int H, void* stream);
+int sed_gru_seq_fwd_packed(const float* gi, const float* whh_t, const float* const* bhh,
+                           float* out, float* saved, int B, int T, int H, void* stream);
 size_t sed_gru_seq_bwd_workspace_bytes(int B, int H);
 int sed_gru_seq_bwd(const float* dout, const float* saved, const float* const* whh,
                     float* dgi, float* dgh, float* const* dbih, float* const* dbhh, void* workspace,
                     int B, int T, int H, void* stream);
+int sed_gru_seq_bwd_partials(const float* dout, const float* saved, const float* const* whh,
+                             float* dgi, float* dgh, void* workspace, int B, int T, int H, void* stream);
+int sed_gru_bias_grad(const void* workspace, float* const* dbih, float* const* dbhh, int B, int H, void* stream);
 int sed_gru_seq_variant(int B, int H, int* bt, int* hreg, int* hlds);
 
 int sed_loss_fwd_bwd(const float* logits, const float* targets, int n, int kind, float alpha,
@@ -306,6 +323,10 @@
 #define SED_NET_AUX_FIRST 0x1
 #define SED_NET_NO_GATE 0x2
 #define SED_NET_DIRECT_CONV 0x4
+#define SED_NET_UNFUSED_TAIL 0x8
+#define SED_NET_UNFUSED_PACK 0x10
+#define SED_NET_UNFUSED_BIAS 0x20
+#define SED_NET_UNFUSED_FIN 0x40
 
 typedef struct sed_net_params {
     float* conv_w[SED_MAX_CONV];
@@ -329,6 +350,13 @@
 int sed_net_backward(const sed_net_cfg* cfg, const sed_net_params* p, const sed_net_params* g,
                      const float* x, const float* dlogits, void* workspace, uint64_t seed, const uint64_t* seed_dev,
                      int stage_begin, int stage_end, void* stream, void* aux_stream);
+int sed_net_forward_body(const sed_net_cfg* cfg, const sed_net_params* p, const float* x, void* workspace,
+                         uint64_t seed, const uint64_t* seed_dev, void* stream);
+int sed_net_head_loss_rows(const sed_net_cfg* cfg, const sed_net_params* p, const float* targets, int kind, float alpha,
+                           float gamma, float* logits, float* dlogits, float* probs, void* workspace, void* stream);
+int sed_net_backward_fused_head(const sed_net_cfg* cfg, const sed_net_params* p, const sed_net_params* g,
+                                const float* x, float* loss, void* workspace, uint64_t seed, const uint64_t* seed_dev,
+                                int stage_begin, int stage_end, void* stream, void* aux_stream);
 int sed_net_backward_ready_stage(const sed_net_cfg* cfg, int block);
 
 int sed_net_sync_region(const sed_net_cfg* cfg, int backward, int block, size_t* offset_bytes, size_t* n_floats);
diff --git a/sed_crnn_amd/_lib.py b/sed_crnn_amd/_lib.py
--- a/sed_crnn_amd/_lib.py
+++ b/sed_crnn_amd/_lib.py
@@ -82,6 +82,7 @@
     "sed_conv1_stats_workspace_bytes": (_sz, [_i, _i, _i]),
     "sed_conv1_moments_doubles": (_sz, [_i]),
     "sed_conv1_stats": (_i, [_fp, _fp, _fp, _fp, _fp, _i, _i, _i, _i, _i, _fp, _stream]),
+    "sed_conv1_stats_bn_finalize": (_i, [_fp, _fp, _fp, _fp, _fp, _i, _i, _i, _i, _i, _fp, _fp, _fp, _fp, _fp, _f, _f, _fp, _fp, _fp, _fp, _stream]),
     "sed_conv1_bn_relu_pool_drop_fwd": (_i, [_fp, _fp, _fp, _fp, _fp, _fp, _i, _i, _i, _i, _i, _i, _i, _f, _u64, _fp, _fp, _stream]),
     "sed_conv1_rgrad_supported": (_i, [_i, _i, _i, _i, _i, _i]),
     "sed_conv1_bwd_wgrad_workspace_bytes": (_sz, [_i, _i, _i, _i]),
@@ -113,10 +114,17 @@
     "sed_linear_fwd": (_i, [_fp, _fp, _fp, _fp, _i, _i, _i, _i, _stream]),
     "sed_linear_bwd_workspace_bytes": (_sz, [_i, _i, _i]),
     "sed_linear_bwd": (_i, [_fp, _fp, _fp, _fp, _fp, _fp, _fp, _fp, _i, _i, _i, _i, _stream]),
+    "sed_head_loss_workspace_bytes": (_sz, [_i, _i]),
+    "sed_head_loss_rows": (_i, [_fp, _fp, _fp, _fp, _i, _i, _i, _f, _f, _fp, _fp, _fp, _fp, _fp, _stream]),
+    "sed_head_loss_finish": (_i, [_fp, _i, _i, _fp, _fp, _fp, _stream]),
+    "sed_head_loss_fwd_bwd": (_i, [_fp, _fp, _fp, _fp, _i, _i, _i, _f, _f, _fp, _fp, _fp, _fp, _fp, _fp, _fp, _fp, _stream]),
     "sed_gru_seq_workspace_bytes": (_sz, [_i]),
     "sed_gru_seq_fwd": (_i, [_fp, _pp, _pp, _fp, _fp, _fp, _i, _i, _i, _stream]),
     "sed_gru_seq_bwd_workspace_bytes": (_sz, [_i, _i]),
     "sed_gru_seq_bwd": (_i, [_fp, _fp, _pp, _fp, _fp, _pp, _pp, _fp, _i, _i, _i, _stream]),
+    "sed_gru_seq_fwd_packed": (_i, [_fp, _fp, _pp, _fp, _fp, _i, _i, _i, _stream]),
+    "sed_gru_seq_bwd_partials": (_i, [_fp, _fp, _pp, _fp, _fp, _fp, _i, _i, _i, _stream]),
+    "sed_gru_bias_grad": (_i, [_fp, _pp, _pp, _i, _i, _stream]),
     "sed_gru_seq_variant": (_i, [_i, _i, C.POINTER(_i), C.POINTER(_i), C.POINTER(_i)]),
     "sed_loss_fwd_bwd": (_i, [_fp, _fp, _i, _i, _f, _f, _i, _fp, _fp, _fp, _stream]),
     "sed_sigmoid": (_i, [_fp, _fp, _i, _stream]),
@@ -177,6 +185,9 @@
     "sed_net_workspace_region": (_i, [C.POINTER(NetCfg), _i, C.c_char_p, _i, C.POINTER(_sz), C.POINTER(_sz)]),
     "sed_net_routing": (_i, [C.POINTER(NetCfg), C.POINTER(NetParams), _fp, _fp, _i, _fp, _stream]),
     "sed_net_inference_plan": (_i, [C.POINTER(NetCfg), C.POINTER(C.c_int), C.POINTER(C.c_int)]),
+    "sed_net_forward_body": (_i, [C.POINTER(NetCfg), C.POINTER(NetParams), _fp, _fp, _u64, _fp, _stream]),
+    "sed_net_head_loss_rows": (_i, [C.POINTER(NetCfg), C.POINTER(NetParams), _fp, _i, _f, _f, _fp, _fp, _fp, _fp, _stream]),
+    "sed_net_backward_fused_head": (_i, [C.POINTER(NetCfg), C.POINTER(NetParams), C.POINTER(NetParams), _fp, _fp, _fp, _u64, _fp, _i, _i, _stream, _stream]),
     "sed_net_forward_phases": (_i, [C.POINTER(NetCfg), C.POINTER(NetParams), _fp, _fp, _fp, _i, _u64, _i, _i, _f, _stream]),
     "sed_net_backward_phases": (_i, [C.POINTER(NetCfg), C.POINTER(NetParams), C.POINTER(NetParams), _fp, _fp, _fp, _u64, _i, _i, _f, _stream]),
     "sed_net_backward": (_i, [C.POINTER(NetCfg), C.POINTER(NetParams), C.POINTER(NetParams), _fp, _fp, _fp, _u64, _fp, _i, _i, _stream, _stream]),
diff --git a/sed_crnn_amd/csrc/bnpool.hip b/sed_crnn_amd/csrc/bnpool.hip
--- a/sed_crnn_amd/csrc/bnpool.hip
+++ b/sed_crnn_amd/csrc/bnpool.hip
@@ -35,21 +35,7 @@
     double A, Q;
     bn_two_channel_sums(part, rows, C, c, c < C, sred, &A, &Q);
     if (threadIdx.x < 2 && c < C) {
-        double m = A / count;
-        double var = Q / count - m * m;
-        if (var < 0.0) var = 0.0;
-        float rstd = (float)(1.0 / sqrt(var + (double)eps));
-        float g = gamma[c], bt = beta[c];
-        mean_o[c] = (float)m;
-        rstd_o[c] = rstd;
-        float sc = g * rstd;
-        scale_o[c] = sc;
-        shift_o[c] = bt - (float)m * sc;
-        if (rmean) {
-            double unb = count > 1.0 ? var * count / (count - 1.0) : var;
-            rmean[c] = (1.f - momentum) * rmean[c] + momentum * (float)m;
-            rvar[c] = (1.f - momentum) * rvar[c] + momentum * (float)unb;
-        }
+        sed_bn_train_coeffs(A, Q, count, c, gamma, beta, rmean, rvar, momentum, eps, mean_o, rstd_o, scale_o, shift_o);
     }
 }
 
diff --git a/sed_crnn_amd/csrc/common.h b/sed_crnn_amd/csrc/common.h
--- a/sed_crnn_amd/csrc/common.h
+++ b/sed_crnn_amd/csrc/common.h
@@ -44,7 +44,8 @@
 };
 
 int sed_internal_conv_pack_multi(int n, const float* const* w, float* const* wf, float* const* wd, const int* Cout, const int* Cin,
-                                 const int* wino_f, const int* wino_d, void* stream);
+                                 const int* wino_f, const int* wino_d, int n_gru, const float* const* gru_whh, float* const* gru_wt,
+                                 const int* gru_H, void* stream);
 
 int sed_internal_conv_pack_eval(int n, const float* const* w, const float* const* bias, const float* const* gamma,
                                 const float* const* beta, const float* const* rm, const float* const* rv, float eps,
@@ -97,4 +98,46 @@
     return v;
 }
 __device__ __forceinline__ float sigmoidf_(float x) { return 1.0f / (1.0f + __expf(-x)); }
+
+__device__ __forceinline__ void sed_loss_elem(float xi, float ti, int kind, float alpha, float gamma, float* l_out, float* d_out, float* p_out) {
+    float p = 1.f / (1.f + expf(-xi));
+    float l, d;
+    if (kind == 0) {
+        l = fmaxf(xi, 0.f) - xi * ti + log1pf(expf(-fabsf(xi)));
+        d = p - ti;
+    } else {
+        bool pos = (ti == 1.f);
+        float pt = pos ? p : 1.f - p;
+        float om = 1.f - pt;
+        float lg = logf(pt + 1e-12f);
+        float pw = powf(om, gamma);
+        l = -alpha * pw * lg;
+        float dpw = (gamma == 0.f) ? 0.f : gamma * powf(om, gamma - 1.f);
+        float dl_dpt = -alpha * (-dpw * lg + pw / (pt + 1e-12f));
+        float dpt_dx = pos ? p * (1.f - p) : -p * (1.f - p);
+        d = dl_dpt * dpt_dx;
+    }
+    *l_out = l; *d_out = d; *p_out = p;
+}
+
+__device__ __forceinline__ void sed_bn_train_coeffs(double A, double Q, double count, int c, const float* __restrict__ gamma,
+                                                    const float* __restrict__ beta, float* __restrict__ rmean, float* __restrict__ rvar,
+                                                    float momentum, float eps, float* __restrict__ mean_o, float* __restrict__ rstd_o,
+                                                    float* __restrict__ scale_o, float* __restrict__ shift_o) {
+    double m = A / count;
+    double var = Q / count - m * m;
+    if (var < 0.0) var = 0.0;
+    float rstd = (float)(1.0 / sqrt(var + (double)eps));
+    float g = gamma[c], bt = beta[c];
+    mean_o[c] = (float)m;
+    rstd_o[c] = rstd;
+    float sc = g * rstd;
+    scale_o[c] = sc;
+    shift_o[c] = bt - (float)m * sc;
+    if (rmean) {
+        double unb = count > 1.0 ? var * count / (count - 1.0) : var;
+        rmean[c] = (1.f - momentum) * rmean[c] + momentum * (float)m;
+        rvar[c] = (1.f - momentum) * rvar[c] + momentum * (float)unb;
+    }
+}
 #endif
diff --git a/sed_crnn_amd/csrc/conv.hip b/sed_crnn_amd/csrc/conv.hip
--- a/sed_crnn_amd/csrc/conv.hip
+++ b/sed_crnn_amd/csrc/conv.hip
@@ -118,10 +118,20 @@
     int wino_f[SED_MAX_CONV], wino_d[SED_MAX_CONV];
     const float* perm_src[2]; float* perm_dst; int perm_rows, perm_C, perm_Fp;
     __bf16* wb[SED_MAX_CONV]; int perm_bf16;
+    int n_gru; const float* gru_w[SED_MAX_GRU][2]; float* gru_wt[SED_MAX_GRU]; int gru_H[SED_MAX_GRU];
 };
 __global__ void conv_pack_w_multi_k(ConvPackMulti a, int n) {
     const int l = blockIdx.y;
     const int i = blockIdx.x * blockDim.x + threadIdx.x;
+    if (a.n_gru > 0 && l >= n) {
+        const int g = l - n, H = a.gru_H[g], nw = 3 * H * H;
+        for (int e2 = i; e2 < 2 * nw; e2 += gridDim.x * blockDim.x) {
+            const int dir = e2 / nw, e = e2 - dir * nw;
+            const int r = e / H, k = e - r * H;
+            a.gru_wt[g][(size_t)dir * nw + (size_t)k * 3 * H + r] = a.gru_w[g][dir][e];
+        }
+        return;
+    }
     if (l == n) {
         extern __shared__ __attribute__((aligned(16))) float prow[];
         const int K = a.perm_C * a.perm_Fp;
@@ -172,14 +182,22 @@
     const size_t lds = a.perm_src[0] ? (size_t)a.perm_C * a.perm_Fp * sizeof(float) : 0;
     SED_REQUIRE(lds <= 64 * 1024, "conv_pack: a GRU input row of %zu bytes does not fit the re-ordering buffer", lds);
     if (lds > 48 * 1024) SED_TRY(set_lds_early(lds));
-    conv_pack_w_multi_k<<<dim3(gx, n + (a.perm_src[0] ? 1 : 0)), 256, lds, as_stream(stream)>>>(a, n);
+    SED_REQUIRE(!(a.perm_src[0] && a.n_gru > 0), "conv_pack: the permutation and the GRU slices exclude each other");
+    conv_pack_w_multi_k<<<dim3(gx, n + (a.perm_src[0] ? 1 : 0) + a.n_gru), 256, lds, as_stream(stream)>>>(a, n);
     SED_LAUNCH_CHECK("conv_pack_w_multi");
     return 0;
 }
 int sed_internal_conv_pack_multi(int n, const float* const* w, float* const* wf, float* const* wd, const int* Cout, const int* Cin,
-                                 const int* wino_f, const int* wino_d, void* stream) {
+                                 const int* wino_f, const int* wino_d, int n_gru, const float* const* gru_whh, float* const* gru_wt,
+                                 const int* gru_H, void* stream) {
     SED_REQUIRE(n > 0 && n <= SED_MAX_CONV && w && wf && wd && Cout && Cin, "conv_pack_multi: bad arguments");
+    SED_REQUIRE(n_gru >= 0 && n_gru <= SED_MAX_GRU && (n_gru == 0 || (gru_whh && gru_wt && gru_H)), "conv_pack_multi: bad GRU arguments");
     ConvPackMulti a{};
+    a.n_gru = n_gru;
+    for (int g = 0; g < n_gru; ++g) {
+        SED_REQUIRE(gru_whh[2 * g] && gru_whh[2 * g + 1] && gru_wt[g] && gru_H[g] > 0, "conv_pack_multi: bad GRU layer %d", g);
+        a.gru_w[g][0] = gru_whh[2 * g]; a.gru_w[g][1] = gru_whh[2 * g + 1]; a.gru_wt[g] = gru_wt[g]; a.gru_H[g] = gru_H[g];
+    }
     for (int l = 0; l < n; ++l) {
         SED_REQUIRE(w[l] && Cout[l] > 0 && Cin[l] > 0, "conv_pack_multi: bad layer %d", l);
         a.w[l] = w[l]; a.wf[l] = wf[l]; a.wd[l] = wd[l]; a.Cout[l] = Cout[l]; a.Cin[l] = Cin[l];
diff --git a/sed_crnn_amd/csrc/conv1.hip b/sed_crnn_amd/csrc/conv1.hip
--- a/sed_crnn_amd/csrc/conv1.hip
+++ b/sed_crnn_amd/csrc/conv1.hip
@@ -341,13 +341,13 @@
         partials[(size_t)blockIdx.x * NG + i] = (red[i * 4] + red[i * 4 + 1]) + (red[i * 4 + 2] + red[i * 4 + 3]);
 }
 
-template <int CIN>
-__global__ __launch_bounds__(256) void conv1_gram_finalize_k(const float* __restrict__ partials, int nblk, const float* __restrict__ wp,
-                                                             const float* __restrict__ bias, double count, int C, float* __restrict__ stat,
-                                                             double* __restrict__ gram_out) {
+struct Conv1BnFin { const float* gamma; const float* beta; float* rmean; float* rvar; float momentum, eps;
+                    float* mean_o; float* rstd_o; float* scale_o; float* shift_o; };
+template <int CIN, bool BN>
+__device__ __forceinline__ void conv1_gram_finalize_body(const float* __restrict__ partials, int nblk, const float* __restrict__ wp,
+                                                         const float* __restrict__ bias, double count, int C, float* __restrict__ stat,
+                                                         double* __restrict__ gram_out, const Conv1BnFin& bn, double* G, double (*Gq)[64]) {
     constexpr int NK = 9 * CIN, NG = NK + NK * (NK + 1) / 2;
-    __shared__ double G[NG];
-    __shared__ double Gq[4][64];
     {
         const int il = threadIdx.x & 63, q = threadIdx.x >> 6;
         for (int i0 = 0; i0 < NG; i0 += 64) {
@@ -379,9 +379,33 @@
 #pragma unroll
             for (int k2 = k; k2 < NK; ++k2) { q += (k2 == k ? 1.0 : 2.0) * w[k] * w[k2] * G[g]; ++g; }
         }
-        stat[c] = (float)(count * b + ws1);
-        stat[C + c] = (float)(q + 2.0 * b * ws1 + count * b * b);
-    }
+        const float s1 = (float)(count * b + ws1), s2 = (float)(q + 2.0 * b * ws1 + count * b * b);
+        stat[c] = s1;
+        stat[C + c] = s2;
+        if (BN) {
+            double A = 0.0, Q = 0.0;
+            A += (double)s1; Q += (double)s2;
+            sed_bn_train_coeffs(A, Q, count, c, bn.gamma, bn.beta, bn.rmean, bn.rvar, bn.momentum, bn.eps, bn.mean_o, bn.rstd_o, bn.scale_o, bn.shift_o);
+        }
+    }
+}
+template <int CIN>
+__global__ __launch_bounds__(256) void conv1_gram_finalize_k(const float* __restrict__ partials, int nblk, const float* __restrict__ wp,
+                                                             const float* __restrict__ bias, double count, int C, float* __restrict__ stat,
+                                                             double* __restrict__ gram_out) {
+    constexpr int NK = 9 * CIN, NG = NK + NK * (NK + 1) / 2;
+    __shared__ double G[NG];
+    __shared__ double Gq[4][64];
+    conv1_gram_finalize_body<CIN, false>(partials, nblk, wp, bias, count, C, stat, gram_out, Conv1BnFin{}, G, Gq);
+}
+template <int CIN>
+__global__ __launch_bounds__(256) void conv1_gram_bn_finalize_k(const float* __restrict__ partials, int nblk, const float* __restrict__ wp,
+                                                                const float* __restrict__ bias, double count, int C, float* __restrict__ stat,
+                                                                double* __restrict__ gram_out, Conv1BnFin bn) {
+    constexpr int NK = 9 * CIN, NG = NK + NK * (NK + 1) / 2;
+    __shared__ double G[NG];
+    __shared__ double Gq[4][64];
+    conv1_gram_finalize_body<CIN, true>(partials, nblk, wp, bias, count, C, stat, gram_out, bn, G, Gq);
 }
 
 #define C1_MM_BLOCKS 1024
@@ -836,8 +860,8 @@
     return (size_t)256 * (nk + nk * (nk + 1) / 2) * sizeof(float);
 }
 
-extern "C" int sed_conv1_stats(const float* x, const float* wp, const float* bias, float* stat_partials, void* workspace,
-                               int B, int Cin, int F, int T, int C, double* gram_out, void* stream) {
+static int conv1_stats_impl(const float* x, const float* wp, const float* bias, float* stat_partials, void* workspace,
+                            int B, int Cin, int F, int T, int C, double* gram_out, const Conv1BnFin* bn, void* stream) {
     SED_REQUIRE(x && wp && stat_partials && workspace, "conv1_stats: null pointer");
     SED_REQUIRE(c1_shape_ok(Cin, F, T, C, 1, 1, 4), "conv1_stats: shape Cin=%d F=%d T=%d C=%d is not supported", Cin, F, T, C);
     hipStream_t s = as_stream(stream);
@@ -879,14 +903,34 @@
     if (Cin == 1) {
         conv1_gram_k<1><<<grid, 256, lds, s>>>(x, (float*)workspace, B, F, T);
         SED_LAUNCH_CHECK("conv1_gram");
-        conv1_gram_finalize_k<1><<<1, 256, 0, s>>>((const float*)workspace, grid, wp, bias, count, C, stat_partials, gram_out);
+        if (bn) conv1_gram_bn_finalize_k<1><<<1, 256, 0, s>>>((const float*)workspace, grid, wp, bias, count, C, stat_partials, gram_out, *bn);
+        else conv1_gram_finalize_k<1><<<1, 256, 0, s>>>((const float*)workspace, grid, wp, bias, count, C, stat_partials, gram_out);
     } else {
         conv1_gram_k<2><<<grid, 256, lds, s>>>(x, (float*)workspace, B, F, T);
         SED_LAUNCH_CHECK("conv1_gram");
-        conv1_gram_finalize_k<2><<<1, 256, 0, s>>>((const float*)workspace, grid, wp, bias, count, C, stat_partials, gram_out);
+        if (bn) conv1_gram_bn_finalize_k<2><<<1, 256, 0, s>>>((const float*)workspace, grid, wp, bias, count, C, stat_partials, gram_out, *bn);
+        else conv1_gram_finalize_k<2><<<1, 256, 0, s>>>((const float*)workspace, grid, wp, bias, count, C, stat_partials, gram_out);
     }
     SED_LAUNCH_CHECK("conv1_gram_finalize");
     return 0;
+}
+
+extern "C" int sed_conv1_stats(const float* x, const float* wp, const float* bias, float* stat_partials, void* workspace,
+                               int B, int Cin, int F, int T, int C, double* gram_out, void* stream) {
+    return conv1_stats_impl(x, wp, bias, stat_partials, workspace, B, Cin, F, T, C, gram_out, nullptr, stream);
+}
+
+extern "C" int sed_conv1_stats_bn_finalize(const float* x, const float* wp, const float* bias, float* stat_partials, void* workspace,
+                                           int B, int Cin, int F, int T, int C, double* gram_out, const float* gamma, const float* beta,
+                                           float* rmean, float* rvar, float momentum, float eps, float* mean, float* rstd,
+                                           float* scale, float* shift, void* stream) {
+    SED_REQUIRE(gamma && beta && mean && rstd && scale && shift, "conv1_stats_bn_finalize: null pointer");
+    if (Cin > 2) {
+        SED_TRY(conv1_stats_impl(x, wp, bias, stat_partials, workspace, B, Cin, F, T, C, gram_out, nullptr, stream));
+        return sed_bn_finalize_train(stat_partials, 1, C, (double)B * T * F, gamma, beta, rmean, rvar, momentum, eps, mean, rstd, scale, shift, stream);
+    }
+    const Conv1BnFin bn{gamma, beta, rmean, rvar, momentum, eps, mean, rstd, scale, shift};
+    return conv1_stats_impl(x, wp, bias, stat_partials, workspace, B, Cin, F, T, C, gram_out, &bn, stream);
 }
 
 extern "C" int sed_conv1_bn_relu_pool_drop_fwd(const float* x, const float* wp, const float* bias, const float* scale,
diff --git a/sed_crnn_amd/csrc/gemm.hip b/sed_crnn_amd/csrc/gemm.hip
--- a/sed_crnn_amd/csrc/gemm.hip
+++ b/sed_crnn_amd/csrc/gemm.hip
@@ -449,3 +449,121 @@
     SED_LAUNCH_CHECK("linear_dw_reduce");
     return 0;
 }
+
+__global__ __launch_bounds__(256) void head_loss_rows_k(const float* __restrict__ x, const float* __restrict__ W,
+                                                        const float* __restrict__ b, const float* __restrict__ t, int M, int K,
+                                                        int kind, float alpha, float gamma, float scale, float* __restrict__ logits,
+                                                        float* __restrict__ terms, float* __restrict__ dlogits, float* __restrict__ probs,
+                                                        float* __restrict__ dx, float* __restrict__ part) {
+    __shared__ float sum_s[LIN_CHUNK];
+    const int lane = threadIdx.x & 63, wave = threadIdx.x >> 6;
+    const int m_lo = blockIdx.x * LIN_CHUNK, rows = (M - m_lo < LIN_CHUNK) ? M - m_lo : LIN_CHUNK;
+    const float* xr = x + (size_t)m_lo * K;
+    {
+        float a[LIN_CHUNK / 4];
+#pragma unroll
+        for (int j = 0; j < LIN_CHUNK / 4; ++j) a[j] = 0.f;
+        for (int k = lane; k < K; k += 64) {
+            const float w = W[k];
+#pragma unroll
+            for (int j = 0; j < LIN_CHUNK / 4; ++j) {
+                const int r = wave + 4 * j;
+                const float xv = xr[(r < rows ? r : 0) * K + k];
+                a[j] = fmaf(xv, w, a[j]);
+            }
+        }
+#pragma unroll
+        for (int j = 0; j < LIN_CHUNK / 4; ++j) {
+            const float s = wave_sum(a[j]);
+            if (lane == 0) sum_s[wave + 4 * j] = s;
+        }
+    }
+    __syncthreads();
+    if (threadIdx.x < rows) {
+        const int m = m_lo + threadIdx.x;
+        float xi = sum_s[threadIdx.x];
+        xi += b ? b[0] : 0.f;
+        float l, d, p;
+        sed_loss_elem(xi, t[m], kind, alpha, gamma, &l, &d, &p);
+        const float dl = d * scale;
+        logits[m] = xi; terms[m] = l; dlogits[m] = dl; probs[m] = p;
+        sum_s[threadIdx.x] = dl;
+    }
+    __syncthreads();
+    for (int i = threadIdx.x; i < rows * K; i += 256) {
+        const int r = i / K, k = i - r * K;
+        dx[(size_t)m_lo * K + i] = fmaf(sum_s[r], W[k], 0.f);
+    }
+    const int tot = K + 1;
+    for (int i = threadIdx.x; i < tot; i += 256) {
+        float acc = 0.f;
+        if (i < K) {
+#pragma unroll 16
+            for (int r = 0; r < rows; ++r) acc = fmaf(sum_s[r], xr[r * K + i], acc);
+        } else {
+            for (int r = 0; r < rows; ++r) acc += sum_s[r];
+        }
+        part[(size_t)blockIdx.x * tot + i] = acc;
+    }
+}
+
+__global__ __launch_bounds__(1024) void head_loss_finish_k(const float* __restrict__ terms, int n, float scale, float* __restrict__ loss,
+                                                           const float* __restrict__ part, int chunks, int K,
+                                                           float* __restrict__ dW, float* __restrict__ db) {
+    if (blockIdx.x == 0) {
+        __shared__ double red[16];
+        double acc = 0.0;
+        for (int i = threadIdx.x; i < n; i += 1024) acc += (double)terms[i];
+        acc = wave_sum_d(acc);
+        if ((threadIdx.x & 63) == 0) red[threadIdx.x >> 6] = acc;
+        __syncthreads();
+        if (threadIdx.x == 0) {
+            double a = 0.0;
+            for (int w = 0; w < 16; ++w) a += red[w];
+            loss[0] = (float)(a * (double)scale);
+        }
+        return;
+    }
+    const int tot = K + 1, i = (blockIdx.x - 1) * 1024 + threadIdx.x;
+    if (i >= tot) return;
+    double a = 0.0;
+#pragma unroll 8
+    for (int c = 0; c < chunks; ++c) a += (double)part[(size_t)c * tot + i];
+    if (i < K) dW[i] = (float)a;
+    else if (db) db[0] = (float)a;
+}
+
+extern "C" size_t sed_head_loss_workspace_bytes(int M, int K) {
+    return sed_linear_bwd_workspace_bytes(M, K, 1) + (size_t)(M > 0 ? M : 0) * sizeof(float);
+}
+
+extern "C" int sed_head_loss_rows(const float* x, const float* W, const float* b, const float* targets, int M, int K, int kind,
+                                  float alpha, float gamma, float* logits, float* dlogits, float* probs, float* dx,
+                                  void* workspace, void* stream) {
+    SED_REQUIRE(x && W && targets && logits && dlogits && probs && dx && workspace && M > 0 && K > 0, "head_loss_rows: bad arguments");
+    SED_REQUIRE(kind == 0 || kind == 1, "head_loss_rows: kind must be 0 (bce) or 1 (focal)");
+    const int chunks = cdiv(M, LIN_CHUNK);
+    float* part = (float*)workspace;
+    float* terms = part + (size_t)chunks * (K + 1);
+    head_loss_rows_k<<<chunks, 256, 0, as_stream(stream)>>>(x, W, b, targets, M, K, kind, alpha, gamma, 1.f / (float)M, logits, terms,
+                                                            dlogits, probs, dx, part);
+    SED_LAUNCH_CHECK("head_loss_rows");
+    return 0;
+}
+
+extern "C" int sed_head_loss_finish(const void* workspace, int M, int K, float* loss, float* dW, float* db, void* stream) {
+    SED_REQUIRE(workspace && loss && dW && M > 0 && K > 0, "head_loss_finish: bad arguments");
+    const int chunks = cdiv(M, LIN_CHUNK);
+    const float* part = (const float*)workspace;
+    const float* terms = part + (size_t)chunks * (K + 1);
+    head_loss_finish_k<<<1 + cdiv(K + 1, 1024), 1024, 0, as_stream(stream)>>>(terms, M, 1.f / (float)M, loss, part, chunks, K, dW, db);
+    SED_LAUNCH_CHECK("head_loss_finish");
+    return 0;
+}
+
+extern "C" int sed_head_loss_fwd_bwd(const float* x, const float* W, const float* b, const float* targets, int M, int K, int kind,
+                                     float alpha, float gamma, float* logits, float* loss, float* dlogits, float* probs, float* dx,
+                                     float* dW, float* db, void* workspace, void* stream) {
+    SED_TRY(sed_head_loss_rows(x, W, b, targets, M, K, kind, alpha, gamma, logits, dlogits, probs, dx, workspace, stream));
+    return sed_head_loss_finish(workspace, M, K, loss, dW, db, stream);
+}
diff --git a/sed_crnn_amd/csrc/gru.hip b/sed_crnn_amd/csrc/gru.hip
--- a/sed_crnn_amd/csrc/gru.hip
+++ b/sed_crnn_amd/csrc/gru.hip
@@ -329,6 +329,22 @@
         default: GRU_BT3(0, KERNEL, __VA_ARGS__); break;                                      \
     }
 
+static int gru_seq_fwd_launch(const float* gi, const float* wt, const float* bhh0, const float* bhh1, float* out, float* saved,
+                              int B, int T, int H, hipStream_t s) {
+    const GruVariant v = gru_variant(H, B, GRU_HR_FWD);
+    dim3 grid(cdiv(B, v.bt), 2);
+    int nt = gru_threads(H);
+    size_t lds = (size_t)v.bt * 4 * H * sizeof(float);
+    SedProfScope prof(SED_K_GRU_FWD, s, 2.0 * 2 * B * (double)T * 3 * H * H);
+    if (v.hlds > 0)
+        (void)hipFuncSetAttribute((const void*)gru_seq_fwd_k<GRU_HR_FWD, 1, 256, GRU_HL>, hipFuncAttributeMaxDynamicSharedMemorySize, 160 * 1024);
+#define GRU_HRX GRU_HR_FWD
+    GRU_DISPATCH(gru_seq_fwd_k, gi, wt, bhh0, bhh1, out, saved, B, T, H);
+#undef GRU_HRX
+    SED_LAUNCH_CHECK("gru_seq_fwd");
+    return 0;
+}
+
 extern "C" int sed_gru_seq_fwd(const float* gi, const float* const* whh, const float* const* bhh, float* out,
                                float* saved, void* workspace, int B, int T, int H, void* stream) {
     SED_REQUIRE(gi && whh && bhh && out && workspace && whh[0] && whh[1] && bhh[0] && bhh[1], "gru_seq_fwd: null pointer");
@@ -338,31 +354,22 @@
     int n = 2 * 3 * H * H;
     gru_pack_whh_t_k<<<cdiv(n, 256), 256, 0, s>>>(whh[0], whh[1], wt, H);
     SED_LAUNCH_CHECK("gru_pack_whh_t");
-    const GruVariant v = gru_variant(H, B, GRU_HR_FWD);
-    dim3 grid(cdiv(B, v.bt), 2);
-    int nt = gru_threads(H);
-    size_t lds = (size_t)v.bt * 4 * H * sizeof(float);
-    SedProfScope prof(SED_K_GRU_FWD, s, 2.0 * 2 * B * (double)T * 3 * H * H);
-    if (v.hlds > 0)
-        (void)hipFuncSetAttribute((const void*)gru_seq_fwd_k<GRU_HR_FWD, 1, 256, GRU_HL>, hipFuncAttributeMaxDynamicSharedMemorySize, 160 * 1024);
-#define GRU_HRX GRU_HR_FWD
-    GRU_DISPATCH(gru_seq_fwd_k, gi, wt, bhh[0], bhh[1], out, saved, B, T, H);
-#undef GRU_HRX
-    SED_LAUNCH_CHECK("gru_seq_fwd");
-    return 0;
+    return gru_seq_fwd_launch(gi, wt, bhh[0], bhh[1], out, saved, B, T, H, s);
+}
+
+extern "C" int sed_gru_seq_fwd_packed(const float* gi, const float* whh_t, const float* const* bhh, float* out,
+                                      float* saved, int B, int T, int H, void* stream) {
+    SED_REQUIRE(gi && whh_t && bhh && out && bhh[0] && bhh[1], "gru_seq_fwd_packed: null pointer");
+    SED_REQUIRE(B > 0 && T > 0 && H > 0 && H % 4 == 0 && 3 * H <= 1024, "gru_seq_fwd_packed: H=%d must be a multiple of 4 and <= 341", H);
+    return gru_seq_fwd_launch(gi, whh_t, bhh[0], bhh[1], out, saved, B, T, H, as_stream(stream));
 }
 
 extern "C" size_t sed_gru_seq_bwd_workspace_bytes(int B, int H) { return (size_t)cdiv(B, gru_bt(H, B)) * 2 * 4 * H * sizeof(float); }
 
-extern "C" int sed_gru_seq_bwd(const float* dout, const float* saved, const float* const* whh, float* dgi,
-                               float* dgh, float* const* dbih, float* const* dbhh, void* workspace, int B, int T,
-                               int H, void* stream) {
+static int gru_seq_bwd_launch(const float* dout, const float* saved, const float* const* whh, float* dgi, float* dgh, float* bpart,
+                              int B, int T, int H, hipStream_t s) {
     SED_REQUIRE(dout && saved && whh && whh[0] && whh[1] && dgi && dgh, "gru_seq_bwd: null pointer");
-    const bool want_bias = dbih && dbhh;
-    SED_REQUIRE(!want_bias || (workspace && dbih[0] && dbih[1] && dbhh[0] && dbhh[1]), "gru_seq_bwd: bias gradients need all four outputs and a workspace");
-    float* bpart = want_bias ? (float*)workspace : nullptr;
     SED_REQUIRE(B > 0 && T > 0 && H > 0 && H % 4 == 0 && 3 * H <= 1024, "gru_seq_bwd: H=%d must be a multiple of 4 and <= 341", H);
-    hipStream_t s = as_stream(stream);
     const GruVariant v = gru_variant(H, B, GRU_HR);
     dim3 grid(cdiv(B, v.bt), 2);
     int nt = gru_threads(H);
@@ -374,9 +381,29 @@
     GRU_DISPATCH(gru_seq_bwd_k, dout, saved, whh[0], whh[1], dgi, dgh, bpart, B, T, H);
 #undef GRU_HRX
     SED_LAUNCH_CHECK("gru_seq_bwd");
-    if (want_bias) {
-        gru_bias_grad_k<<<cdiv(8 * H, 256), 256, 0, s>>>(bpart, cdiv(B, v.bt), H, dbih[0], dbih[1], dbhh[0], dbhh[1]);
-        SED_LAUNCH_CHECK("gru_bias_grad");
-    }
     return 0;
 }
+
+extern "C" int sed_gru_bias_grad(const void* workspace, float* const* dbih, float* const* dbhh, int B, int H, void* stream) {
+    SED_REQUIRE(workspace && dbih && dbhh && dbih[0] && dbih[1] && dbhh[0] && dbhh[1], "gru_bias_grad: null pointer");
+    SED_REQUIRE(B > 0 && H > 0 && H % 4 == 0 && 3 * H <= 1024, "gru_bias_grad: H=%d must be a multiple of 4 and <= 341", H);
+    gru_bias_grad_k<<<cdiv(8 * H, 256), 256, 0, as_stream(stream)>>>((const float*)workspace, cdiv(B, gru_bt(H, B)), H, dbih[0], dbih[1], dbhh[0], dbhh[1]);
+    SED_LAUNCH_CHECK("gru_bias_grad");
+    return 0;
+}
+
+extern "C" int sed_gru_seq_bwd_partials(const float* dout, const float* saved, const float* const* whh, float* dgi,
+                                        float* dgh, void* workspace, int B, int T, int H, void* stream) {
+    SED_REQUIRE(workspace, "gru_seq_bwd_partials: null workspace");
+    return gru_seq_bwd_launch(dout, saved, whh, dgi, dgh, (float*)workspace, B, T, H, as_stream(stream));
+}
+
+extern "C" int sed_gru_seq_bwd(const float* dout, const float* saved, const float* const* whh, float* dgi,
+                               float* dgh, float* const* dbih, float* const* dbhh, void* workspace, int B, int T,
+                               int H, void* stream) {
+    const bool want_bias = dbih && dbhh;
+    SED_REQUIRE(!want_bias || (workspace && dbih[0] && dbih[1] && dbhh[0] && dbhh[1]), "gru_seq_bwd: bias gradients need all four outputs and a workspace");
+    SED_TRY(gru_seq_bwd_launch(dout, saved, whh, dgi, dgh, want_bias ? (float*)workspace : nullptr, B, T, H, as_stream(stream)));
+    if (want_bias) SED_TRY(sed_gru_bias_grad(workspace, dbih, dbhh, B, H, stream));
+    return 0;
+}
diff --git a/sed_crnn_amd/csrc/misc.hip b/sed_crnn_amd/csrc/misc.hip
--- a/sed_crnn_amd/csrc/misc.hip
+++ b/sed_crnn_amd/csrc/misc.hip
@@ -8,23 +8,8 @@
     double acc = 0.0;
     for (int i = threadIdx.x; i < n; i += 1024) {
         float xi = x[i], ti = t[i];
-        float p = 1.f / (1.f + expf(-xi));
-        float l, d;
-        if (kind == 0) {
-            l = fmaxf(xi, 0.f) - xi * ti + log1pf(expf(-fabsf(xi)));
-            d = p - ti;
-        } else {
-            bool pos = (ti == 1.f);
-            float pt = pos ? p : 1.f - p;
-            float om = 1.f - pt;
-            float lg = logf(pt + 1e-12f);
-            float pw = powf(om, gamma);
-            l = -alpha * pw * lg;
-            float dpw = (gamma == 0.f) ? 0.f : gamma * powf(om, gamma - 1.f);
-            float dl_dpt = -alpha * (-dpw * lg + pw / (pt + 1e-12f));
-            float dpt_dx = pos ? p * (1.f - p) : -p * (1.f - p);
-            d = dl_dpt * dpt_dx;
-        }
+        float l, d, p;
+        sed_loss_elem(xi, ti, kind, alpha, gamma, &l, &d, &p);
         acc += (double)l;
         if (dx) dx[i] = d * scale;
         if (probs) probs[i] = p;
diff --git a/sed_crnn_amd/csrc/net.hip b/sed_crnn_amd/csrc/net.hip
--- a/sed_crnn_amd/csrc/net.hip
+++ b/sed_crnn_amd/csrc/net.hip
@@ -25,6 +25,8 @@
     size_t bias_f[SED_MAX_CONV];
     size_t wih_perm;
     size_t gi[SED_MAX_GRU], gout[SED_MAX_GRU], saved[SED_MAX_GRU], gru_ws;
+    size_t gru_wt[SED_MAX_GRU];
+    size_t gru_bpart[SED_MAX_GRU];
     size_t act[SED_MAX_DENSE];
     size_t wgrad_zrow;
     size_t wg_arrive;
@@ -46,7 +48,7 @@
     SED_REQUIRE(c->n_dense >= 1 && c->n_dense <= SED_MAX_DENSE, "net: n_dense=%d out of range", c->n_dense);
     SED_REQUIRE(c->conv_mode >= 0 && c->conv_mode <= 2, "net: conv_mode=%d (0 = exact fp32, 1 = bf16x3 experiment, 2 = bf16 inference)", c->conv_mode);
     SED_REQUIRE(c->conv_mode != 2 || !training, "net: conv_mode 2 (bf16 inference) is an eval-only plan; training runs with conv_mode 0 or 1");
-    SED_REQUIRE((c->flags & ~(SED_NET_AUX_FIRST | SED_NET_NO_GATE | SED_NET_DIRECT_CONV)) == 0, "net: unknown flags 0x%x", c->flags);
+    SED_REQUIRE((c->flags & ~(SED_NET_AUX_FIRST | SED_NET_NO_GATE | SED_NET_DIRECT_CONV | SED_NET_UNFUSED_TAIL | SED_NET_UNFUSED_PACK | SED_NET_UNFUSED_BIAS | SED_NET_UNFUSED_FIN)) == 0, "net: unknown flags 0x%x", c->flags);
     memset(L, 0, sizeof(*L));
     L->n_conv = c->n_conv; L->n_gru = c->n_gru; L->n_dense = c->n_dense;
     const int fm = c->conv_mode == 2 ? 0 : c->conv_mode;
@@ -164,6 +166,7 @@
         if (in > max2H) max2H = in;
     }
     L->gru_ws = cv.take((size_t)6 * maxH * maxH);
+    for (int i = 0; i < c->n_gru; ++i) L->gru_wt[i] = cv.take((size_t)6 * c->H[i] * c->H[i]);
     size_t max_lin_ws = 0;
     for (int j = 0; j < c->n_dense; ++j) {
         SED_REQUIRE(c->D[j] > 0, "net: dense size D[%d]=%d", j, c->D[j]);
@@ -190,9 +193,10 @@
             L->dgh[i] = cv.take(M * 6 * c->H[i]);
         }
         L->gru_bws = cv.take(sed_gru_seq_bwd_workspace_bytes(c->B, maxH) / sizeof(float));
+        for (int i = 0; i < c->n_gru; ++i) L->gru_bpart[i] = cv.take(sed_gru_seq_bwd_workspace_bytes(c->B, c->H[i]) / sizeof(float));
         for (int i = 0; i < c->n_gru; ++i) L->dgout[i] = cv.take(M * 2 * c->H[i]);
         for (int j = 0; j < c->n_dense - 1; ++j) L->dact[j] = cv.take(M * c->D[j]);
-        L->lin_ws = cv.take(max_lin_ws);
+        L->lin_ws = cv.take(max_lin_ws + M);
     }
     {
         size_t gw = 0;
@@ -232,8 +236,9 @@
 }
 
 static int forward_impl(const sed_net_cfg* c, const sed_net_params* p, const float* x, float* logits, void* workspace,
-                        int training, uint64_t seed, const uint64_t* seed_dev, int pb, int pe, float count_scale, void* stream) {
-    SED_REQUIRE(p && x && logits && workspace, "net_forward: null pointer");
+                        int training, uint64_t seed, const uint64_t* seed_dev, int pb, int pe, float count_scale, void* stream,
+                        bool skip_head = false) {
+    SED_REQUIRE(p && x && (logits || skip_head) && workspace, "net_forward: null pointer");
     Layout L;
     SED_TRY(build_layout(c, training, &L));
     SED_REQUIRE(pb >= 0 && pe <= 2 * L.n_conv + 1 && pb < pe, "net_forward: bad phase range [%d,%d)", pb, pe);
@@ -284,6 +289,8 @@
         }
     }
     const bool packed_up_front = !eval_plan && pb == 0 && c->conv_mode == 0 && L.n_conv > 1;
+    const bool fin_fused = !(c->flags & (SED_NET_UNFUSED_TAIL | SED_NET_UNFUSED_FIN));
+    const bool gru_packed = packed_up_front && !(c->flags & (SED_NET_UNFUSED_TAIL | SED_NET_UNFUSED_PACK)) && pe > 2 * L.n_conv;
     if (packed_up_front) {
         const float* w[SED_MAX_CONV]; float* wf[SED_MAX_CONV]; float* wd[SED_MAX_CONV]; int co[SED_MAX_CONV], ci[SED_MAX_CONV];
         int wnf[SED_MAX_CONV], wnd[SED_MAX_CONV];
@@ -292,7 +299,12 @@
             w[l] = p->conv_w[l]; wf[l] = ws + L.wp_f[l]; wd[l] = (training && l > 0) ? ws + L.wp_d[l] : nullptr;
             co[l] = L.cv[l].C; ci[l] = L.cv[l].Cin; wnf[l] = L.cv[l].wino; wnd[l] = L.cv[l].wino_d;
         }
-        SED_TRY(sed_internal_conv_pack_multi(L.n_conv, w, wf, wd, co, ci, wnf, wnd, stream));
+        const float* gw[2 * SED_MAX_GRU]; float* gwt[SED_MAX_GRU]; int gH[SED_MAX_GRU];
+        for (int i = 0; i < L.n_gru && gru_packed; ++i) {
+            SED_REQUIRE(p->gru_whh[i][0] && p->gru_whh[i][1], "net_forward: missing parameters of GRU layer %d", i);
+            gw[2 * i] = p->gru_whh[i][0]; gw[2 * i + 1] = p->gru_whh[i][1]; gwt[i] = ws + L.gru_wt[i]; gH[i] = L.gr[i].H;
+        }
+        SED_TRY(sed_internal_conv_pack_multi(L.n_conv, w, wf, wd, co, ci, wnf, wnd, gru_packed ? L.n_gru : 0, gw, gwt, gH, stream));
     }
     for (int l = 0; l < L.n_conv && !eval_plan; ++l) {
         const ConvL& q = L.cv[l];
@@ -311,7 +323,11 @@
                     SED_TRY(sed_conv3x3_pack_weights_ex(p->conv_w[l], q.wino ? nullptr : ws + L.wp_f[l], q.wino_d ? nullptr : wdp,
                                                         q.C, q.Cin, (l > 0) ? c->conv_mode : 0, stream));
             }
-            if (q.fused) {
+            if (q.fused && training && one_shot && fin_fused) {
+                SED_TRY(sed_conv1_stats_bn_finalize(in, ws + L.wp_f[l], p->conv_b[l], ws + L.stat[l], ws + L.c1_stat_ws, B, q.Cin, q.F, q.T, q.C,
+                                                    q.rgrad ? (double*)(ws + L.c1_mom) : nullptr, p->bn_g[l], p->bn_b[l], p->bn_rm[l], p->bn_rv[l],
+                                                    c->bn_momentum, c->bn_eps, ws + L.mean[l], ws + L.rstd[l], ws + L.scale[l], ws + L.shift[l], stream));
+            } else if (q.fused) {
                 if (training) SED_TRY(sed_conv1_stats(in, ws + L.wp_f[l], p->conv_b[l], ws + L.stat[l], ws + L.c1_stat_ws, B, q.Cin, q.F, q.T, q.C,
                                                       q.rgrad ? (double*)(ws + L.c1_mom) : nullptr, stream));
             } else if (q.wino) {
@@ -325,7 +341,8 @@
         }
         if (!do_b) continue;
         const double count = (double)B * q.T * q.F;
-        if (training && one_shot)
+        if (training && one_shot && q.fused && fin_fused) {
+        } else if (training && one_shot)
             SED_TRY(sed_bn_finalize_train(ws + L.stat[l], q.rows, q.C, count, p->bn_g[l], p->bn_b[l],
                                           p->bn_rm[l], p->bn_rv[l], c->bn_momentum, c->bn_eps, ws + L.mean[l],
                                           ws + L.rstd[l], ws + L.scale[l], ws + L.shift[l], stream));
@@ -376,10 +393,14 @@
         }
         const float* whh[2] = {p->gru_whh[i][0], p->gru_whh[i][1]};
         const float* bhh[2] = {p->gru_bhh[i][0], p->gru_bhh[i][1]};
-        SED_TRY(sed_gru_seq_fwd(ws + L.gi[i], whh, bhh, ws + L.gout[i], training ? ws + L.saved[i] : nullptr,
-                                ws + L.gru_ws, B, L.Tp, H, stream));
+        if (gru_packed)
+            SED_TRY(sed_gru_seq_fwd_packed(ws + L.gi[i], ws + L.gru_wt[i], bhh, ws + L.gout[i], training ? ws + L.saved[i] : nullptr, B, L.Tp, H, stream));
+        else
+            SED_TRY(sed_gru_seq_fwd(ws + L.gi[i], whh, bhh, ws + L.gout[i], training ? ws + L.saved[i] : nullptr,
+                                    ws + L.gru_ws, B, L.Tp, H, stream));
         gin = ws + L.gout[i];
     }
+    if (skip_head) return 0;
     const float* din = gin;
     for (int j = 0; j < L.n_dense; ++j) {
         SED_REQUIRE(p->dense_w[j] && p->dense_b[j], "net_forward: missing parameters of dense layer %d", j);
@@ -394,6 +415,26 @@
 extern "C" int sed_net_forward(const sed_net_cfg* c, const sed_net_params* p, const float* x, float* logits,
                                void* workspace, int training, uint64_t seed, const uint64_t* seed_dev, void* stream) {
     return forward_impl(c, p, x, logits, workspace, training, seed, seed_dev, 0, 2 * (c ? c->n_conv : 0) + 1, 1.f, stream);
+}
+
+extern "C" int sed_net_forward_body(const sed_net_cfg* c, const sed_net_params* p, const float* x, void* workspace,
+                                    uint64_t seed, const uint64_t* seed_dev, void* stream) {
+    return forward_impl(c, p, x, nullptr, workspace, 1, seed, seed_dev, 0, 2 * (c ? c->n_conv : 0) + 1, 1.f, stream, true);
+}
+
+static int fused_head_ok(const Layout& L) { return L.n_dense == 1 && L.dN[0] == 1; }
+
+extern "C" int sed_net_head_loss_rows(const sed_net_cfg* c, const sed_net_params* p, const float* targets, int kind, float alpha,
+                                      float gamma, float* logits, float* dlogits, float* probs, void* workspace, void* stream) {
+    SED_REQUIRE(p && targets && logits && dlogits && probs && workspace, "net_head_loss_rows: null pointer");
+    Layout L;
+    SED_TRY(build_layout(c, 1, &L));
+    SED_REQUIRE(fused_head_ok(L), "net_head_loss_rows: the fused head is one dense layer with one output (this net: %d layers, %d outputs)",
+                L.n_dense, L.dN[L.n_dense - 1]);
+    SED_REQUIRE(p->dense_w[0] && p->dense_b[0], "net_head_loss_rows: missing parameters of dense layer 0");
+    float* ws = (float*)workspace;
+    return sed_head_loss_rows(ws + L.gout[L.n_gru - 1], p->dense_w[0], p->dense_b[0], targets, L.M, L.dK[0], kind, alpha, gamma,
+                              logits, dlogits, probs, ws + L.dgout[L.n_gru - 1], ws + L.lin_ws, stream);
 }
 
 extern "C" int sed_net_forward_phases(const sed_net_cfg* c, const sed_net_params* p, const float* x, float* logits,
@@ -567,10 +608,10 @@
     return sed_conv3x3_fwd_ex(ws + L.dconv[l], 0, ws + L.wp_d[l], nullptr, ws + L.gradA, nullptr, c->B, q.C, q.F, q.T, q.Cin, c->conv_mode, st);
 }
 
-extern "C" int sed_net_backward(const sed_net_cfg* c, const sed_net_params* p, const sed_net_params* g,
-                                const float* x, const float* dlogits, void* workspace, uint64_t seed,
-                                const uint64_t* seed_dev, int stage_begin, int stage_end, void* stream, void* aux_stream) {
-    SED_REQUIRE(p && g && x && dlogits && workspace, "net_backward: null pointer");
+static int backward_impl(const sed_net_cfg* c, const sed_net_params* p, const sed_net_params* g,
+                         const float* x, const float* dlogits, float* fused_loss, void* workspace, uint64_t seed,
+                         const uint64_t* seed_dev, int stage_begin, int stage_end, void* stream, void* aux_stream) {
+    SED_REQUIRE(p && g && x && (dlogits || fused_loss) && workspace, "net_backward: null pointer");
     constexpr int kMaxDev = 16;
     static thread_local hipEvent_t ev_all[kMaxDev][2][SED_MAX_CONV] = {};
     static thread_local hipEvent_t ev_gru_all[kMaxDev][SED_MAX_GRU + 5] = {};
@@ -625,7 +666,11 @@
 
     if (stage_begin == 0) {
         const float* gru_last = ws + L.gout[L.n_gru - 1];
-        for (int j = L.n_dense - 1; j >= 0; --j) {
+        if (fused_loss) {
+            SED_REQUIRE(fused_head_ok(L), "net_backward: the fused head is one dense layer with one output");
+            SED_REQUIRE(g->dense_w[0] && g->dense_b[0], "net_backward: missing gradient buffers of dense layer 0");
+        }
+        for (int j = L.n_dense - 1; j >= 0 && !fused_loss; --j) {
             const int last = (j == L.n_dense - 1);
             const float* xin = (j == 0) ? gru_last : ws + L.act[j - 1];
             float* dy = last ? const_cast<float*>(dlogits) : ws + L.dact[j];
@@ -646,14 +691,21 @@
                             "net_backward: missing gradient buffers of GRU layer %d dir %d", i, d);
             float* dbih[2] = {g->gru_bih[i][0], g->gru_bih[i][1]};
             float* dbhh[2] = {g->gru_bhh[i][0], g->gru_bhh[i][1]};
-            SED_TRY(sed_gru_seq_bwd(ws + L.dgout[i], ws + L.saved[i], whh, dgi, dgh, dbih, dbhh, ws + L.gru_bws, B, L.Tp, H, stream));
+            const bool bias_split = s_aux && !(c->flags & (SED_NET_UNFUSED_TAIL | SED_NET_UNFUSED_BIAS));
+            const bool finish_here = fused_loss && i == L.n_gru - 1;
+            if (bias_split)
+                SED_TRY(sed_gru_seq_bwd_partials(ws + L.dgout[i], ws + L.saved[i], whh, dgi, dgh, ws + L.gru_bpart[i], B, L.Tp, H, stream));
+            else
+                SED_TRY(sed_gru_seq_bwd(ws + L.dgout[i], ws + L.saved[i], whh, dgi, dgh, dbih, dbhh, ws + L.gru_bws, B, L.Tp, H, stream));
+            if (finish_here && !s_aux) SED_TRY(sed_head_loss_finish(ws + L.lin_ws, M, L.dK[0], fused_loss, g->dense_w[0], g->dense_b[0], stream));
             const bool on_aux = s_aux && i > 0;
             void* wst = on_aux ? aux_stream : stream;
             float* wws = ws + (on_aux ? L.gemm_ws_aux : L.gemm_ws);
-            if (on_aux) {
+            if (on_aux || (finish_here && s_aux)) {
                 (void)hipEventRecord(ev_gru[i], s_main);
                 (void)hipStreamWaitEvent(s_aux, ev_gru[i], 0);
             }
+            if (finish_here && s_aux) SED_TRY(sed_head_loss_finish(ws + L.lin_ws, M, L.dK[0], fused_loss, g->dense_w[0], g->dense_b[0], aux_stream));
             auto dw_hh = [&]() -> int {
                 for (int d = 0; d < 2; ++d)
                     SED_TRY(sed_gemm_f32_wgrad(dgh + d * 3 * H, 1, 6 * H, ws + L.saved[i] + ((size_t)d * 5 + 4) * H, 10 * H, 1,
@@ -671,6 +723,7 @@
                 return 0;
             };
             if (on_aux) SED_TRY(dw_ih(aux_stream, wws));
+            if (bias_split && i > 0) SED_TRY(sed_gru_bias_grad(ws + L.gru_bpart[i], dbih, dbhh, B, H, aux_stream));
             if (i == 0 && s_aux) (void)hipEventRecord(ev_gru[SED_MAX_GRU], s_aux);
             if (fused) {
                 SED_TRY(sed_gemm_f32(dgi, 6 * H, 1, p->gru_wih[i][0], K, 1, dxin, K, nullptr, 0.f, M, K, 6 * H, stream));
@@ -688,6 +741,7 @@
             }
             if (!on_aux) SED_TRY(dw_ih(stream, ws + L.gemm_ws));
             if (s_aux && i == 0) SED_TRY(dw_hh());
+            if (bias_split && i == 0) SED_TRY(sed_gru_bias_grad(ws + L.gru_bpart[i], dbih, dbhh, B, H, stream));
         }
         if (s_aux) (void)hipStreamWaitEvent(s_main, ev_gru[SED_MAX_GRU], 0);
     }
@@ -791,6 +845,20 @@
     return 0;
 }
 
+extern "C" int sed_net_backward(const sed_net_cfg* c, const sed_net_params* p, const sed_net_params* g,
+                                const float* x, const float* dlogits, void* workspace, uint64_t seed,
+                                const uint64_t* seed_dev, int stage_begin, int stage_end, void* stream, void* aux_stream) {
+    SED_REQUIRE(dlogits, "net_backward: null pointer");
+    return backward_impl(c, p, g, x, dlogits, nullptr, workspace, seed, seed_dev, stage_begin, stage_end, stream, aux_stream);
+}
+
+extern "C" int sed_net_backward_fused_head(const sed_net_cfg* c, const sed_net_params* p, const sed_net_params* g,
+                                           const float* x, float* loss, void* workspace, uint64_t seed, const uint64_t* seed_dev,
+                                           int stage_begin, int stage_end, void* stream, void* aux_stream) {
+    SED_REQUIRE(loss, "net_backward_fused_head: null pointer");
+    return backward_impl(c, p, g, x, nullptr, loss, workspace, seed, seed_dev, stage_begin, stage_end, stream, aux_stream);
+}
+
 extern "C" int sed_net_backward_ready_stage(const sed_net_cfg* c, int block) {
     if (!c || block < 0 || block >= c->n_conv) { sed_set_error("net_backward_ready_stage: bad arguments"); return SED_EINVAL; }
     return block == 0 ? c->n_conv : c->n_conv - 1;
diff --git a/sed_crnn_amd/model.py b/sed_crnn_amd/model.py
--- a/sed_crnn_amd/model.py
+++ b/sed_crnn_amd/model.py
@@ -160,6 +160,7 @@
         self.flat_features = conv_channels[-1] * f
         self.time_factor = math.prod(pt for _, pt in self.pools)
         self._last = None
+        self._fused_loss = None
         self.overlap_wgrad = True
         self._sync_bn, self._sync_group = False, None
         self._aux_stream = None
@@ -233,7 +234,7 @@
 
     def __getstate__(self):
         st = self.__dict__.copy()
-        for k in ("_structs", "_ws", "_aux_stream", "_last", "_arena", "_arena_grad", "_arena_params", "_grad_views",
+        for k in ("_structs", "_ws", "_aux_stream", "_last", "_fused_loss", "_arena", "_arena_grad", "_arena_params", "_grad_views",
                   "_arena_offsets", "_stage_ends"):
             st.pop(k, None)
         return st
@@ -453,7 +454,11 @@
                                     _lib.stream_ptr()), "sed_net_routing")
         return route
 
-    def _run_forward(self, x, training, step_state=None):
+    def fused_head_supported(self):
+        return (len(self.dense) == 1 and self.dense[0] == 1 and self._sync_world() == 1
+                and not (int(getattr(self, "plan_flags", 0)) & 0x8))
+
+    def _run_forward(self, x, training, step_state=None, head=True):
         self._check_input(x)
         x = x.detach().contiguous().float()
         B, _, _, T = x.shape
@@ -469,8 +474,15 @@
             self._nbt_pending += 1
             self._last = (cfg, ws, x)
             self._last_state = step_state
+            self._fused_loss = None
         seed = self._seed if training else 0
         world = self._sync_world() if training else 1
+        if not head:
+            if not (training and self.fused_head_supported()):
+                raise RuntimeError("sed_crnn_amd: the head-less forward belongs to the fused fit step (fused_head_supported())")
+            check(lib().sed_net_forward_body(C.byref(cfg), C.byref(P), _lib.ptr(x), _lib.ptr(ws), seed, _lib.ptr(step_state),
+                                             _lib.stream_ptr()), "sed_net_forward_body")
+            return None
         if world > 1:
             args = (C.byref(cfg), C.byref(P), _lib.ptr(x), _lib.ptr(logits), _lib.ptr(ws), 1, seed)
             n = len(self.conv_channels)
@@ -484,6 +496,25 @@
                                     int(training), seed, _lib.ptr(step_state) if training else None, _lib.stream_ptr()),
               "sed_net_forward")
         return logits
+
+    def _run_head_loss(self, y, kind="bce", alpha=0.25, gamma=2.0):
+        if kind not in ("bce", "focal"):
+            raise ValueError(f"loss kind must be 'bce' or 'focal', got {kind!r}")
+        if self._last is None:
+            raise RuntimeError("sed_crnn_amd: head + loss without a training forward")
+        cfg, ws, x = self._last
+        P, _ = self._param_structs()
+        shape = (cfg.B, cfg.T // self.time_factor, 1)
+        if tuple(y.shape) != shape:
+            raise ValueError(f"logits {shape} and targets {tuple(y.shape)} differ in shape")
+        y = y.detach().contiguous().float()
+        logits, d, p = (torch.empty(shape, device=x.device, dtype=torch.float32) for _ in range(3))
+        loss = torch.empty(1, device=x.device, dtype=torch.float32)
+        check(lib().sed_net_head_loss_rows(C.byref(cfg), C.byref(P), _lib.ptr(y), 0 if kind == "bce" else 1, alpha, gamma,
+                                           _lib.ptr(logits), _lib.ptr(d), _lib.ptr(p), _lib.ptr(ws), _lib.stream_ptr()),
+              "sed_net_head_loss_rows")
+        self._fused_loss = loss
+        return loss, d, p, logits
 
     def _run_backward(self, x, dlogits, stage_begin=0, stage_end=None):
         if self._last is None:
@@ -508,6 +539,12 @@
         if getattr(self, "_aux_stream", None) is None or self._aux_stream.device != x.device:
             self._aux_stream = torch.cuda.Stream(device=x.device)
         aux = C.c_void_p(self._aux_stream.cuda_stream) if self.overlap_wgrad else None
+        fused_loss = getattr(self, "_fused_loss", None)
+        if fused_loss is not None:
+            check(lib().sed_net_backward_fused_head(C.byref(cfg), C.byref(P), C.byref(G), _lib.ptr(x), _lib.ptr(fused_loss),
+                                                    _lib.ptr(ws), self._seed, _lib.ptr(getattr(self, "_last_state", None)),
+                                                    stage_begin, stage_end, _lib.stream_ptr(), aux), "sed_net_backward_fused_head")
+            return
         check(lib().sed_net_backward(C.byref(cfg), C.byref(P), C.byref(G), _lib.ptr(x), _lib.ptr(dlogits),
                                      _lib.ptr(ws), self._seed, _lib.ptr(getattr(self, "_last_state", None)), stage_begin,
                                      stage_end, _lib.stream_ptr(), aux), "sed_net_backward")
diff --git a/sed_crnn_amd/ops.py b/sed_crnn_amd/ops.py
--- a/sed_crnn_amd/ops.py
+++ b/sed_crnn_amd/ops.py
@@ -317,6 +317,21 @@
     check(lib().sed_loss_fwd_bwd(ptr(_f32c(logits)), ptr(_f32c(targets)), n, 0 if kind == "bce" else 1, alpha, gamma,
                                  int(reduction == "mean"), ptr(loss), ptr(d), ptr(p), stream_ptr()), "loss_fwd_bwd")
     return loss, d, p
+
+
+def head_loss_fwd_bwd(x, W, b, targets, kind="bce", alpha=0.25, gamma=2.0):
+    if kind not in ("bce", "focal"):
+        raise ValueError(f"loss kind must be 'bce' or 'focal', got {kind!r}")
+    M, K = x.shape
+    if tuple(W.shape) != (1, K) or targets.numel() != M:
+        raise ValueError(f"head_loss_fwd_bwd: x {tuple(x.shape)}, W {tuple(W.shape)} (one output), {targets.numel()} targets")
+    x, W, t = _f32c(x), _f32c(W), _f32c(targets)
+    ws = torch.empty(lib().sed_head_loss_workspace_bytes(M, K) // 4 + 1, device=x.device)
+    logits, d, p = (torch.empty(M, 1, device=x.device) for _ in range(3))
+    loss, dx, dW, db = torch.empty(1, device=x.device), torch.empty_like(x), torch.empty_like(W), torch.empty(1, device=x.device)
+    check(lib().sed_head_loss_fwd_bwd(ptr(x), ptr(W), ptr(b), ptr(t), M, K, 0 if kind == "bce" else 1, alpha, gamma, ptr(logits),
+                                      ptr(loss), ptr(d), ptr(p), ptr(dx), ptr(dW), ptr(db), ptr(ws), stream_ptr()), "head_loss_fwd_bwd")
+    return loss, p, d, dx, dW, db, logits
 
 
 def sigmoid(x):
diff --git a/sed_crnn_amd/trainer.py b/sed_crnn_amd/trainer.py
--- a/sed_crnn_amd/trainer.py
+++ b/sed_crnn_amd/trainer.py
@@ -60,8 +60,12 @@
         if state is not None:
             from ._lib import check, lib, ptr, stream_ptr
             check(lib().sed_step_advance(ptr(state), stream_ptr()), "sed_step_advance")
-        logits = m._run_forward(x, training=True, step_state=state)
-        loss, dlogits, probs = ops.loss_fwd_bwd(logits, y, self.loss_kind, self.alpha, self.gamma, "mean")
+        if m.fused_head_supported() and self.loss_kind in ("bce", "focal"):
+            m._run_forward(x, training=True, step_state=state, head=False)
+            loss, dlogits, probs, _ = m._run_head_loss(y, self.loss_kind, self.alpha, self.gamma)
+        else:
+            logits = m._run_forward(x, training=True, step_state=state)
+            loss, dlogits, probs = ops.loss_fwd_bwd(logits, y, self.loss_kind, self.alpha, self.gamma, "mean")
         nstage = len(m.conv_channels) + 1
         if self.reducer is None:
             m._run_backward(x, dlogits, 0, nstage)
```

Measured after the change: 5.981 million mel-frames/s (median of 6 runs). No clear change (+1.0%).
